# zenustech/zpc

Hardware: AMD Instinct MI355X
Metric: particle*steps/s (P2G+G2P) (higher is better)
Workload: dtype f32

## Files before the change

include/zs_rocm.h:

```cpp
#ifndef ZS_ROCM_H
#define ZS_ROCM_H
#include <stdbool.h>
#include <stddef.h>
#include <stdint.h>

#ifdef __cplusplus
extern "C" {
#endif

#if defined(__GNUC__)
#  define ZS_ROCM_EXPORT __attribute__((visibility("default")))
#else
#  define ZS_ROCM_EXPORT
#endif

typedef struct zs_rocm_policy zs_rocm_policy;

ZS_ROCM_EXPORT zs_rocm_policy *policy__device(void);
ZS_ROCM_EXPORT void del_policy__device(zs_rocm_policy *);
ZS_ROCM_EXPORT void zs_rocm_policy_sync(zs_rocm_policy *, int sync);
ZS_ROCM_EXPORT void zs_rocm_policy_profile(zs_rocm_policy *, int profile);
ZS_ROCM_EXPORT void zs_rocm_policy_device(zs_rocm_policy *, int procid);
ZS_ROCM_EXPORT void zs_rocm_policy_stream(zs_rocm_policy *, int streamid);
ZS_ROCM_EXPORT void zs_rocm_policy_listen(zs_rocm_policy *, int incomingProc, int incomingStreamid);
// ... 315 lines not shown
typedef struct {
  zs_rocm_attr mass;
  zs_rocm_attr pos;
  zs_rocm_attr vel;
  zs_rocm_attr C;
  zs_rocm_attr F;
  zs_rocm_attr logJp;
  zs_rocm_attr stress;
  size_t n;
} zs_rocm_particles;

enum {
  ZS_MPM_FIXED_COROTATED = 0, ZS_MPM_DRUCKER_PRAGER = 1, ZS_MPM_VONMISES_FIXED_COROTATED = 2, ZS_MPM_NACC = 3,
  ZS_MPM_EQUATION_OF_STATE = 4
};
typedef struct {
  int model;
  float dx, dt;
  float volume, E, nu;
  float cohesion, beta, yieldSurface;
  int volCorrection;
  int side;
  int keyIsOrigin;
  float yieldStress;
  float xi, Msqr;
  int hardeningOn;
  float bulk, viscosity;
} zs_rocm_mpm_params;
ZS_ROCM_EXPORT float zs_rocm_nacc_msqr(float fa);


ZS_ROCM_EXPORT void zs_rocm_mpm_compute_sparsity(zs_rocm_policy *, zs_rocm_bht_3 *, zs_rocm_attr pos, size_t n,
                                                 float dx, int side, int keyIsOrigin);
ZS_ROCM_EXPORT void zs_rocm_mpm_enlarge_sparsity(zs_rocm_policy *, zs_rocm_bht_3 *, const int lo[3], const int hi[3],
                                                 int keyStride);
typedef struct zs_rocm_index_buckets zs_rocm_index_buckets;
typedef struct {
  zs_rocm_hashtable *table;
  int *indices;
  int *offsets, *counts;
  int numBuckets, numEntries;
  float dx;
} zs_rocm_index_buckets_view;
ZS_ROCM_EXPORT zs_rocm_index_buckets *zs_rocm_index_buckets_create(void);
ZS_ROCM_EXPORT void zs_rocm_index_buckets_destroy(zs_rocm_index_buckets *);
ZS_ROCM_EXPORT void zs_rocm_index_buckets_get_view(const zs_rocm_index_buckets *, zs_rocm_index_buckets_view *out);
ZS_ROCM_EXPORT void zs_rocm_index_buckets_for_particles(zs_rocm_policy *, zs_rocm_index_buckets *, zs_rocm_attr pos, size_t n,
                                                        float dx, float displacement, size_t expectedCells);
ZS_ROCM_EXPORT void zs_rocm_index_buckets_for_partition(zs_rocm_policy *, zs_rocm_index_buckets *, zs_rocm_attr pos, size_t n, float dx,
                                                        const zs_rocm_bht_3 *table, int side, int keyIsOrigin);
ZS_ROCM_EXPORT void zs_rocm_mpm_partition_for_particles(zs_rocm_policy *, zs_rocm_hashtable *, zs_rocm_attr pos, size_t n,
                                                        float dx, int blocklen);
ZS_ROCM_EXPORT void zs_rocm_mpm_enlarge_sparsity__hashtable(zs_rocm_policy *, zs_rocm_hashtable *, const int lo[3],
                                                            const int hi[3]);

ZS_ROCM_EXPORT void zs_rocm_mpm_bin_particles(zs_rocm_policy *, const zs_rocm_bht_3 *, zs_rocm_attr pos, size_t n,
                                              float dx, int side, int keyIsOrigin, int *order, int *binStart,
                                              unsigned *cellCount);
ZS_ROCM_EXPORT void zs_rocm_mpm_build_neighbors(zs_rocm_policy *, const zs_rocm_bht_3 *, int *nbr, int keyStride);

ZS_ROCM_EXPORT void zs_rocm_mpm_p2g(zs_rocm_policy *, const zs_rocm_mpm_params *, zs_rocm_particles,
                                    const zs_rocm_bht_3 *, float *grid, size_t nblocks, const int *binStart,
                                    const unsigned *cellCount, const int *nbr);
ZS_ROCM_EXPORT void zs_rocm_mpm_grid_update(zs_rocm_policy *, const zs_rocm_mpm_params *, float *grid, size_t nblocks,
                                            const float extf[3], float *maxVelSqr);
enum { ZS_ROCM_GEOM_PLANE = 0, ZS_ROCM_GEOM_CUBOID = 1, ZS_ROCM_GEOM_SPHERE = 2, ZS_ROCM_GEOM_CYLINDER = 3 };
enum { ZS_ROCM_COLLIDER_STICKY = 0, ZS_ROCM_COLLIDER_SLIP = 1, ZS_ROCM_COLLIDER_SEPARATE = 2 };
typedef struct zs_rocm_collider {
  int geometry, type;
  float param[8];
  float s, dsdt;
  float R[9];
  float omega[3];
  float b[3], dbdt[3];
} zs_rocm_collider;
ZS_ROCM_EXPORT void zs_rocm_collider_init(zs_rocm_collider *c, int geometry, int type, const float *param, int nparam);
ZS_ROCM_EXPORT void zs_rocm_mpm_apply_boundary(zs_rocm_policy *, const zs_rocm_mpm_params *, const zs_rocm_bht_3 *, float *grid,
                                               size_t nblocks, const zs_rocm_collider *collider);
ZS_ROCM_EXPORT void zs_rocm_collider_resolve(zs_rocm_policy *, const zs_rocm_collider *collider, const float *x, float *v, size_t n,
                                             int *inside);
ZS_ROCM_EXPORT int zs_rocm_mpm_p2c2g(zs_rocm_policy *, const zs_rocm_mpm_params *, zs_rocm_particles, const zs_rocm_index_buckets *buckets,
                                     const zs_rocm_bht_3 *, float *grid, size_t nblocks, int kind);
ZS_ROCM_EXPORT void zs_rocm_mpm_pre_g2c2p(zs_rocm_policy *, zs_rocm_particles);
ZS_ROCM_EXPORT int zs_rocm_mpm_g2c2p(zs_rocm_policy *, const zs_rocm_mpm_params *, zs_rocm_particles, const zs_rocm_index_buckets *buckets,
                                     const zs_rocm_bht_3 *, const float *grid, size_t nblocks);
ZS_ROCM_EXPORT void zs_rocm_mpm_post_g2c2p(zs_rocm_policy *, const zs_rocm_mpm_params *, zs_rocm_particles);
ZS_ROCM_EXPORT int zs_rocm_mpm_g2c2p_step(zs_rocm_policy *, const zs_rocm_mpm_params *, zs_rocm_particles, const zs_rocm_bht_3 *,
                                          const float *grid, size_t nblocks);
ZS_ROCM_EXPORT void zs_rocm_mpm_g2p(zs_rocm_policy *, const zs_rocm_mpm_params *, zs_rocm_particles,
                                    const zs_rocm_bht_3 *, const float *grid, size_t nblocks, const int *binStart,
                                    const unsigned *cellCount, const int *nbr);
ZS_ROCM_EXPORT int zs_rocm_mpm_implicit_force(zs_rocm_policy *, const zs_rocm_mpm_params *, zs_rocm_particles, const zs_rocm_bht_3 *,
                                              size_t nblocks, const int *binStart, const unsigned *cellCount, const int *nbr,
                                              const float *vIn, float *fOut, float *trial);
ZS_ROCM_EXPORT int zs_rocm_mpm_implicit_multiply(zs_rocm_policy *, const zs_rocm_mpm_params *, zs_rocm_particles, const zs_rocm_bht_3 *,
                                                 const float *grid, size_t nblocks, const int *binStart, const unsigned *cellCount,
                                                 const int *nbr, const float *vIn, float *out);
ZS_ROCM_EXPORT int zs_rocm_mpm_implicit_project(zs_rocm_policy *, const zs_rocm_mpm_params *, const zs_rocm_bht_3 *, const float *grid,
                                                size_t nblocks, const zs_rocm_collider *collider, float *inout);
ZS_ROCM_EXPORT int zs_rocm_mpm_implicit_precondition(zs_rocm_policy *, const float *grid, size_t nblocks, int side, const float *in,
                                                     float *out);
ZS_ROCM_EXPORT void zs_rocm_dof_assign(zs_rocm_policy *, const float *a, float *b, size_t n);
ZS_ROCM_EXPORT void zs_rocm_dof_fill(zs_rocm_policy *, float *a, float v, size_t n);
ZS_ROCM_EXPORT int zs_rocm_dof_compwise(zs_rocm_policy *, int op, const float *a, const float *b, float *c, size_t n);
ZS_ROCM_EXPORT void zs_rocm_dof_linear_combine(zs_rocm_policy *, float m, const float *a, float n_, const float *b, float *c, size_t n);
ZS_ROCM_EXPORT void zs_rocm_dof_dot(zs_rocm_policy *, const float *a, const float *b, size_t n, float *out);
ZS_ROCM_EXPORT int zs_rocm_mpm_implicit_solve(zs_rocm_policy *, const zs_rocm_mpm_params *, zs_rocm_particles, const zs_rocm_bht_3 *,
                                              const float *grid, size_t nblocks, const int *binStart, const unsigned *cellCount,
                                              const int *nbr, const zs_rocm_collider *collider, const float *b, float *x, int maxIters,
                                              float tol, float relTol, int *iters);
typedef struct zs_rocm_levelset {
  zs_rocm_bht_view_lite table;
  const float *tiles;
  size_t numBlocks;
  int numChannels, sdfChannel, velChannel;
  float h;
  float origin[3];
  float background;
  unsigned *stats;
} zs_rocm_levelset;
ZS_ROCM_EXPORT int zs_rocm_levelset_sample(zs_rocm_policy *, const zs_rocm_levelset *, const float *x, size_t n, float *sdf, float *normal,
                                           float *vel);
ZS_ROCM_EXPORT int zs_rocm_levelset_collider_resolve(zs_rocm_policy *, const zs_rocm_collider *collider, const zs_rocm_levelset *, const float *x,
                                                     float *v, size_t n, int *inside);
ZS_ROCM_EXPORT int zs_rocm_mpm_apply_boundary_levelset(zs_rocm_policy *, const zs_rocm_mpm_params *, const zs_rocm_bht_3 *, float *grid,
                                                       size_t nblocks, const zs_rocm_collider *collider, const zs_rocm_levelset *);
ZS_ROCM_EXPORT int zs_rocm_mpm_implicit_project_levelset(zs_rocm_policy *, const zs_rocm_mpm_params *, const zs_rocm_bht_3 *, const float *grid,
                                                         size_t nblocks, const zs_rocm_collider *collider, const zs_rocm_levelset *,
                                                         float *inout);
ZS_ROCM_EXPORT int zs_rocm_mpm_implicit_solve_levelset(zs_rocm_policy *, const zs_rocm_mpm_params *, zs_rocm_particles, const zs_rocm_bht_3 *,
                                                       const float *grid, size_t nblocks, const int *binStart, const unsigned *cellCount,
                                                       const int *nbr, const zs_rocm_collider *collider, const zs_rocm_levelset *,
                                                       const float *b, float *x, int maxIters, float tol, float relTol, int *iters);
typedef struct zs_rocm_levelset_transition {
  zs_rocm_levelset src, dst;
  float stepDt, alpha, maxSpeed;
} zs_rocm_levelset_transition;
ZS_ROCM_EXPORT int zs_rocm_levelset_max_speed(zs_rocm_policy *, const zs_rocm_levelset *, float *out);
ZS_ROCM_EXPORT int zs_rocm_levelset_transition_sample(zs_rocm_policy *, const zs_rocm_levelset_transition *, const float *x, size_t n, float *sdf,
                                                      float *normal, float *vel);
ZS_ROCM_EXPORT int zs_rocm_levelset_transition_collider_resolve(zs_rocm_policy *, const zs_rocm_collider *collider,
                                                                const zs_rocm_levelset_transition *, const float *x, float *v, size_t n,
                                                                int *inside);
ZS_ROCM_EXPORT int zs_rocm_mpm_apply_boundary_transition(zs_rocm_policy *, const zs_rocm_mpm_params *, const zs_rocm_bht_3 *, float *grid,
                                                         size_t nblocks, const zs_rocm_collider *collider, const zs_rocm_levelset_transition *);
ZS_ROCM_EXPORT int zs_rocm_mpm_implicit_project_transition(zs_rocm_policy *, const zs_rocm_mpm_params *, const zs_rocm_bht_3 *, const float *grid,
                                                           size_t nblocks, const zs_rocm_collider *collider,
                                                           const zs_rocm_levelset_transition *, float *inout);
ZS_ROCM_EXPORT int zs_rocm_mpm_implicit_solve_transition(zs_rocm_policy *, const zs_rocm_mpm_params *, zs_rocm_particles, const zs_rocm_bht_3 *,
                                                         const float *grid, size_t nblocks, const int *binStart, const unsigned *cellCount,
                                                         const int *nbr, const zs_rocm_collider *collider,
                                                         const zs_rocm_levelset_transition *, const float *b, float *x, int maxIters, float tol,
                                                         float relTol, int *iters);
typedef struct zs_rocm_mesh zs_rocm_mesh;
typedef struct {
  const float *verts;
  const int *tris;
  const float *vel;
  const float *faceNormals, *vertNormals, *edgeNormals;
  zs_rocm_lbvh_view bvh;
  int numVerts, numTris;
} zs_rocm_mesh_view;
#define ZS_ROCM_MESH_STAT_WORDS 8
ZS_ROCM_EXPORT zs_rocm_mesh *zs_rocm_mesh_create(zs_rocm_policy *, const float *verts, size_t nv, const int *tris, size_t nt, const float *vel);
ZS_ROCM_EXPORT void zs_rocm_mesh_destroy(zs_rocm_mesh *);
ZS_ROCM_EXPORT int zs_rocm_mesh_refit(zs_rocm_policy *, zs_rocm_mesh *, const float *verts, const float *vel);
ZS_ROCM_EXPORT void zs_rocm_mesh_stats(zs_rocm_policy *, const zs_rocm_mesh *, int *out);
ZS_ROCM_EXPORT int zs_rocm_mesh_total_box(zs_rocm_policy *, const zs_rocm_mesh *, float *box6);
ZS_ROCM_EXPORT void zs_rocm_mesh_get_view(const zs_rocm_mesh *, zs_rocm_mesh_view *out);
ZS_ROCM_EXPORT int zs_rocm_mesh_closest_point(zs_rocm_policy *, const zs_rocm_mesh *, const float *points, size_t nq, float cap, float *dist,
                                              int *tri, int *feature, float *bary);
ZS_ROCM_EXPORT int zs_rocm_mesh_signed_distance(zs_rocm_policy *, const zs_rocm_mesh *, const float *points, size_t nq, float cap, float *sdf,
                                                float *vel);
ZS_ROCM_EXPORT size_t zs_rocm_mesh_levelset_count(zs_rocm_policy *, const zs_rocm_mesh *, const float *origin, float voxel, float band);
ZS_ROCM_EXPORT int zs_rocm_mesh_levelset_candidates(zs_rocm_policy *, const zs_rocm_mesh *, const float *origin, float voxel, float band,
                                                    zs_rocm_bht_3 *cand);
ZS_ROCM_EXPORT int zs_rocm_mesh_levelset_blocks(zs_rocm_policy *, const zs_rocm_mesh *, const float *origin, float voxel, float band,
                                                const zs_rocm_bht_3 *cand, size_t ncand, float *tiles, int numChannels, int *keep,
                                                unsigned *stats);
ZS_ROCM_EXPORT size_t zs_rocm_mesh_levelset_select(zs_rocm_policy *, const zs_rocm_bht_3 *cand, size_t ncand, const int *keep, int *keptKeys);
ZS_ROCM_EXPORT int zs_rocm_mesh_levelset_gather(zs_rocm_policy *, const zs_rocm_bht_3 *cand, size_t ncand, const int *keep, const float *tiles,
                                                const zs_rocm_bht_3 *table, float *dstTiles, int numChannels);
#define ZS_ROCM_SLOT_STATUS_WORDS (8 + 2 * 256)
ZS_ROCM_EXPORT size_t zs_rocm_mpm_slot_outbox_bytes(size_t nbins, int outboxCap, int which);
ZS_ROCM_EXPORT void zs_rocm_mpm_build_neighbors27(zs_rocm_policy *, const zs_rocm_bht_3 *, int *nbr27 , int keyStride);
ZS_ROCM_EXPORT int zs_rocm_mpm_slot_particles(zs_rocm_policy *, const zs_rocm_bht_3 *, zs_rocm_attr pos, size_t n, float dx, int side,
                                              int keyIsOrigin, int K, const float *src, float *dst, int C, unsigned *cellMask, int *status);
ZS_ROCM_EXPORT size_t zs_rocm_mpm_slot_list(zs_rocm_policy *, const unsigned *cellMask, size_t nbins, int K, int *slots);
typedef struct zs_rocm_slot_storage {
  unsigned *cellMask;
  int K;
  const int *nbr;
  const int *nbr27;
  int *moverCount;
  unsigned *claim;
  float *moverRec;
  int outboxCap;
  int *status;
  const unsigned char *blockEdge;
} zs_rocm_slot_storage;
ZS_ROCM_EXPORT void zs_rocm_mpm_partition_edge(zs_rocm_policy *, const zs_rocm_bht_3 *, unsigned char *edge , int keyStride,
                                               int lo, int hi);
ZS_ROCM_EXPORT void zs_rocm_mpm_slot_compute_sparsity(zs_rocm_policy *, const zs_rocm_bht_3 *oldTab, const unsigned *cellMask, size_t nblocksOld,
                                                      int side, int keyIsOrigin, zs_rocm_bht_3 *newTab);
ZS_ROCM_EXPORT int zs_rocm_mpm_reslot(zs_rocm_policy *, const zs_rocm_bht_3 *oldTab, const zs_rocm_bht_3 *newTab, int side, int K, int C,
                                      const float *oldBuf, float *newBuf, const unsigned *oldMask, unsigned *newMask, const float *oldGrid,
                                      float *newGrid, int *status);
ZS_ROCM_EXPORT int zs_rocm_mpm_g2p2g_slots(zs_rocm_policy *, const zs_rocm_mpm_params *, zs_rocm_particles, const zs_rocm_bht_3 *,
                                           const float *gridA, float *gridB, size_t nblocks, const zs_rocm_slot_storage *st, int writeAll,
                                           size_t blockBegin, size_t blockEnd, int finish);
ZS_ROCM_EXPORT int zs_rocm_mpm_g2p2g_slotted(zs_rocm_policy *, const zs_rocm_mpm_params *, zs_rocm_particles, const zs_rocm_bht_3 *,
                                             const float *gridA, float *gridB, size_t nblocks, unsigned *cellMask, int K, const int *nbr,
                                             const int *nbr27, int *moverCount, unsigned *claim, float *moverRec, int outboxCap,
                                             int writeAll, int *status);
ZS_ROCM_EXPORT int zs_rocm_mpm_g2p2g_slotted_range(zs_rocm_policy *, const zs_rocm_mpm_params *, zs_rocm_particles, const zs_rocm_bht_3 *,
                                                   const float *gridA, float *gridB, size_t nblocks, unsigned *cellMask, int K, const int *nbr,
                                                   const int *nbr27, int *moverCount, unsigned *claim, float *moverRec, int outboxCap,
                                                   int writeAll, int *status, size_t blockBegin, size_t blockEnd, int finish);
ZS_ROCM_EXPORT int zs_rocm_mpm_g2p2g(zs_rocm_policy *, const zs_rocm_mpm_params *, zs_rocm_particles, const zs_rocm_bht_3 *,
                                     const float *gridA, float *gridB, size_t nblocks, const int *binStart,
                                     const unsigned *cellCount, const int *nbr, int writeAll);
ZS_ROCM_EXPORT int zs_rocm_mpm_g2p2g_range(zs_rocm_policy *, const zs_rocm_mpm_params *, zs_rocm_particles, const zs_rocm_bht_3 *,
                                           const float *gridA, float *gridB, size_t nblocks, const int *binStart,
                                           const unsigned *cellCount, const int *nbr, int writeAll, size_t blockBegin,
                                           size_t blockEnd, int *driftFlag);
ZS_ROCM_EXPORT int zs_rocm_mpm_g2p2g_reorder_range(zs_rocm_policy *, const zs_rocm_mpm_params *, zs_rocm_particles particlesOut,
                                                   zs_rocm_particles particlesIn, const int *order, const zs_rocm_bht_3 *,
                                                   const float *gridA, float *gridB, size_t nblocks, const int *binStart,
                                                   const unsigned *cellCount, const int *nbr, int writeAll, size_t blockBegin,
                                                   size_t blockEnd, int *driftFlag);
ZS_ROCM_EXPORT void zs_rocm_mpm_update_stress(zs_rocm_policy *, const zs_rocm_mpm_params *, zs_rocm_particles);
ZS_ROCM_EXPORT int zs_rocm_mpm_stress_channels(void);
ZS_ROCM_EXPORT void zs_rocm_mpm_stress(zs_rocm_policy *, const zs_rocm_mpm_params *, float *F, float *logJp, size_t n, float *PF);
ZS_ROCM_EXPORT void zs_rocm_svd3(zs_rocm_policy *, const float *F, size_t n, float *U, float *S, float *V);

ZS_ROCM_EXPORT void zs_rocm_mpm_owner_rank(zs_rocm_policy *, zs_rocm_attr pos, size_t n, float dx, const int lo[3], const int hi[3],
                                           const int dims[3], int align, int *owner);
ZS_ROCM_EXPORT void zs_rocm_mpm_owner_counts(zs_rocm_policy *, const int *owner, size_t n, int world, int *counts);
ZS_ROCM_EXPORT void zs_rocm_mpm_halo_pack(zs_rocm_policy *, const float *grid, const int *blocks, size_t nb, int side,
                                          int chn0, int nchn, float *buf);
ZS_ROCM_EXPORT void zs_rocm_mpm_halo_unpack(zs_rocm_policy *, float *grid, const int *blocks, size_t nb, int side,
                                            int chn0, int nchn, const float *buf, int add);


typedef struct zs_rocm_dist zs_rocm_dist;
ZS_ROCM_EXPORT size_t zs_rocm_dist_unique_id_bytes(void);
ZS_ROCM_EXPORT int zs_rocm_dist_unique_id(void *out);
ZS_ROCM_EXPORT zs_rocm_dist *zs_rocm_dist_create(int rank, int world, const void *uniqueId, int device);
ZS_ROCM_EXPORT void zs_rocm_dist_destroy(zs_rocm_dist *);
ZS_ROCM_EXPORT int zs_rocm_dist_rank(const zs_rocm_dist *);
ZS_ROCM_EXPORT int zs_rocm_dist_world(const zs_rocm_dist *);
ZS_ROCM_EXPORT int zs_rocm_dist_comm_count(const zs_rocm_dist *);
ZS_ROCM_EXPORT int zs_rocm_dist_halo_exchange(zs_rocm_dist *, zs_rocm_policy *, float *grid, int side, int chn0, int nchn, const int *blocks,
                                              size_t totalBlocks, int npeers, const int *peerRank, const size_t *peerOffset,
                                              const size_t *peerCount, float *sendbuf, float *recvbuf);
ZS_ROCM_EXPORT int zs_rocm_dist_allreduce_f32(zs_rocm_dist *, zs_rocm_policy *, float *buf, size_t n, int op);
ZS_ROCM_EXPORT int zs_rocm_dist_allreduce_i64(zs_rocm_dist *, zs_rocm_policy *, long long *buf, size_t n, int op);
ZS_ROCM_EXPORT int zs_rocm_dist_alltoall_i64(zs_rocm_dist *, zs_rocm_policy *, const long long *send, long long *recv);
ZS_ROCM_EXPORT int zs_rocm_dist_alltoallv_f32(zs_rocm_dist *, zs_rocm_policy *, const float *send, const size_t *sendCounts,
                                              const size_t *sendOffsets, float *recv, const size_t *recvCounts, const size_t *recvOffsets);
ZS_ROCM_EXPORT int zs_rocm_dist_barrier(zs_rocm_dist *, zs_rocm_policy *);
typedef struct zs_rocm_halo_plan zs_rocm_halo_plan;
ZS_ROCM_EXPORT size_t zs_rocm_halo_plan_from_keys(const int *keysAll, const size_t *counts, int world, int rank, int *npeers, int *peerRank,
                                                  size_t *peerOffset, size_t *peerCount, int *blocks);
ZS_ROCM_EXPORT zs_rocm_halo_plan *zs_rocm_dist_halo_plan_create(zs_rocm_dist *, zs_rocm_policy *, const int *keys, size_t nblocks, int side);
ZS_ROCM_EXPORT void zs_rocm_dist_halo_plan_destroy(zs_rocm_halo_plan *);
ZS_ROCM_EXPORT int zs_rocm_dist_halo_plan_npeers(const zs_rocm_halo_plan *);
ZS_ROCM_EXPORT size_t zs_rocm_dist_halo_plan_blocks(const zs_rocm_halo_plan *);
ZS_ROCM_EXPORT size_t zs_rocm_dist_halo_plan_bytes(const zs_rocm_halo_plan *);
ZS_ROCM_EXPORT const int *zs_rocm_dist_halo_plan_block_list(const zs_rocm_halo_plan *);
ZS_ROCM_EXPORT int zs_rocm_dist_halo_plan_exchange(zs_rocm_halo_plan *, zs_rocm_dist *, zs_rocm_policy *, float *grid, int chn0, int nchn);
ZS_ROCM_EXPORT zs_rocm_halo_plan *zs_rocm_dist_halo_plan_from_lists(zs_rocm_dist *, int side, int npeers, const int *peerRank,
                                                                    const size_t *peerOffset, const size_t *peerCount, const int *blocks,
                                                                    size_t total);
typedef struct zs_rocm_mpm_step {
  const zs_rocm_mpm_params *params;
  zs_rocm_particles particles;
  const zs_rocm_bht_3 *table;
  const float *gridA;
  float *gridB;
  size_t nblocks;
  const zs_rocm_slot_storage *storage;
  int writeAll;
  float extf[3];
  float *maxVelSqr;
  const zs_rocm_collider *collider;
  size_t nBoundary;
  zs_rocm_dist *dist;
  zs_rocm_halo_plan *plan;
  zs_rocm_policy *commPolicy;
  float *haloGrid;
  void *evTransferBegin, *evTransferEnd;
  void **evBreakdown;
  int haloChannels;
  int rangeSchedule;
  float *handoverSnapshot;
  const zs_rocm_levelset *levelset;
} zs_rocm_mpm_step;
#define ZS_ROCM_STEP_EVENTS 8
#define ZS_ROCM_RANGES_IN_TURN 0
#define ZS_ROCM_RANGES_SIDE_BY_SIDE 1
#define ZS_ROCM_RANGES_ONE_LAUNCH 2
ZS_ROCM_EXPORT int zs_rocm_mpm_step_slotted(zs_rocm_policy *, const zs_rocm_mpm_step *);

#ifdef __cplusplus
}
#endif
#endif
```

zpc_amd/_lib.py:

```python
import ctypes as C
import os

_HERE = os.path.dirname(os.path.abspath(__file__))
LIB_PATH = os.path.join(_HERE, "lib", "libzsrocm.so")
if os.environ.get("ZS_ROCM_LIB"):
    LIB_PATH = os.environ["ZS_ROCM_LIB"]
    print("[zpc_amd] using HIP library %s" % LIB_PATH, flush=True)


class Port(C.Structure):
    _fields_ = [("base", C.c_void_p), ("idx", C.c_uint32), ("numTileBits", C.c_uint32),
                ("tileMask", C.c_uint32), ("numChns", C.c_uint32)]


class HashTableView(C.Structure):
    _fields_ = [("keys", C.c_void_p), ("indices", C.c_void_p), ("status", C.c_void_p), ("activeKeys", C.c_void_p),
                ("cnt", C.c_void_p), ("tableSize", C.c_int)]


class LBvhView(C.Structure):
    _fields_ = [("orderedBvs", C.c_void_p), ("parents", C.c_void_p), ("levels", C.c_void_p), ("leafInds", C.c_void_p),
                ("auxIndices", C.c_void_p), ("numNodes", C.c_int), ("numLeaves", C.c_int)]


# ... 51 lines not shown
def lib():
    global _lib
    if _lib is None:
        if not os.path.exists(LIB_PATH):
            raise RuntimeError(
                "libzsrocm.so not built (%s): run `python -m zpc_amd.build` -- zpc_amd has no CPU fallback" % LIB_PATH)
        try:
            import torch
        except ImportError:
            pass
        _lib = C.CDLL(LIB_PATH)
        _declare(_lib)
    return _lib


class Collider(C.Structure):
    _fields_ = [("geometry", C.c_int), ("type", C.c_int), ("param", C.c_float * 8), ("s", C.c_float), ("dsdt", C.c_float),
                ("R", C.c_float * 9), ("omega", C.c_float * 3), ("b", C.c_float * 3), ("dbdt", C.c_float * 3)]


class LevelSet(C.Structure):
    _fields_ = [("table", BhtViewLite), ("tiles", C.c_void_p), ("numBlocks", C.c_size_t), ("numChannels", C.c_int),
                ("sdfChannel", C.c_int), ("velChannel", C.c_int), ("h", C.c_float), ("origin", C.c_float * 3), ("background", C.c_float),
                ("stats", C.c_void_p)]


class LevelSetTransition(C.Structure):
    _fields_ = [("src", LevelSet), ("dst", LevelSet), ("stepDt", C.c_float), ("alpha", C.c_float), ("maxSpeed", C.c_float)]


class MeshView(C.Structure):
    _fields_ = [("verts", C.c_void_p), ("tris", C.c_void_p), ("vel", C.c_void_p), ("faceNormals", C.c_void_p), ("vertNormals", C.c_void_p),
                ("edgeNormals", C.c_void_p), ("bvh", LBvhView), ("numVerts", C.c_int), ("numTris", C.c_int)]


def _declare(L):
    vp, sz, i32, f32 = C.c_void_p, C.c_size_t, C.c_int, C.c_float
    L.policy__device.restype = vp
    L.del_policy__device.argtypes = [vp]
    for n in ("sync", "profile", "device", "stream", "block"):
        getattr(L, "zs_rocm_policy_" + n).argtypes = [vp, i32]
    L.zs_rocm_policy_listen.argtypes = [vp, i32, i32]
    L.zs_rocm_policy_shmem.argtypes = [vp, sz]
    L.zs_rocm_policy_external_stream.argtypes = [vp, vp]
    L.zs_rocm_policy_get_stream.argtypes = [vp]
    L.zs_rocm_policy_get_stream.restype = vp
    L.zs_rocm_policy_should_sync.argtypes = [vp]
    L.zs_rocm_policy_sync_ctx.argtypes = [vp]
    L.zs_rocm_policy_last_elapsed_ms.argtypes = [vp]
    L.zs_rocm_policy_last_elapsed_ms.restype = f32
    L.zs_rocm_memset.argtypes = [vp, vp, i32, sz]
    L.zs_rocm_dist_unique_id_bytes.restype = sz
    L.zs_rocm_dist_unique_id.argtypes = [vp]
    L.zs_rocm_dist_create.argtypes = [i32, i32, vp, i32]
    L.zs_rocm_dist_create.restype = vp
    L.zs_rocm_dist_destroy.argtypes = [vp]
    L.zs_rocm_dist_rank.argtypes = [vp]
    L.zs_rocm_dist_world.argtypes = [vp]
    L.zs_rocm_dist_comm_count.argtypes = [vp]
    L.zs_rocm_dist_comm_count.restype = C.c_int
    L.zs_rocm_dist_halo_exchange.argtypes = [vp, vp, vp, i32, i32, i32, vp, sz, i32, vp, vp, vp, vp, vp]
    L.zs_rocm_dist_allreduce_f32.argtypes = [vp, vp, vp, sz, i32]
    L.zs_rocm_dist_allreduce_i64.argtypes = [vp, vp, vp, sz, i32]
    L.zs_rocm_dist_alltoall_i64.argtypes = [vp, vp, vp, vp]
    L.zs_rocm_dist_alltoallv_f32.argtypes = [vp, vp, vp, vp, vp, vp, vp, vp]
    L.zs_rocm_dist_barrier.argtypes = [vp, vp]
    L.zs_rocm_halo_plan_from_keys.argtypes = [vp, vp, i32, i32, vp, vp, vp, vp, vp]
    L.zs_rocm_halo_plan_from_keys.restype = sz
    L.zs_rocm_dist_halo_plan_create.argtypes = [vp, vp, vp, sz, i32]
    L.zs_rocm_dist_halo_plan_create.restype = vp
    L.zs_rocm_dist_halo_plan_destroy.argtypes = [vp]
    L.zs_rocm_dist_halo_plan_npeers.argtypes = [vp]
    L.zs_rocm_dist_halo_plan_npeers.restype = i32
    L.zs_rocm_dist_halo_plan_blocks.argtypes = [vp]
    L.zs_rocm_dist_halo_plan_blocks.restype = sz
    L.zs_rocm_dist_halo_plan_bytes.argtypes = [vp]
    L.zs_rocm_dist_halo_plan_bytes.restype = sz
    L.zs_rocm_dist_halo_plan_block_list.argtypes = [vp]
    L.zs_rocm_dist_halo_plan_block_list.restype = vp
    L.zs_rocm_dist_halo_plan_exchange.argtypes = [vp, vp, vp, vp, i32, i32]
    L.zs_rocm_dist_halo_plan_exchange.restype = i32
    L.zs_rocm_mpm_slot_outbox_bytes.argtypes = [sz, i32, i32]
    L.zs_rocm_mpm_slot_outbox_bytes.restype = sz
    L.zs_rocm_mpm_build_neighbors27.argtypes = [vp, vp, vp, i32]
    L.zs_rocm_mpm_slot_particles.argtypes = [vp, vp, Port, sz, f32, i32, i32, i32, vp, vp, i32, vp, vp]
    L.zs_rocm_mpm_slot_particles.restype = i32
    L.zs_rocm_mpm_slot_list.argtypes = [vp, vp, sz, i32, vp]
    L.zs_rocm_mpm_slot_list.restype = sz
    L.zs_rocm_policy_temporary.argtypes = [vp, sz]
    L.zs_rocm_policy_temporary.restype = vp
    L.zs_rocm_policy_temporary_free.argtypes = [vp, vp]
    L.zs_rocm_last_error.argtypes = [i32]
    L.zs_rocm_clear_error.argtypes = [i32]
    L.launch__device.argtypes = [vp, vp, sz, vp]
    L.rocm_compile_program.argtypes = [C.c_char_p, i32, C.c_char_p, C.c_bool, C.c_bool, C.c_bool, C.c_bool, C.c_char_p]
    L.rocm_compile_program.restype = sz
    L.rocm_load_module.argtypes = [vp, C.c_char_p]
    L.rocm_load_module.restype = vp
    L.rocm_unload_module.argtypes = [vp, vp]
    L.rocm_get_kernel.argtypes = [vp, vp, C.c_char_p]
    L.rocm_get_kernel.restype = vp
    L.rocm_launch_kernel.argtypes = [vp, vp, sz, vp, vp]
    L.rocm_launch_kernel.restype = sz
    for T in ("int", "float", "double"):
        for op in ("reduce_sum", "reduce_prod", "reduce_min", "reduce_max", "exclusive_scan_sum",
                   "exclusive_scan_prod", "inclusive_scan_sum", "inclusive_scan_prod"):
            getattr(L, "%s__rocm_%s_1" % (op, T)).argtypes = [vp, Port, Port, Port]
        getattr(L, "radix_sort__rocm_%s_1" % T).argtypes = [vp, Port, Port, Port]
        getattr(L, "merge_sort__rocm_%s_1" % T).argtypes = [vp, Port, Port]
        getattr(L, "merge_sort_pair__rocm_%s_1" % T).argtypes = [vp, Port, Port, sz]
        getattr(L, "radix_sort_pair__rocm_%s_1" % T).argtypes = [vp, Port, Port, Port, Port, sz]
    for S, ct in (("i32", C.c_int32), ("i64", C.c_int64), ("f32", C.c_float), ("f64", C.c_double)):
        getattr(L, "zs_rocm_reduce_" + S).argtypes = [vp, vp, sz, vp, ct, i32]
        getattr(L, "zs_rocm_scan_" + S).argtypes = [vp, vp, sz, vp, ct, i32, i32]
    for S in ("i32", "u32", "i64", "u64"):
        getattr(L, "zs_rocm_radix_sort_" + S).argtypes = [vp, vp, vp, vp, vp, sz, i32, i32]
    for S in ("i32", "u32", "i64", "u64", "f32", "f64"):
        getattr(L, "zs_rocm_merge_sort_" + S).argtypes = [vp, vp, vp, sz, i32]


def _declare_containers(L):
    vp, sz, i32, f32, i8 = C.c_void_p, C.c_size_t, C.c_int, C.c_float, C.c_int8
    L.allocator.argtypes = [i32, i8]
    L.allocator.restype = vp
    L.del_allocator.argtypes = [vp]
    L.property_tags.argtypes = [C.POINTER(C.c_char_p), C.POINTER(C.c_int), sz]
    L.property_tags.restype = vp
    L.del_property_tags.argtypes = [vp]
    L.allocator_virtual.argtypes = [i32, i8, sz]
    L.allocator_virtual.restype = vp
    L.del_allocator_virtual.argtypes = [vp]
    L.property_tags_get_item.argtypes = [vp, sz, C.POINTER(C.c_char_p), C.POINTER(sz)]
    L.property_tags_get_size.argtypes = [vp]
    L.property_tags_get_size.restype = sz
    for T, ct in (("int", C.c_int), ("float", C.c_float), ("double", C.c_double)):
        for sfx in ("", "_virtual"):
            g = lambda n: getattr(L, (n % T) + sfx)
            g("container__v_%s").argtypes = [vp, sz]
            g("container__v_%s").restype = vp
            g("del_container__v_%s").argtypes = [vp]
            g("relocate_container__v_%s").argtypes = [vp, i32, i8]
            g("resize_container__v_%s").argtypes = [vp, sz]
            g("reset_container__v_%s").argtypes = [vp, i32]
            g("container_size__v_%s").argtypes = [vp]
            g("container_size__v_%s").restype = sz
            g("container_capacity__v_%s").argtypes = [vp]
            g("container_capacity__v_%s").restype = sz
            g("get_val_container__v_%s").argtypes = [vp]
            g("get_val_container__v_%s").restype = ct
            g("set_val_container__v_%s").argtypes = [vp, ct]
            g("get_val_i_container__v_%s").argtypes = [vp, sz]
            g("get_val_i_container__v_%s").restype = ct
            g("set_val_i_container__v_%s").argtypes = [vp, sz, ct]
            g("copy_to_container__v_%s").argtypes = [vp, vp]
            g("copy_from_container__v_%s").argtypes = [vp, vp]
            g("get_handle_container__v_%s").argtypes = [vp]
            g("get_handle_container__v_%s").restype = vp
            g("pyview__v_%s").argtypes = [vp]
            g("pyview__v_%s").restype = C.POINTER(C.c_void_p)
            g("pyview__v_const_%s").argtypes = [vp]
            g("pyview__v_const_%s").restype = C.POINTER(C.c_void_p)
            for it in ("get_iterator_1__v_%s", "get_iterator_1__v_const_%s", "get_iterator_3__v_%s", "get_iterator_3__v_const_%s"):
                g(it).argtypes = [vp, C.c_uint32]
                g(it).restype = Port
        getattr(L, "del_pyview__v_%s" % T).argtypes = [vp]
        getattr(L, "del_pyview__v_const_%s" % T).argtypes = [vp]
        getattr(L, "container_data__v_%s" % T).argtypes = [vp]
        getattr(L, "container_data__v_%s" % T).restype = vp
        for Lw in (8, 32, 64, 512):
            s = "%s_%d" % (T, Lw)
            for sfx in ("", "_virtual"):
                h = lambda n: getattr(L, (n % s) + sfx)
                h("container__tv_%s").argtypes = [vp, vp, sz]
                h("container__tv_%s").restype = vp
                h("del_container__tv_%s").argtypes = [vp]
                h("relocate_container__tv_%s").argtypes = [vp, i32, i8]
                h("resize_container__tv_%s").argtypes = [vp, sz]
                h("reset_container__tv_%s").argtypes = [vp, i32]
                for q in ("container_size__tv_%s", "container_capacity__tv_%s"):
                    h(q).argtypes = [vp]
                    h(q).restype = sz
                h("property_offset__tv_%s").argtypes = [vp, C.c_char_p]
                h("property_size__tv_%s").argtypes = [vp, C.c_char_p]
                for it in ("get_iterator_1__tv_%s", "get_iterator_3__tv_%s"):
                    h(it).argtypes = [vp, C.c_uint32, C.c_uint32]
                    h(it).restype = Port
                for it in ("get_iterator_1__tv_const_%s", "get_iterator_3__tv_const_%s"):
                    h(it).argtypes = [vp, C.c_uint32, C.c_uint32]
                    h(it).restype = Port
                for pv, rt in (("pyview__tv_%s", TvViewLite), ("pyview__tv_const_%s", TvViewLite), ("pyview__tvn_%s", TvNamedViewLite),
                               ("pyview__tvn_const_%s", TvNamedViewLite)):
                    h(pv).argtypes = [vp]
                    h(pv).restype = C.POINTER(rt)
                h("append_properties__rocm_tv_%s").argtypes = [vp, vp, vp]
            k = lambda n: getattr(L, n % s)
            for dv in ("del_pyview__tv_%s", "del_pyview__tv_const_%s", "del_pyview__tvn_%s", "del_pyview__tvn_const_%s"):
                k(dv).argtypes = [vp]
            k("container_num_channels__tv_%s").argtypes = [vp]
            k("container_num_channels__tv_%s").restype = sz
            k("container_data__tv_%s").argtypes = [vp]
            k("container_data__tv_%s").restype = vp
            k("zs_rocm_fill__tv_%s").argtypes = [vp, vp, ct]
            k("zs_rocm_reorder__tv_%s").argtypes = [vp, vp, vp, i32]
    L.zs_rocm_tv_from_aos_f32.argtypes = [vp, vp, sz, i32, i32, vp]
    L.zs_rocm_tv_to_aos_f32.argtypes = [vp, vp, sz, i32, i32, vp]
    L.zs_rocm_tv_scale_f32.argtypes = [vp, vp, sz, i32, i32, f32]
    L.zs_rocm_tv_gather_f32.argtypes = [vp, vp, vp, sz, i32, i32, vp]
    L.zs_rocm_tv_gather_channels_f32.argtypes = [vp, vp, vp, sz, i32, i32, vp, C.c_uint64]
    L.zs_rocm_tv_gather_rows_f32.argtypes = [vp, vp, vp, sz, i32, i32, vp]
    L.zs_rocm_tv_scatter_rows_f32.argtypes = [vp, vp, sz, i32, i32, vp, sz]
    for D, B in ((d, b) for d in (1, 2, 3, 4) for b in (16, 32)):
        s = "bht_int_%d_int_%d" % (D, B)
        for sfx in ("", "_virtual"):
            getattr(L, "relocate_container__" + s + sfx).argtypes = [vp, i32, i8]
            getattr(L, "pyview__bht_const_int_%d_int_%d" % (D, B) + sfx).argtypes = [vp]
            getattr(L, "pyview__bht_const_int_%d_int_%d" % (D, B) + sfx).restype = C.POINTER(BhtViewLite)
            if sfx:
                getattr(L, "container__" + s + sfx).argtypes = [vp, sz]
                getattr(L, "container__" + s + sfx).restype = vp
                getattr(L, "del_container__" + s + sfx).argtypes = [vp]
                getattr(L, "container_size__" + s + sfx).argtypes = [vp]
                getattr(L, "container_size__" + s + sfx).restype = sz
        getattr(L, "container__" + s).argtypes = [vp, sz]
        getattr(L, "container__" + s).restype = vp
        getattr(L, "del_container__" + s).argtypes = [vp]
        getattr(L, "container_size__" + s).argtypes = [vp]
        getattr(L, "container_size__" + s).restype = sz
        getattr(L, "container_capacity__" + s).argtypes = [vp]
        getattr(L, "container_capacity__" + s).restype = sz
        getattr(L, "reset_container__" + s).argtypes = [vp, i32]
        getattr(L, "pyview__" + s).argtypes = [vp]
        getattr(L, "pyview__" + s).restype = C.POINTER(BhtViewLite)
        getattr(L, "del_pyview__" + s).argtypes = [C.POINTER(BhtViewLite)]
        getattr(L, "resize_container__rocm_" + s).argtypes = [vp, vp, sz]
        getattr(L, "zs_rocm_insert__" + s).argtypes = [vp, vp, vp, sz, vp]
        getattr(L, "zs_rocm_query__" + s).argtypes = [vp, vp, vp, sz, vp]
        getattr(L, "zs_rocm_assign__" + s).argtypes = [vp, vp, vp, sz]
        getattr(L, "zs_rocm_reorder__" + s).argtypes = [vp, vp, vp, i32]
        getattr(L, "zs_rocm_canonicalize__" + s).argtypes = [vp, vp]
        getattr(L, "zs_rocm_canonicalize_axes__" + s).argtypes = [vp, vp, C.POINTER(C.c_int)]
        getattr(L, "zs_rocm_canonicalize_axes__" + s).restype = i32
        getattr(L, "zs_rocm_canonicalize_tail__" + s).argtypes = [vp, vp, C.POINTER(C.c_int), sz]
        getattr(L, "zs_rocm_canonicalize_tail__" + s).restype = i32
        getattr(L, "zs_rocm_order_morton__" + s).argtypes = [vp, vp]
    L.zs_rocm_hashtable_create.argtypes = [i32, sz, i32, i32]
    L.zs_rocm_hashtable_create.restype = vp
    L.zs_rocm_hashtable_destroy.argtypes = [vp]
    L.zs_rocm_hashtable_dim.argtypes = [vp]
    L.zs_rocm_hashtable_table_size.argtypes = [vp]
    L.zs_rocm_hashtable_table_size.restype = sz
    L.zs_rocm_hashtable_size.argtypes = [vp]
    L.zs_rocm_hashtable_get_view.argtypes = [vp, C.POINTER(HashTableView)]
    L.zs_rocm_hashtable_reset.argtypes = [vp, vp, i32]
    L.zs_rocm_hashtable_insert.argtypes = [vp, vp, vp, sz, vp]
    L.zs_rocm_hashtable_insert_ids.argtypes = [vp, vp, vp, vp, sz, vp]
    L.zs_rocm_hashtable_query.argtypes = [vp, vp, vp, sz, vp]
    L.zs_rocm_hashtable_entry.argtypes = [vp, vp, vp, sz, vp]
    L.zs_rocm_hashtable_resize.argtypes = [vp, vp, sz]
    L.zs_rocm_hashtable_preserve.argtypes = [vp, vp, sz]
    L.zs_rocm_mpm_partition_for_particles.argtypes = [vp, vp, Port, sz, f32, i32]
    L.zs_rocm_mpm_enlarge_sparsity__hashtable.argtypes = [vp, vp, C.POINTER(C.c_int), C.POINTER(C.c_int)]
    L.zs_rocm_lbvh_create.restype = vp
    L.zs_rocm_lbvh_destroy.argtypes = [vp]
    L.zs_rocm_lbvh_num_leaves.argtypes = [vp]
    L.zs_rocm_lbvh_num_leaves.restype = sz
    L.zs_rocm_lbvh_num_nodes.argtypes = [vp]
    L.zs_rocm_lbvh_num_nodes.restype = sz
    L.zs_rocm_lbvh_get_view.argtypes = [vp, C.POINTER(LBvhView)]
    L.zs_rocm_lbvh_build.argtypes = [vp, vp, vp, sz, i32]
    L.zs_rocm_lbvh_refit.argtypes = [vp, vp, vp, sz]
    L.zs_rocm_lbvh_total_box.argtypes = [vp, vp, vp]
    L.zs_rocm_lbvh_query_count.argtypes = [vp, vp, vp, sz, vp]
    L.zs_rocm_lbvh_query_fill.argtypes = [vp, vp, vp, sz, vp, vp]
    L.zs_rocm_lbvh_self_query_count.argtypes = [vp, vp, vp]
    L.zs_rocm_lbvh_self_query_fill.argtypes = [vp, vp, vp, vp]
    L.zs_rocm_index_buckets_create.restype = vp
    L.zs_rocm_index_buckets_destroy.argtypes = [vp]
    L.zs_rocm_index_buckets_get_view.argtypes = [vp, C.POINTER(IndexBucketsView)]
    L.zs_rocm_index_buckets_for_particles.argtypes = [vp, vp, Port, sz, f32, f32, sz]
    L.zs_rocm_index_buckets_for_partition.argtypes = [vp, vp, Port, sz, f32, vp, i32, i32]
    PP = C.POINTER(MpmParams)
    L.zs_rocm_mpm_compute_sparsity.argtypes = [vp, vp, Port, sz, f32, i32, i32]
    L.zs_rocm_mpm_enlarge_sparsity.argtypes = [vp, vp, C.POINTER(C.c_int), C.POINTER(C.c_int), i32]
    L.zs_rocm_mpm_bin_particles.argtypes = [vp, vp, Port, sz, f32, i32, i32, vp, vp, vp]
    L.zs_rocm_mpm_build_neighbors.argtypes = [vp, vp, vp, i32]
    L.zs_rocm_mpm_p2g.argtypes = [vp, PP, Particles, vp, vp, sz, vp, vp, vp]
    L.zs_rocm_mpm_owner_rank.argtypes = [vp, Port, sz, f32, C.POINTER(C.c_int), C.POINTER(C.c_int), C.POINTER(C.c_int), i32, vp]
    L.zs_rocm_mpm_owner_counts.argtypes = [vp, vp, sz, i32, vp]
    L.zs_rocm_mpm_owner_counts.restype = None
    L.zs_rocm_mpm_g2p2g.argtypes = [vp, PP, Particles, vp, vp, vp, sz, vp, vp, vp, i32]
    L.zs_rocm_mpm_g2p2g_range.argtypes = [vp, PP, Particles, vp, vp, vp, sz, vp, vp, vp, i32, sz, sz, vp]
    L.zs_rocm_mpm_g2p2g_slotted.argtypes = [vp, PP, Particles, vp, vp, vp, sz, vp, i32, vp, vp, vp, vp, vp, i32, i32, vp]
    L.zs_rocm_mpm_g2p2g_slotted.restype = i32
    L.zs_rocm_mpm_g2p2g_slotted_range.argtypes = [vp, PP, Particles, vp, vp, vp, sz, vp, i32, vp, vp, vp, vp, vp, i32, i32, vp, sz, sz, i32]
    L.zs_rocm_mpm_g2p2g_slotted_range.restype = i32
    L.zs_rocm_mpm_g2p2g_slots.argtypes = [vp, PP, Particles, vp, vp, vp, sz, C.POINTER(SlotStorage), i32, sz, sz, i32]
    L.zs_rocm_mpm_g2p2g_slots.restype = i32
    L.zs_rocm_mpm_partition_edge.argtypes = [vp, vp, vp, i32, i32, i32]
    L.zs_rocm_mpm_slot_compute_sparsity.argtypes = [vp, vp, vp, sz, i32, i32, vp]
    L.zs_rocm_mpm_reslot.argtypes = [vp, vp, vp, i32, i32, i32, vp, vp, vp, vp, vp, vp, vp]
    L.zs_rocm_mpm_reslot.restype = i32
    L.zs_rocm_mpm_step_slotted.argtypes = [vp, C.POINTER(MpmStep)]
    L.zs_rocm_mpm_step_slotted.restype = i32
    L.zs_rocm_dist_halo_plan_from_lists.argtypes = [vp, i32, i32, C.POINTER(C.c_int), C.POINTER(C.c_size_t), C.POINTER(C.c_size_t),
                                                    C.POINTER(C.c_int), sz]
    L.zs_rocm_dist_halo_plan_from_lists.restype = vp
    L.zs_rocm_mpm_g2p2g_reorder_range.argtypes = [vp, PP, Particles, Particles, vp, vp, vp, vp, sz, vp, vp, vp, i32, sz, sz, vp]
    L.zs_rocm_mpm_grid_update.argtypes = [vp, PP, vp, sz, C.POINTER(C.c_float), vp]
    L.zs_rocm_mpm_g2p.argtypes = [vp, PP, Particles, vp, vp, sz, vp, vp, vp]
    L.zs_rocm_mpm_p2c2g.argtypes = [vp, PP, Particles, vp, vp, vp, sz, i32]
    L.zs_rocm_mpm_p2c2g.restype = i32
    L.zs_rocm_mpm_pre_g2c2p.argtypes = [vp, Particles]
    L.zs_rocm_mpm_g2c2p.argtypes = [vp, PP, Particles, vp, vp, vp, sz]
    L.zs_rocm_mpm_g2c2p.restype = i32
    L.zs_rocm_mpm_post_g2c2p.argtypes = [vp, PP, Particles]
    L.zs_rocm_mpm_g2c2p_step.argtypes = [vp, PP, Particles, vp, vp, sz]
    L.zs_rocm_mpm_g2c2p_step.restype = i32
    L.zs_rocm_mpm_stress.argtypes = [vp, PP, vp, vp, sz, vp]
    L.zs_rocm_mpm_update_stress.argtypes = [vp, PP, Particles]
    L.zs_rocm_svd3.argtypes = [vp, vp, sz, vp, vp, vp]
    L.zs_rocm_nacc_msqr.argtypes = [f32]
    L.zs_rocm_nacc_msqr.restype = f32
    L.zs_rocm_collider_init.argtypes = [C.POINTER(Collider), i32, i32, C.POINTER(C.c_float), i32]
    L.zs_rocm_mpm_apply_boundary.argtypes = [vp, PP, vp, vp, sz, C.POINTER(Collider)]
    L.zs_rocm_collider_resolve.argtypes = [vp, C.POINTER(Collider), vp, vp, sz, vp]
    L.zs_rocm_mpm_implicit_force.argtypes = [vp, PP, Particles, vp, sz, vp, vp, vp, vp, vp, vp]
    L.zs_rocm_mpm_implicit_multiply.argtypes = [vp, PP, Particles, vp, vp, sz, vp, vp, vp, vp, vp]
    L.zs_rocm_mpm_implicit_project.argtypes = [vp, PP, vp, vp, sz, C.POINTER(Collider), vp]
    L.zs_rocm_mpm_implicit_precondition.argtypes = [vp, vp, sz, i32, vp, vp]
    L.zs_rocm_mpm_implicit_solve.argtypes = [vp, PP, Particles, vp, vp, sz, vp, vp, vp, C.POINTER(Collider), vp, vp, i32, f32, f32,
                                             C.POINTER(C.c_int)]
    for name in ("force", "multiply", "project", "precondition", "solve"):
        getattr(L, "zs_rocm_mpm_implicit_" + name).restype = i32
    PC, PL = C.POINTER(Collider), C.POINTER(LevelSet)
    L.zs_rocm_levelset_sample.argtypes = [vp, PL, vp, sz, vp, vp, vp]
    L.zs_rocm_levelset_collider_resolve.argtypes = [vp, PC, PL, vp, vp, sz, vp]
    L.zs_rocm_mpm_apply_boundary_levelset.argtypes = [vp, PP, vp, vp, sz, PC, PL]
    L.zs_rocm_mpm_implicit_project_levelset.argtypes = [vp, PP, vp, vp, sz, PC, PL, vp]
    L.zs_rocm_mpm_implicit_solve_levelset.argtypes = [vp, PP, Particles, vp, vp, sz, vp, vp, vp, PC, PL, vp, vp, i32, f32, f32,
                                                      C.POINTER(C.c_int)]
    for name in ("levelset_sample", "levelset_collider_resolve", "mpm_apply_boundary_levelset", "mpm_implicit_project_levelset",
                 "mpm_implicit_solve_levelset"):
        getattr(L, "zs_rocm_" + name).restype = i32
    PT = C.POINTER(LevelSetTransition)
    L.zs_rocm_levelset_max_speed.argtypes = [vp, PL, vp]
    L.zs_rocm_levelset_transition_sample.argtypes = [vp, PT, vp, sz, vp, vp, vp]
    L.zs_rocm_levelset_transition_collider_resolve.argtypes = [vp, PC, PT, vp, vp, sz, vp]
    L.zs_rocm_mpm_apply_boundary_transition.argtypes = [vp, PP, vp, vp, sz, PC, PT]
    L.zs_rocm_mpm_implicit_project_transition.argtypes = [vp, PP, vp, vp, sz, PC, PT, vp]
    L.zs_rocm_mpm_implicit_solve_transition.argtypes = [vp, PP, Particles, vp, vp, sz, vp, vp, vp, PC, PT, vp, vp, i32, f32, f32,
                                                        C.POINTER(C.c_int)]
    for name in ("levelset_max_speed", "levelset_transition_sample", "levelset_transition_collider_resolve", "mpm_apply_boundary_transition",
                 "mpm_implicit_project_transition", "mpm_implicit_solve_transition"):
        getattr(L, "zs_rocm_" + name).restype = i32
    L.zs_rocm_mesh_create.argtypes = [vp, vp, sz, vp, sz, vp]
    L.zs_rocm_mesh_create.restype = vp
    L.zs_rocm_mesh_destroy.argtypes = [vp]
    L.zs_rocm_mesh_destroy.restype = None
    L.zs_rocm_mesh_refit.argtypes = [vp, vp, vp, vp]
    L.zs_rocm_mesh_stats.argtypes = [vp, vp, C.POINTER(C.c_int)]
    L.zs_rocm_mesh_stats.restype = None
    L.zs_rocm_mesh_total_box.argtypes = [vp, vp, C.POINTER(C.c_float)]
    L.zs_rocm_mesh_get_view.argtypes = [vp, C.POINTER(MeshView)]
    L.zs_rocm_mesh_get_view.restype = None
    L.zs_rocm_mesh_closest_point.argtypes = [vp, vp, vp, sz, f32, vp, vp, vp, vp]
    L.zs_rocm_mesh_signed_distance.argtypes = [vp, vp, vp, sz, f32, vp, vp]
    P3 = C.POINTER(C.c_float)
    L.zs_rocm_mesh_levelset_count.argtypes = [vp, vp, P3, f32, f32]
    L.zs_rocm_mesh_levelset_count.restype = sz
    L.zs_rocm_mesh_levelset_candidates.argtypes = [vp, vp, P3, f32, f32, vp]
    L.zs_rocm_mesh_levelset_blocks.argtypes = [vp, vp, P3, f32, f32, vp, sz, vp, i32, vp, vp]
    L.zs_rocm_mesh_levelset_select.argtypes = [vp, vp, sz, vp, vp]
    L.zs_rocm_mesh_levelset_select.restype = sz
    L.zs_rocm_mesh_levelset_gather.argtypes = [vp, vp, sz, vp, vp, vp, vp, i32]
    for name in ("refit", "total_box", "closest_point", "signed_distance", "levelset_candidates", "levelset_blocks", "levelset_gather"):
        getattr(L, "zs_rocm_mesh_" + name).restype = i32
    L.zs_rocm_dof_assign.argtypes = [vp, vp, vp, sz]
    L.zs_rocm_dof_assign.restype = None
    L.zs_rocm_dof_fill.argtypes = [vp, vp, f32, sz]
    L.zs_rocm_dof_fill.restype = None
    L.zs_rocm_dof_compwise.argtypes = [vp, i32, vp, vp, vp, sz]
    L.zs_rocm_dof_compwise.restype = i32
    L.zs_rocm_dof_linear_combine.argtypes = [vp, f32, vp, f32, vp, vp, sz]
    L.zs_rocm_dof_linear_combine.restype = None
    L.zs_rocm_dof_dot.argtypes = [vp, vp, vp, sz, vp]
    L.zs_rocm_dof_dot.restype = None
    L.zs_rocm_mpm_halo_pack.argtypes = [vp, vp, vp, sz, i32, i32, i32, vp]
    L.zs_rocm_mpm_halo_unpack.argtypes = [vp, vp, vp, sz, i32, i32, i32, vp, i32]


_declare_base = _declare


def _declare(L):
    _declare_base(L)
    _declare_containers(L)
```

zpc_amd/csrc/common.hpp:

```cpp
#pragma once
#include <hip/hip_runtime.h>

#include <cstdint>
#include <cstdio>
#include <cstdlib>
#include <map>
#include <mutex>
#include <vector>

#include "../../include/zs_rocm.h"

namespace zsr {

constexpr int kWave = 64;
constexpr int kNumSpareStreams = 32;
constexpr size_t kCtlBytes = 132 << 10;
constexpr size_t kCtlDesc8 = 32 << 10, kCtlTicket = 128 << 10;
constexpr size_t kCtlScanTiles = 4096;

struct DeviceContext {
  int dev = 0;
  hipStream_t streams[kNumSpareStreams] = {};
  hipEvent_t events[kNumSpareStreams + 1] = {};
  int errorStatus = 0;
  bool errorPrinted = false;
  int cuCount = 0;
  std::mutex mtx;
  struct Block {
    char *ptr = nullptr;
    size_t cap = 0;
  };
  struct Arena {
    std::vector<Block> blocks;
    char *ctl = nullptr;
    unsigned scanGen = 0, ticketShadow = 0;
  };
  std::map<hipStream_t, Arena> arenas;
};

DeviceContext &context(int dev);
int current_device();
void report_error(hipError_t e, const char *what, const char *file, int line);

struct DeviceGuard {
  int prev, dev;
  explicit DeviceGuard(int d) : prev(current_device()), dev(d) {
    if (dev >= 0 && dev != prev) (void)hipSetDevice(dev);
  }
  ~DeviceGuard() {
    if (dev >= 0 && dev != prev) (void)hipSetDevice(prev);
  }
};

#define ZSR_CHECK(expr)                                                  \
  do {                                                                   \
    hipError_t _e = (expr);                                              \
    if (_e != hipSuccess) ::zsr::report_error(_e, #expr, __FILE__, __LINE__); \
  } while (0)

}

struct zs_rocm_allocator {
  int memsrc;
  int8_t devid;
  size_t virtualReserve = 0;
};

struct zs_rocm_policy {
  int sync = 1;
  int profile = 0;
  int device = -1;
  int streamid = -1;
  int listenProc = -1, listenStream = -1;
  size_t shmem = 0;
  int block = 0;
  hipStream_t external = nullptr;
  bool hasExternal = false;
  float lastMs = 0.f;
};

namespace zsr {

struct Launch {
  explicit Launch(zs_rocm_policy *p, const char *what);
  ~Launch();
  hipStream_t stream = nullptr;
  int dev = 0, prevDev = 0;
  zs_rocm_policy *pol;
  const char *what;
  hipEvent_t t0 = nullptr, t1 = nullptr;
  void *temp(size_t bytes);
  std::vector<size_t> tempUsed;
  DeviceContext::Arena &control();
  char *scan_control(size_t numTiles, unsigned &gen, unsigned &ticketBase, bool &wrapped);
  void scan_control_reset();
  unsigned cu_count();
};

template <class T> struct Port {
  T *base;
  uint32_t idx, bits, mask, chns;
  __host__ __device__ __forceinline__ size_t off(size_t i) const {
    size_t j = (size_t)idx + i;
    return (((j >> bits) * (size_t)chns) << bits) | (j & (size_t)mask);
  }
  __host__ __device__ __forceinline__ T &operator[](size_t i) const { return base[off(i)]; }
  __host__ __device__ __forceinline__ size_t cstride() const { return (size_t)mask + 1; }
  __host__ __device__ bool contiguous() const { return chns == 1; }
};
template <class T, class P> inline Port<T> make_port(const P &p) {
  return Port<T>{(T *)p.base, p.idx, p.numTileBits, p.tileMask, p.numChns};
}
template <class T> inline Port<T> contiguous_port(T *p) { return Port<T>{p, 0u, 0u, 0u, 1u}; }

inline unsigned ceil_div(size_t a, size_t b) { return (unsigned)((a + b - 1) / b); }

int mpm_g2p2g_slots_signal(zs_rocm_policy *pol, const zs_rocm_mpm_params *p, zs_rocm_particles ps, const zs_rocm_bht_3 *tab, const float *gridA,
                           float *gridB, size_t nblocks, const zs_rocm_slot_storage *st, int writeAll, size_t blockBegin, size_t blockEnd, int finish,
                           unsigned long long *signal, size_t signalBlocks);
bool levelset_collider_ok(const zs_rocm_collider *collider, const zs_rocm_levelset *levelset);
void levelset_blocks_enqueue(hipStream_t stream, const zs_rocm_mpm_params *p, const int *activeKeys, float *grid, size_t nblocks,
                             const zs_rocm_collider *collider, const zs_rocm_levelset *levelset, float *dof);
bool levelset_ok(const zs_rocm_levelset *levelset);
bool transition_collider_ok(const zs_rocm_collider *collider, const zs_rocm_levelset_transition *transition);
bool transition_blocks_enqueue(hipStream_t stream, const zs_rocm_mpm_params *p, const int *activeKeys, float *grid, size_t nblocks,
                               const zs_rocm_collider *collider, const zs_rocm_levelset_transition *transition, float *dof);

}

namespace zsr {

__device__ __forceinline__ int lane_id() { return (int)(threadIdx.x & 63); }
__device__ __forceinline__ int wave_id() { return (int)(threadIdx.x >> 6); }

template <class T> __device__ __forceinline__ T shfl_down(T v, int d) { return __shfl_down(v, d, 64); }
template <class T> __device__ __forceinline__ T shfl_up(T v, int d) { return __shfl_up(v, d, 64); }
template <class T> __device__ __forceinline__ T shfl(T v, int l) { return __shfl(v, l, 64); }

__device__ __forceinline__ unsigned long long lanemask_lt() {
  return (1ull << (threadIdx.x & 63)) - 1ull;
}

enum { OP_PLUS = 0, OP_MUL = 1, OP_MIN = 2, OP_MAX = 3 };
template <int OP, class T> __host__ __device__ __forceinline__ T apply(T a, T b) {
  if constexpr (OP == OP_PLUS) return a + b;
  else if constexpr (OP == OP_MUL) return a * b;
  else if constexpr (OP == OP_MIN) return a < b ? a : b;
  else return a > b ? a : b;
}

}
```

zpc_amd/csrc/dist.hip:

```cpp
#include <rccl/rccl.h>

#include <algorithm>
#include <cstring>
#include <utility>
#include <vector>

#include "common.hpp"

struct zs_rocm_dist {
  ncclComm_t comm = nullptr;
  int rank = 0, world = 1, device = 0;
  bool broken = false;
};

namespace zsr {
static int nccl_check(ncclResult_t r, const char *what, const char *file, int line) {
  if (r == ncclSuccess) return 0;
  fprintf(stderr, "[zs_rocm | rccl] %s failed: %s at %s:%d\n", what, ncclGetErrorString(r), file, line);
  report_error(hipErrorUnknown, what, file, line);
  return -1;
}
#define ZSR_NCCL(expr)                                               \
  do {                                                               \
    if (::zsr::nccl_check((expr), #expr, __FILE__, __LINE__)) return -1; \
// ... 34 lines not shown
zs_rocm_dist *zs_rocm_dist_create(int rank, int world, const void *uniqueId, int device) {
  if (world < 1 || rank < 0 || rank >= world || !uniqueId) return nullptr;
  auto *d = new zs_rocm_dist;
  d->rank = rank;
  d->world = world;
  d->device = device >= 0 ? device : current_device();
  DeviceGuard guard(d->device);
  ncclUniqueId id;
  std::memcpy(&id, uniqueId, sizeof(id));
  if (nccl_check(ncclCommInitRank(&d->comm, world, id, rank), "ncclCommInitRank", __FILE__, __LINE__)) {
    delete d;
    return nullptr;
  }
  int count = -1, urank = -1, cudev = -1;
  (void)ncclCommCount(d->comm, &count);
  (void)ncclCommUserRank(d->comm, &urank);
  (void)ncclCommCuDevice(d->comm, &cudev);
  if (count != world || urank != rank) {
    fprintf(stderr, "[zs_rocm] dist_create: RCCL communicator has %d ranks (asked for %d), this rank is %d (asked for %d), device %d\n", count, world,
            urank, rank, cudev);
    (void)ncclCommAbort(d->comm);
    delete d;
    return nullptr;
  }
  if (getenv("ZS_ROCM_DIST_VERBOSE"))
    fprintf(stderr, "[zs_rocm] dist_create: rank %d of ncclCommCount = %d on HIP device %d\n", urank, count, cudev);
  return d;
}
int zs_rocm_dist_comm_count(const zs_rocm_dist *d) {
  int count = -1;
  if (!d || !d->comm || ncclCommCount(d->comm, &count) != ncclSuccess) return -1;
  return count;
}
void zs_rocm_dist_destroy(zs_rocm_dist *d) {
  if (!d) return;
  if (d->comm) (void)(d->broken ? ncclCommAbort(d->comm) : ncclCommDestroy(d->comm));
  delete d;
}
int zs_rocm_dist_rank(const zs_rocm_dist *d) { return d->rank; }
int zs_rocm_dist_world(const zs_rocm_dist *d) { return d->world; }

int zs_rocm_dist_halo_exchange(zs_rocm_dist *d, zs_rocm_policy *pol, float *grid, int side, int chn0, int nchn, const int *blocks,
                               size_t totalBlocks, int npeers, const int *peerRank, const size_t *peerOffset, const size_t *peerCount,
                               float *sendbuf, float *recvbuf) {
  if (!d || !totalBlocks || npeers <= 0) return 0;
  if ((side != 4 && side != 8) || chn0 < 0 || nchn < 1 || chn0 + nchn > 7) {
    report_error(hipErrorInvalidValue, "halo_exchange: side must be 4 | 8 and [chn0, chn0 + nchn) within the 7 grid channels", __FILE__, __LINE__);
    return -1;
  }
  const size_t bf = (size_t)nchn * side * side * side;
  if (same_device(d, pol, "halo_exchange")) return -1;
  zs_rocm_mpm_halo_pack(pol, grid, blocks, totalBlocks, side, chn0, nchn, sendbuf);
  {
    Launch L(pol, "halo_exchange");
    ZSR_NCCL(ncclGroupStart());
    for (int k = 0; k < npeers; ++k) {
      ZSR_NCCL_G(d, ncclSend(sendbuf + peerOffset[k] * bf, peerCount[k] * bf, ncclFloat, peerRank[k], d->comm, L.stream));
      ZSR_NCCL_G(d, ncclRecv(recvbuf + peerOffset[k] * bf, peerCount[k] * bf, ncclFloat, peerRank[k], d->comm, L.stream));
    }
    ZSR_NCCL(ncclGroupEnd());
  }
  zs_rocm_mpm_halo_unpack(pol, grid, blocks, totalBlocks, side, chn0, nchn, recvbuf, 2);
  return 0;
}

size_t zs_rocm_halo_plan_from_keys(const int *keysAll, const size_t *counts, int world, int rank, int *npeers, int *peerRank,
                                   size_t *peerOffset, size_t *peerCount, int *blocks) {
  struct Key {
    int k[3];
    bool operator<(const Key &o) const { return k[0] != o.k[0] ? k[0] < o.k[0] : (k[1] != o.k[1] ? k[1] < o.k[1] : k[2] < o.k[2]); }
    bool operator==(const Key &o) const { return k[0] == o.k[0] && k[1] == o.k[1] && k[2] == o.k[2]; }
  };
  std::vector<size_t> start(world + 1, 0);
  for (int r = 0; r < world; ++r) start[r + 1] = start[r] + counts[r];
  std::vector<std::pair<Key, int>> mine(counts[rank]);
  for (size_t i = 0; i < counts[rank]; ++i) {
    const int *q = keysAll + 3 * (start[rank] + i);
    mine[i] = {Key{{q[0], q[1], q[2]}}, (int)i};
  }
  std::sort(mine.begin(), mine.end(), [](const auto &a, const auto &b) { return a.first < b.first; });
  size_t total = 0;
  int np = 0;
  std::vector<Key> theirs;
  for (int p = 0; p < world; ++p) {
    if (p == rank || counts[p] == 0 || mine.empty()) continue;
    theirs.resize(counts[p]);
    for (size_t i = 0; i < counts[p]; ++i) {
      const int *q = keysAll + 3 * (start[p] + i);
      theirs[i] = Key{{q[0], q[1], q[2]}};
    }
    std::sort(theirs.begin(), theirs.end());
    size_t a = 0, b = 0, n = 0;
    while (a < mine.size() && b < theirs.size()) {
      if (mine[a].first < theirs[b]) ++a;
      else if (theirs[b] < mine[a].first) ++b;
      else {
        if (blocks) blocks[total + n] = mine[a].second;
        ++n, ++a, ++b;
      }
    }
    if (n) {
      if (peerRank) {
        peerRank[np] = p;
        peerOffset[np] = total;
        peerCount[np] = n;
      }
      ++np;
      total += n;
    }
  }
  if (npeers) *npeers = np;
  return total;
}

struct zs_rocm_halo_plan {
  hipEvent_t evBoundary = nullptr, evDone = nullptr;
  hipEvent_t evReady = nullptr;
  unsigned long long *signal = nullptr;
  unsigned long long signalTarget = 0;
  int device = 0, side = 0, npeers = 0;
  size_t total = 0;
  std::vector<int> peerRank;
  std::vector<size_t> peerOffset, peerCount;
  int *blocks = nullptr;
  float *sendbuf = nullptr, *recvbuf = nullptr;
};
zs_rocm_halo_plan *zs_rocm_dist_halo_plan_create(zs_rocm_dist *d, zs_rocm_policy *pol, const int *keys, size_t nblocks, int side) {
  if (!d || (side != 4 && side != 8)) return nullptr;
  if (same_device(d, pol, "halo_plan_create")) return nullptr;
  Launch L(pol, "halo_plan");
  auto *plan = new zs_rocm_halo_plan;
  plan->device = d->device;
  plan->side = side;
  const int world = d->world;
  unsigned long long *cntD = (unsigned long long *)L.temp(sizeof(unsigned long long) * (size_t)(world + 1));
  const unsigned long long mineCnt = nblocks;
  std::vector<unsigned long long> cntH(world);
  bool ok = hipMemcpyAsync(cntD + world, &mineCnt, sizeof(mineCnt), hipMemcpyHostToDevice, L.stream) == hipSuccess;
  ok = ok && ncclAllGather(cntD + world, cntD, 1, ncclUint64, d->comm, L.stream) == ncclSuccess;
  ok = ok && hipMemcpyAsync(cntH.data(), cntD, sizeof(unsigned long long) * world, hipMemcpyDeviceToHost, L.stream) == hipSuccess;
  ok = ok && hipStreamSynchronize(L.stream) == hipSuccess;
  if (!ok) {
    report_error(hipErrorUnknown, "halo plan: count all-gather", __FILE__, __LINE__);
    delete plan;
    return nullptr;
  }
  size_t mx = 1;
  for (int r = 0; r < world; ++r) mx = std::max<size_t>(mx, cntH[r]);
  int *padD = (int *)L.temp(sizeof(int) * 3 * mx * (size_t)(world + 1));
  int *mineD = padD + 3 * mx * (size_t)world;
  ok = hipMemsetAsync(mineD, 0, sizeof(int) * 3 * mx, L.stream) == hipSuccess;
  if (nblocks) ok = ok && hipMemcpyAsync(mineD, keys, sizeof(int) * 3 * nblocks, hipMemcpyDeviceToDevice, L.stream) == hipSuccess;
  ok = ok && ncclAllGather(mineD, padD, 3 * mx, ncclInt32, d->comm, L.stream) == ncclSuccess;
  std::vector<int> padH(3 * mx * (size_t)world);
  ok = ok && hipMemcpyAsync(padH.data(), padD, sizeof(int) * padH.size(), hipMemcpyDeviceToHost, L.stream) == hipSuccess;
  ok = ok && hipStreamSynchronize(L.stream) == hipSuccess;
  if (!ok) {
    report_error(hipErrorUnknown, "halo plan: key all-gather", __FILE__, __LINE__);
    delete plan;
    return nullptr;
  }
  std::vector<int> keysAll;
  std::vector<size_t> counts(world);
  for (int r = 0; r < world; ++r) {
    counts[r] = cntH[r];
    keysAll.insert(keysAll.end(), padH.begin() + 3 * mx * (size_t)r, padH.begin() + 3 * (mx * (size_t)r + counts[r]));
  }
  int np = 0;
  const size_t total = zs_rocm_halo_plan_from_keys(keysAll.data(), counts.data(), world, d->rank, &np, nullptr, nullptr, nullptr, nullptr);
  plan->npeers = np;
  plan->total = total;
  plan->peerRank.resize(np);
  plan->peerOffset.resize(np);
  plan->peerCount.resize(np);
  std::vector<int> blocksH(total);
  zs_rocm_halo_plan_from_keys(keysAll.data(), counts.data(), world, d->rank, &np, plan->peerRank.data(), plan->peerOffset.data(),
                              plan->peerCount.data(), blocksH.data());
  if (total) {
    DeviceGuard guard(d->device);
    const size_t bf = (size_t)7 * side * side * side;
    ok = hipMalloc((void **)&plan->blocks, sizeof(int) * total) == hipSuccess && hipMalloc((void **)&plan->sendbuf, sizeof(float) * total * bf) == hipSuccess
         && hipMalloc((void **)&plan->recvbuf, sizeof(float) * total * bf) == hipSuccess
         && hipMemcpy(plan->blocks, blocksH.data(), sizeof(int) * total, hipMemcpyHostToDevice) == hipSuccess;
    if (!ok) {
      report_error(hipErrorOutOfMemory, "halo plan: buffers", __FILE__, __LINE__);
      zs_rocm_dist_halo_plan_destroy(plan);
      return nullptr;
    }
  }
  return plan;
}
zs_rocm_halo_plan *zs_rocm_dist_halo_plan_from_lists(zs_rocm_dist *d, int side, int npeers, const int *peerRank, const size_t *peerOffset,
                                                     const size_t *peerCount, const int *blocks, size_t total) {
  if (!d || (side != 4 && side != 8) || npeers < 0 || (total && (!blocks || !peerRank || !peerOffset || !peerCount))) return nullptr;
  auto *plan = new zs_rocm_halo_plan;
  plan->device = d->device;
  plan->side = side;
  plan->npeers = npeers;
  plan->total = total;
  plan->peerRank.assign(peerRank, peerRank + npeers);
  plan->peerOffset.assign(peerOffset, peerOffset + npeers);
  plan->peerCount.assign(peerCount, peerCount + npeers);
  if (total) {
    DeviceGuard guard(d->device);
    const size_t bf = (size_t)7 * side * side * side;
    const bool ok = hipMalloc((void **)&plan->blocks, sizeof(int) * total) == hipSuccess && hipMalloc((void **)&plan->sendbuf, sizeof(float) * total * bf) == hipSuccess
                    && hipMalloc((void **)&plan->recvbuf, sizeof(float) * total * bf) == hipSuccess
                    && hipMemcpy(plan->blocks, blocks, sizeof(int) * total, hipMemcpyHostToDevice) == hipSuccess;
    if (!ok) {
      report_error(hipErrorOutOfMemory, "halo plan: buffers", __FILE__, __LINE__);
      zs_rocm_dist_halo_plan_destroy(plan);
      return nullptr;
    }
  }
  return plan;
}
void zs_rocm_dist_halo_plan_destroy(zs_rocm_halo_plan *p) {
  if (!p) return;
  DeviceGuard guard(p->device);
  if (p->evBoundary) (void)hipEventDestroy(p->evBoundary);
  if (p->evReady) (void)hipEventDestroy(p->evReady);
  if (p->signal) (void)hipFree(p->signal);
  if (p->evDone) (void)hipEventDestroy(p->evDone);
  if (p->blocks) (void)hipFree(p->blocks);
  if (p->sendbuf) (void)hipFree(p->sendbuf);
  if (p->recvbuf) (void)hipFree(p->recvbuf);
  delete p;
}
int zs_rocm_dist_halo_plan_npeers(const zs_rocm_halo_plan *p) { return p ? p->npeers : 0; }
size_t zs_rocm_dist_halo_plan_blocks(const zs_rocm_halo_plan *p) { return p ? p->total : 0; }
size_t zs_rocm_dist_halo_plan_bytes(const zs_rocm_halo_plan *p) { return p ? p->total * (size_t)7 * p->side * p->side * p->side * sizeof(float) : 0; }
const int *zs_rocm_dist_halo_plan_block_list(const zs_rocm_halo_plan *p) { return p ? p->blocks : nullptr; }
int zs_rocm_dist_halo_plan_exchange(zs_rocm_halo_plan *p, zs_rocm_dist *d, zs_rocm_policy *pol, float *grid, int chn0, int nchn) {
  if (!p || !p->total) return 0;
  if (chn0 < 0 || nchn < 1 || chn0 + nchn > 7) {
    report_error(hipErrorInvalidValue, "halo_plan_exchange: [chn0, chn0 + nchn) must lie within the 7 grid channels", __FILE__, __LINE__);
    return -1;
  }
  return zs_rocm_dist_halo_exchange(d, pol, grid, p->side, chn0, nchn, p->blocks, p->total, p->npeers, p->peerRank.data(), p->peerOffset.data(),
                                    p->peerCount.data(), p->sendbuf, p->recvbuf);
}

static ncclRedOp_t red_op(int op) { return op == 1 ? ncclMax : (op == 2 ? ncclMin : ncclSum); }
int zs_rocm_dist_allreduce_f32(zs_rocm_dist *d, zs_rocm_policy *pol, float *buf, size_t n, int op) {
  if (!d || !n) return 0;
  if (same_device(d, pol, "allreduce_f32")) return -1;
  Launch L(pol, "allreduce_f32");
  ZSR_NCCL(ncclAllReduce(buf, buf, n, ncclFloat, red_op(op), d->comm, L.stream));
  return 0;
}
int zs_rocm_dist_allreduce_i64(zs_rocm_dist *d, zs_rocm_policy *pol, long long *buf, size_t n, int op) {
  if (!d || !n) return 0;
  if (same_device(d, pol, "allreduce_i64")) return -1;
  Launch L(pol, "allreduce_i64");
  ZSR_NCCL(ncclAllReduce(buf, buf, n, ncclInt64, red_op(op), d->comm, L.stream));
  return 0;
}
int zs_rocm_dist_alltoall_i64(zs_rocm_dist *d, zs_rocm_policy *pol, const long long *send, long long *recv) {
  if (!d) return 0;
  if (same_device(d, pol, "alltoall_i64")) return -1;
  Launch L(pol, "alltoall_i64");
  ZSR_NCCL(ncclGroupStart());
  for (int r = 0; r < d->world; ++r) {
    ZSR_NCCL_G(d, ncclSend(send + r, 1, ncclInt64, r, d->comm, L.stream));
    ZSR_NCCL_G(d, ncclRecv(recv + r, 1, ncclInt64, r, d->comm, L.stream));
  }
  ZSR_NCCL(ncclGroupEnd());
  return 0;
}
int zs_rocm_dist_alltoallv_f32(zs_rocm_dist *d, zs_rocm_policy *pol, const float *send, const size_t *sendCounts, const size_t *sendOffsets,
                               float *recv, const size_t *recvCounts, const size_t *recvOffsets) {
  if (!d) return 0;
  if (same_device(d, pol, "alltoallv_f32")) return -1;
  Launch L(pol, "alltoallv_f32");
  ZSR_NCCL(ncclGroupStart());
  for (int r = 0; r < d->world; ++r) {
    if (sendCounts[r]) ZSR_NCCL_G(d, ncclSend(send + sendOffsets[r], sendCounts[r], ncclFloat, r, d->comm, L.stream));
    if (recvCounts[r]) ZSR_NCCL_G(d, ncclRecv(recv + recvOffsets[r], recvCounts[r], ncclFloat, r, d->comm, L.stream));
  }
  ZSR_NCCL(ncclGroupEnd());
  return 0;
}
int zs_rocm_dist_barrier(zs_rocm_dist *d, zs_rocm_policy *pol) {
  if (!d) return 0;
  if (same_device(d, pol, "dist_barrier")) return -1;
  Launch L(pol, "dist_barrier");
  int *flag = (int *)L.temp(sizeof(int));
  ZSR_CHECK(hipMemsetAsync(flag, 0, sizeof(int), L.stream));
  ZSR_NCCL(ncclAllReduce(flag, flag, 1, ncclInt32, ncclSum, d->comm, L.stream));
  ZSR_CHECK(hipStreamSynchronize(L.stream));
  return 0;
}

}
static __global__ void step_gate_kernel(const unsigned long long *signal, unsigned long long target) {
  const unsigned long long t0 = wall_clock64();
  while (__hip_atomic_load(signal, __ATOMIC_RELAXED, __HIP_MEMORY_SCOPE_AGENT) < target) {
    __builtin_amdgcn_s_sleep(64);
    if (wall_clock64() - t0 > 1000000000ull) __builtin_trap();
  }
}
extern "C" {

int zs_rocm_mpm_step_slotted(zs_rocm_policy *pol, const zs_rocm_mpm_step *a) {
  if (!pol || !a || !a->params || !a->table || !a->gridA || !a->gridB || !a->storage) return -1;
  if (a->levelset && !zsr::levelset_collider_ok(a->collider, a->levelset)) return -1;
  const size_t nb = a->nblocks;
  if (!nb) return 0;
  const int side = a->params->side;
  const size_t gridBytes = nb * (size_t)7 * side * side * side * sizeof(float);
  zs_rocm_memset(pol, a->gridB, 0, gridBytes);
  float *const hgrid = a->haloGrid ? a->haloGrid : a->gridB;
  const bool exchange = a->dist && a->plan && a->plan->total;
  if (a->haloChannels < 0 || a->haloChannels > 7) return -1;
  if (a->rangeSchedule < ZS_ROCM_RANGES_IN_TURN || a->rangeSchedule > ZS_ROCM_RANGES_ONE_LAUNCH) return -1;
  if (a->rangeSchedule == ZS_ROCM_RANGES_ONE_LAUNCH && side != 8) return -1;
  const int hch = a->haloChannels ? a->haloChannels : 7;
  const bool overlap = exchange && a->commPolicy && a->nBoundary > 0 && a->nBoundary < nb;
  int rc = 0;
  auto stamp = [&](void *ev) {
    if (!ev) return;
    Launch L(pol, "step: event");
    ZSR_CHECK(hipEventRecord((hipEvent_t)ev, L.stream));
  };
  auto bd = [&](int k, zs_rocm_policy *on) {
    if (!a->evBreakdown || !a->evBreakdown[k]) return;
    Launch L(on, "step: breakdown event");
    ZSR_CHECK(hipEventRecord((hipEvent_t)a->evBreakdown[k], L.stream));
  };
  stamp(a->evTransferBegin);
  bd(0, pol);
  if (overlap) {
    zs_rocm_halo_plan *p = a->plan;
    if (!p->evBoundary || !p->evDone) {
      DeviceGuard guard(p->device);
      if (!p->evBoundary && hipEventCreateWithFlags(&p->evBoundary, hipEventDisableTiming) != hipSuccess) p->evBoundary = nullptr;
      if (!p->evDone && hipEventCreateWithFlags(&p->evDone, hipEventDisableTiming) != hipSuccess) p->evDone = nullptr;
      if (!p->evBoundary || !p->evDone) {
        report_error(hipErrorOutOfMemory, "step_slotted: could not create the overlap events", __FILE__, __LINE__);
        return -1;
      }
    }
    const int sched = a->rangeSchedule;
    if (sched == ZS_ROCM_RANGES_ONE_LAUNCH) {
      if (!p->signal) {
        DeviceGuard guard(p->device);
        if (hipMalloc((void **)&p->signal, sizeof(unsigned long long)) != hipSuccess) {
          p->signal = nullptr;
          report_error(hipErrorOutOfMemory, "step_slotted: could not allocate the boundary signal", __FILE__, __LINE__);
          return -1;
        }
        Launch L(pol, "step: boundary signal := 0");
        ZSR_CHECK(hipMemsetAsync(p->signal, 0, sizeof(unsigned long long), L.stream));
        ZSR_CHECK(hipStreamSynchronize(L.stream));
        p->signalTarget = 0;
      }
      rc = mpm_g2p2g_slots_signal(pol, a->params, a->particles, a->table, a->gridA, a->gridB, nb, a->storage, a->writeAll, 0, nb, 1, p->signal, a->nBoundary);
      if (rc) return rc;
      p->signalTarget += a->nBoundary;
      {
        Launch C(a->commPolicy, "step: gate");
        hipLaunchKernelGGL(step_gate_kernel, dim3(1), dim3(1), 0, C.stream, (const unsigned long long *)p->signal, p->signalTarget);
      }
      bd(1, a->commPolicy);
    } else {
      const bool sideBySide = sched == ZS_ROCM_RANGES_SIDE_BY_SIDE;
      zs_rocm_policy *const bpol = sideBySide ? a->commPolicy : pol;
      if (sideBySide) {
        if (!p->evReady) {
          DeviceGuard guard(p->device);
          if (hipEventCreateWithFlags(&p->evReady, hipEventDisableTiming) != hipSuccess) {
            p->evReady = nullptr;
            report_error(hipErrorOutOfMemory, "step_slotted: could not create the overlap events", __FILE__, __LINE__);
            return -1;
          }
        }
        {
          Launch L(pol, "step: grids ready");
          ZSR_CHECK(hipEventRecord(p->evReady, L.stream));
        }
        Launch C(a->commPolicy, "step: boundary range start");
        ZSR_CHECK(hipStreamWaitEvent(C.stream, p->evReady, 0));
      }
      rc = zs_rocm_mpm_g2p2g_slots(bpol, a->params, a->particles, a->table, a->gridA, a->gridB, nb, a->storage, a->writeAll, 0, a->nBoundary, 0);
      if (rc) return rc;
      bd(1, bpol);
      {
        Launch L(bpol, "step: boundary done");
        ZSR_CHECK(hipEventRecord(p->evBoundary, L.stream));
      }
      if (!sideBySide) {
        Launch C(a->commPolicy, "step: exchange start");
        ZSR_CHECK(hipStreamWaitEvent(C.stream, p->evBoundary, 0));
      }
    }
    bd(3, a->commPolicy);
    if (a->handoverSnapshot)
      zs_rocm_mpm_halo_pack(a->commPolicy, a->gridB, p->blocks, p->total, p->side, 0, 1, a->handoverSnapshot);
    const int rcx = zs_rocm_dist_halo_plan_exchange(p, a->dist, a->commPolicy, hgrid, 0, hch);
    bd(4, a->commPolicy);
    {
      Launch C(a->commPolicy, "step: exchange done");
      ZSR_CHECK(hipEventRecord(p->evDone, C.stream));
    }
    if (sched == ZS_ROCM_RANGES_IN_TURN) {
      rc = zs_rocm_mpm_g2p2g_slots(pol, a->params, a->particles, a->table, a->gridA, a->gridB, nb, a->storage, a->writeAll, a->nBoundary, nb, 1);
    } else if (sched == ZS_ROCM_RANGES_SIDE_BY_SIDE) {
      rc = zs_rocm_mpm_g2p2g_slots(pol, a->params, a->particles, a->table, a->gridA, a->gridB, nb, a->storage, a->writeAll, a->nBoundary, nb, 0);
      {
        Launch L(pol, "step: wait for the boundary range");
        ZSR_CHECK(hipStreamWaitEvent(L.stream, p->evBoundary, 0));
      }
      const int rcf = zs_rocm_mpm_g2p2g_slots(pol, a->params, a->particles, a->table, a->gridA, a->gridB, nb, a->storage, a->writeAll, nb, nb, 1);
      if (!rc) rc = rcf;
    }
    bd(2, pol);
    stamp(a->evTransferEnd);
    {
      Launch L(pol, "step: wait for the exchange");
      ZSR_CHECK(hipStreamWaitEvent(L.stream, p->evDone, 0));
    }
    bd(5, pol);
    if (rcx || rc) return rcx ? rcx : rc;
  } else {
    bd(1, pol);
    rc = zs_rocm_mpm_g2p2g_slots(pol, a->params, a->particles, a->table, a->gridA, a->gridB, nb, a->storage, a->writeAll, 0, nb, 1);
    if (rc) return rc;
    bd(2, pol);
    stamp(a->evTransferEnd);
    bd(3, pol);
    if (exchange) {
      rc = zs_rocm_dist_halo_plan_exchange(a->plan, a->dist, pol, hgrid, 0, hch);
      if (rc) return rc;
    }
    bd(4, pol);
    bd(5, pol);
  }
  if (a->maxVelSqr) zs_rocm_memset(pol, a->maxVelSqr, 0, sizeof(float));
  zs_rocm_mpm_grid_update(pol, a->params, a->gridB, nb, a->extf, a->maxVelSqr);
  if (a->levelset) rc = zs_rocm_mpm_apply_boundary_levelset(pol, a->params, a->table, a->gridB, nb, a->collider, a->levelset);
  else if (a->collider) zs_rocm_mpm_apply_boundary(pol, a->params, a->table, a->gridB, nb, a->collider);
  bd(6, pol);
  if (a->dist && a->maxVelSqr) rc = zs_rocm_dist_allreduce_f32(a->dist, pol, a->maxVelSqr, 1, 1);
  bd(7, pol);
  return rc;
}

}
```

zpc_amd/csrc/mpm_slot.hpp:

```cpp
#pragma once
#include "mpm_arena.hpp"
#include "mpm_fused_common.hpp"

namespace zsr {

constexpr int SL_REC = 48;
constexpr int SLR_DCELL = 14, SLR_FLAG = 15, SLR_V = 16, SLR_C = 19, SLR_PF = 28;

struct SlotArgs {
  const float *gridA;
  float *gridB;
  unsigned *cellMask;
  int K;
  const int *nbr;
  const int *nbr27;
  int *moverCount;
  unsigned *claim;
  float *moverRec;
  int *status;
  int binBase, nbins, nbinsAll;
  int cap;
  const unsigned char *blockEdge;
  unsigned long long *signal;
  int signalBlocks;
};

constexpr int SL_NCTR = 256, SL_SENT = 8, SL_DELIVERED = 8 + SL_NCTR;
__device__ __forceinline__ int neighbour_bin8(const int *row27, int blk, int sub, int code) {
  if (code == 13) return blk * 8 + sub;
  const int dd[3] = {code / 9 - 1, (code / 3) % 3 - 1, code % 3 - 1};
  int sx[3] = {((sub >> 2) & 1) + dd[0], ((sub >> 1) & 1) + dd[1], (sub & 1) + dd[2]}, bo[3];
#pragma unroll
  for (int d = 0; d < 3; ++d) {
    bo[d] = sx[d] < 0 ? -1 : (sx[d] > 1 ? 1 : 0);
    sx[d] &= 1;
  }
  const int nb = row27[(bo[0] + 1) * 9 + (bo[1] + 1) * 3 + (bo[2] + 1)];
  return nb < 0 ? -1 : nb * 8 + ((sx[0] * 2 + sx[1]) * 2 + sx[2]);
}

constexpr int SL_NG = 9;
constexpr int SL_KMAX = 32;
constexpr int SL_ARRQ = 4;
constexpr int SL_XQ = 64;

__device__ __forceinline__ int nth_low_bit(unsigned w, unsigned t) {
  for (unsigned k = 0; k < t && w; ++k) w &= w - 1u;
  return w ? __ffs((int)w) - 1 : -1;
}
struct SlotShared {
  float *varena;
  float *parena;
  float *stage;
  unsigned long long *smask;
  unsigned short *tab;
  unsigned *mask0;
  unsigned *clr;
  unsigned *arrLocal;
  const int *nbrBlk;
  const int *nbrBin;
  unsigned (*arrCnt)[64];
  unsigned short (*arrQ)[64][SL_ARRQ];
  unsigned *xCnt;
  unsigned (*xq)[SL_XQ];
  int *outCount, *sent, *homed, *xOver;
};

template <int SIDE, class FM, class FV, class FC, class FP>
__device__ __forceinline__ void scatter_node_task(const MpmDev &mp, int node, int ch, const int (&nc)[3], const float (&d0)[3], FM fm, FV fv, FC fC,
                                                  FP fP, const int *nbrBlk, float *gridB, int *status) {
  constexpr int NC = SIDE * SIDE * SIDE;
  const int sel[3] = {node / 9, (node / 3) % 3, node % 3};
  float Wt = 1.f, xi[3];
  int g[3], code = 0;
#pragma unroll
  for (int d = 0; d < 3; ++d) {
    const float u = sel[d] == 0 ? 1.5f - d0[d] : (sel[d] == 1 ? d0[d] - 1.0f : d0[d] - 0.5f);
    Wt *= sel[d] == 1 ? 0.75f - u * u : 0.5f * u * u;
    xi[d] = (float)sel[d] * mp.dx - d0[d] * mp.dx;
    g[d] = nc[d] + sel[d];
    code = code * 3 + (g[d] < 0 ? 0 : (g[d] >= SIDE ? 2 : 1));
  }
  float val;
  if (ch == 0) {
    val = fm() * Wt;
  } else if (ch < 4) {
    const int d = ch - 1;
    val = Wt * fm() * (fv(d) + (fC(d) * xi[0] + fC(3 + d) * xi[1] + fC(6 + d) * xi[2]));
  } else {
    const int d = ch - 4;
    const float dxi = mp.dxi;
    const float kscale = mp.fscale;
    val = (fP(d) * kscale * xi[0] + fP(3 + d) * kscale * xi[1] + fP(6 + d) * kscale * xi[2]) * Wt;
  }
  const int bn = nbrBlk[code];
  if (bn >= 0) {
    const int cell = ((g[0] & (SIDE - 1)) * SIDE + (g[1] & (SIDE - 1))) * SIDE + (g[2] & (SIDE - 1));
    if (val != 0.f) unsafeAtomicAdd(gridB + ((size_t)bn * 7 + ch) * NC + cell, val);
  } else if (ch == 0) {
    status[2] = 1;
  }
}

template <int SIDE, class GEO>
__device__ __forceinline__ void outbox_scatter_global(const MpmDev &mp, const GEO &geo, const float *recs, int n, int w, int lane,
                                                      const int *nbrBlk, float *gridB, int *status) {
  const float dxi = mp.dxi;
#pragma unroll 1
  for (int q = 0;; ++q) {
    const int j = w + 8 * (q / 3), p = q % 3;
    if (j >= n) break;
    const int t = p * 64 + lane;
    const float *rc = recs + (size_t)j * SL_REC;
    if (t >= 189 || (reinterpret_cast<const unsigned *>(rc)[SLR_FLAG] & 1u) == 0u) continue;
    int nc[3];
    float d0[3];
#pragma unroll
    for (int d = 0; d < 3; ++d) {
      const float X = rc[1 + d] * dxi;
      const float fl = floorf(X - 0.5f);
      d0[d] = X - fl;
      nc[d] = (int)fl - geo.org[d] + geo.o[d];
    }
    scatter_node_task<SIDE>(mp, t % 27, t / 27, nc, d0, [&]() { return rc[0]; }, [&](int d) { return rc[SLR_V + d]; },
                            [&](int k) { return rc[SLR_C + k]; }, [&](int k) { return rc[SLR_PF + k]; }, nbrBlk, gridB, status);
  }
}

template <int SIDE, int CS, class GEO>
__device__ __forceinline__ void slot_xlist_scatter(const MpmDev &mp, const GEO &geo, const float *stage, const unsigned *xq, int nx, int lane,
                                                   const int *nbrBlk, const SlotArgs &A) {
  using S = ConsumerSet<CS>;
  constexpr int NC = SIDE * SIDE * SIDE;
  const int node = lane & 31, half = lane >> 5;
  if (node >= 27 || nx <= 0) return;
  const StencilNodeLane sn(node);
#pragma unroll 1
  for (int k = half; k < nx; k += 2) {
    const unsigned e = xq[k];
    const float *st = stage + (size_t)((e & 1023u) >> 6) * (G2P2G_QF * 64) + (e & 63u);
    float Wt = 1.f;
    int g[3], code = 0;
#pragma unroll
    for (int q = 0; q < 3; ++q) {
      Wt *= sn.weight(q, st[(1 + q) * 64]);
      g[q] = (int)((e >> (10 + 3 * q)) & 7u) - 1 + geo.o[q] + sn.sel[q];
      code = code * 3 + 1 + (g[q] >= SIDE ? 1 : 0) - (g[q] < 0 ? 1 : 0);
    }
    const int bn = nbrBlk[code];
    if (bn >= 0) {
      const int cell = ((g[0] & (SIDE - 1)) * SIDE + (g[1] & (SIDE - 1))) * SIDE + (g[2] & (SIDE - 1));
      float *gp = A.gridB + ((size_t)bn * 7 + S::CH0) * NC + cell;
#pragma unroll
      for (int q = 0; q < S::NA; ++q) {
        const float val = sn.value<CS>(st, Wt, q);
        if (val != 0.f) unsafeAtomicAdd(gp + q * NC, val);
      }
    } else if (S::MASS) {
      A.status[2] = 1;
    }
  }
}


struct SlotBinView {
  int bin;
  int org[3];
  size_t rowBase;
  unsigned kmask;
  const float *va;
  unsigned *mask0;
  unsigned *clr;
  unsigned *arrLocal;
  const int *nbrBin;
  int *outCount, *sent, *homed, *xOver;
  unsigned (*arrBlk)[64];
  const unsigned (*maskBlk)[64];
};

template <int SIDE, int SMODEL, bool WRITE_ALL, class VA, bool INBLK = false, class REC, class WAIT>
__device__ __forceinline__ bool slot_produce_entry(const MpmDev &mp, const ParticlesDev &ps, const REC &cur, unsigned code0, size_t i0, int lane,
                                                   unsigned spos, float *myStage, const SlotBinView &bv, const SlotArgs &A, unsigned *arrCnt,
                                                   unsigned short (*arrQ)[SL_ARRQ], unsigned *xCnt, unsigned *xq, WAIT beforeStage) {
  constexpr int LW = 64;
  constexpr bool DP = model_uses_logjp(SMODEL);
  constexpr bool FLUID = model_is_fluid(SMODEL);
  const float dxi = mp.dxi;
  const float D_inv = mp.D_inv;
  bool valid = false;
  const int cell = (int)(code0 & 63u), r = (int)(code0 >> 6);
  const int cx = cell >> 4, cy = (cell >> 2) & 3, cz = cell & 3;
  Arena ar;
  make_arena(mp.dx, mp.dxi, cur.pos, ar);
  const int ocx = ar.corner[0] - bv.org[0], ocy = ar.corner[1] - bv.org[1], ocz = ar.corner[2] - bv.org[2];
  if (ocx != cx || ocy != cy || ocz != cz) {
    A.status[4] = 1;
  } else {
    float vel[3], C[9];
    g2p_gather_lds<VA>(mp, ar, bv.va + VA::at(ocx, ocy, ocz), D_inv, vel, C);
    float pos[3];
#pragma unroll
    for (int d = 0; d < 3; ++d) pos[d] = cur.pos[d] + vel[d] * mp.dt;
    float F[9], PF[9];
    advance_state<FLUID>(cur.F, C, mp.dt, F);
    float lpn[3];
    int nc[3];
#pragma unroll
    for (int d = 0; d < 3; ++d) {
      const float X = pos[d] * dxi;
      const float fl = floorf(X - 0.5f);
      nc[d] = (int)fl - bv.org[d];
      lpn[d] = X - fl;
    }
    const float pm = cur.m;
    float plj = 0.f;
    if constexpr (DP) plj = cur.logJp;
    const bool moved = nc[0] != cx || nc[1] != cy || nc[2] != cz;
    const bool edge = !(lpn[0] >= 0.5f && lpn[0] < 1.5f && lpn[1] >= 0.5f && lpn[1] < 1.5f && lpn[2] >= 0.5f && lpn[2] < 1.5f);
    bool outbox = false;
    bool staged = !moved;
    bool home = false;
    bool byList = false;
    bool lowered = false;
    bool keep = false;
    unsigned recFlag = 0u;
    float *rec = nullptr;
    POff<LW> o = particle_offset<LW>(ps.pos.chns, i0);
    if (moved) {
      int code = 0;
      bool far = false;
#pragma unroll
      for (int d = 0; d < 3; ++d) {
        far = far || (unsigned)(nc[d] + 1) > 5u;
        code = code * 3 + (nc[d] < 0 ? 0 : (nc[d] > 3 ? 2 : 1));
      }
      const int dl = ((nc[0] & 3) * 4 + (nc[1] & 3)) * 4 + (nc[2] & 3);
      unsigned dcell = 0xffffffffu;
      bool viaX = true;
      const int dbin = far ? -1 : (code == 13 ? bv.bin : bv.nbrBin[code]);
      const bool local = !far && (INBLK ? dbin >= 0 && (dbin >> 3) == (bv.bin >> 3) : code == 13);
      if (far) {
        A.status[4] = 1;
        viaX = false;
        keep = true;
      } else if (local) {
        unsigned *const arr = INBLK ? bv.arrBlk[dbin & 7] : bv.arrLocal;
        const unsigned m0 = INBLK ? bv.maskBlk[dbin & 7][dl] : bv.mask0[dl];
        const int rr = nth_low_bit(~m0 & bv.kmask, atomicAdd(&arr[dl], 1u));
        if (rr >= 0) {
          home = true;
          const size_t row = INBLK ? (size_t)dbin * (size_t)A.K : bv.rowBase;
          o = particle_offset<LW>(ps.pos.chns, (row + (size_t)rr) * 64 + (size_t)dl);
        } else {
          A.status[1] = 1;
          keep = true;
        }
        if (code == 13) {
          const unsigned q = edge ? (unsigned)SL_ARRQ : atomicAdd(&arrCnt[dl], 1u);
          if (q < (unsigned)SL_ARRQ) {
            viaX = false;
            staged = true;
            arrQ[dl][q] = (unsigned short)spos;
          }
        }
      } else if (dbin >= 0) {
        outbox = true;
        dcell = (unsigned)dbin * 64u + (unsigned)dl;
      } else {
        A.status[2] = 1;
        keep = true;
      }
      if (viaX) {
        const unsigned k = atomicAdd(xCnt, 1u);
        if (k < (unsigned)SL_XQ) {
          staged = true;
          xq[k] = spos | ((unsigned)(nc[0] + 1) << 10) | ((unsigned)(nc[1] + 1) << 13) |
                       ((unsigned)(nc[2] + 1) << 16);
        } else {
          outbox = true;
          recFlag = 1u;
          atomicAdd(bv.xOver, 1);
        }
      }
      if (outbox) {
        const int k = atomicAdd(bv.outCount, 1);
        if (k < A.cap) {
          rec = A.moverRec + ((size_t)bv.bin * A.cap + (size_t)k) * SL_REC;
#pragma unroll
          for (int d = 0; d < 3; ++d) rec[1 + d] = pos[d];
#pragma unroll
          for (int d = 0; d < 9; ++d) rec[4 + d] = F[d];
          if (WRITE_ALL || recFlag) {
#pragma unroll
            for (int d = 0; d < 3; ++d) rec[SLR_V + d] = vel[d];
#pragma unroll
            for (int d = 0; d < 9; ++d) rec[SLR_C + d] = C[d];
          }
          reinterpret_cast<unsigned *>(rec)[SLR_DCELL] = dcell;
          reinterpret_cast<unsigned *>(rec)[SLR_FLAG] = recFlag | (code0 << 1);
        } else {
          A.status[0] = 1;
          keep = !home;
        }
      }
      if (home || keep) {
        pstore_state<LW, FLUID>(ps.F, o, F);
        pstore<LW, 3>(ps.pos, o, pos);
        if (WRITE_ALL) {
          pstore<LW, 3>(ps.vel, o, vel);
          pstore<LW, 9>(ps.C, o, C);
        }
      }
      if (home) atomicAdd(bv.homed, 1);
      if (!keep) {
        atomicOr(&bv.clr[cell], 1u << r);
        atomicAdd(bv.sent, 1);
      }
    } else {
      {
        const unsigned m0 = bv.mask0[cell];
        if (r > 0 && (m0 >> r) == 1u && (m0 & ((1u << r) - 1u)) != ((1u << r) - 1u) && __popc(~m0 & bv.kmask) >= 8) {
          const int rr = nth_low_bit(~m0 & bv.kmask, atomicAdd(&bv.arrLocal[cell], 1u));
          if (rr >= 0) {
            o = particle_offset<LW>(ps.pos.chns, (bv.rowBase + (size_t)rr) * 64 + (size_t)cell);
            atomicOr(&bv.clr[cell], 1u << r);
            lowered = true;
          }
// ... 195 lines not shown
```

zpc_amd/csrc/mpm_slotblk.hip:

```cpp
#include "mpm_slot.hpp"

namespace zsr {

constexpr int SB_NG = 5;
constexpr int SB_MAXCH = 64;

struct SubGeom {
  int o[3], org[3];
};
__device__ __forceinline__ SubGeom sub_geom(const int (&borg)[3], int b) {
  SubGeom g;
  g.o[0] = ((b >> 2) & 1) * 4;
  g.o[1] = ((b >> 1) & 1) * 4;
  g.o[2] = (b & 1) * 4;
#pragma unroll
  for (int d = 0; d < 3; ++d) g.org[d] = borg[d] + g.o[d];
  return g;
}

struct BlkShared {
  float *varena, *parena, *stage;
  unsigned long long *smask;
  unsigned short (*tab)[SL_KMAX * 64];
  unsigned (*masks)[64];
  unsigned (*clr)[64];
  unsigned (*arrLocal)[64];
  unsigned (*arrCnt)[64];
  unsigned short (*arrQ)[64][SL_ARRQ];
  unsigned *xCnt;
  unsigned (*xq)[SL_XQ];
  int *nbrBlk, (*nbrBin)[27], *nbr8;
  int (*cnt)[4];
  int *oc;
  const unsigned *desc;
  unsigned *done;
  int *sums;
};

struct ChunkDesc {
  unsigned w;
  __device__ static unsigned pack(int b, int c, int qp, bool last, int total, int gbase) {
    return (unsigned)b | ((unsigned)c << 3) | ((unsigned)(qp & 1) << 7) | ((unsigned)last << 8) | ((unsigned)total << 9) | ((unsigned)gbase << 21) | (1u << 31);
  }
  __device__ int bin() const { return (int)(w & 7u); }
  __device__ int idx() const { return (int)((w >> 3) & 15u); }
  __device__ int qp() const { return (int)((w >> 7) & 1u); }
  __device__ bool last() const { return (w >> 8) & 1u; }
  __device__ int total() const { return (int)((w >> 9) & 4095u); }
  __device__ int gbase() const { return (int)((w >> 21) & 127u); }
};
template <int N> __device__ __forceinline__ void blk_chunk_descs(const unsigned *desc, int g, ChunkDesc (&d)[N]) {
#pragma unroll
  for (int k = 0; k < N; ++k) d[k].w = desc[g + k];
#pragma unroll
  for (int k = 0; k < N; ++k) d[k].w = (unsigned)__builtin_amdgcn_readfirstlane((int)d[k].w);
}

__device__ __forceinline__ void blk_build_tab(unsigned mask, int lane, int w, int nw, unsigned short *tab) {
  const unsigned long long lt = lanemask_lt();
  int total = 0;
#pragma unroll 1
  for (int r = 0; r < SL_KMAX; ++r) {
    if (__ballot((mask >> r) != 0u) == 0ull) break;
    const bool has = (mask >> r) & 1u;
    const unsigned long long occ = __ballot(has);
    if ((r % nw) == w && has) tab[total + __popcll(occ & lt)] = (unsigned short)(r * 64 + lane);
    total += __popcll(occ);
  }
}

__device__ __forceinline__ void blk_finish_bin(const BlkShared &sh, const SlotArgs &A, int bin0, int b, int qp, int lane) {
  const int bin = bin0 + b;
  const unsigned c = sh.clr[qp][lane];
  const int cv = sh.cnt[qp][lane & 3];
  if (c) A.claim[((size_t)A.nbinsAll + (size_t)bin) * 64 + lane] = c;
  sh.clr[qp][lane] = 0u;
  const int c0 = __builtin_amdgcn_readlane(cv, 0), c1 = __builtin_amdgcn_readlane(cv, 1), c2 = __builtin_amdgcn_readlane(cv, 2),
            c3 = __builtin_amdgcn_readlane(cv, 3);
  if (lane == 0) {
    const int oc = c0 < A.cap ? c0 : A.cap;
    A.moverCount[bin] = oc;
    sh.oc[b] = oc;
  }
  if (lane < 3) {
    const int add = lane == 0 ? c1 : (lane == 1 ? c2 : (c3 > 0 ? 1 << b : 0));
    if (add) atomicAdd(&sh.sums[lane], add);
  }
  if (lane < 4) sh.cnt[qp][lane] = 0;
}

struct ArenaBin8 {
  static constexpr int W = 8;
  static constexpr int SY = 8, SX = 68, CH = W * SX;
  __device__ static constexpr int at(int x, int y, int z) { return x * SX + y * SY + z; }
};

template <int CS>
__device__ __forceinline__ void blk_xlist_lds(const float *stage, const unsigned *xq, int nx, int lane, float *pa) {
  using S = ConsumerSet<CS>;
  using A8 = ArenaBin8;
  const int node = lane & 31, half = lane >> 5;
  if (nx <= 0) return;
  const StencilNodeLane sn(node);
#pragma unroll 1
  for (int k0 = 0; k0 < nx; k0 += 2) {
    const int k = k0 + half;
    const bool act = node < 27 && k < nx;
    float val[S::NA];
    int an = 0;
    if (act) {
      const unsigned e = xq[k];
      const float *st = stage + (size_t)((e & 1023u) >> 6) * (G2P2G_QF * 64) + (e & 63u);
      float Wt = 1.f;
#pragma unroll
      for (int q = 0; q < 3; ++q) Wt *= sn.weight(q, st[(1 + q) * 64]);
      an = A8::at((int)((e >> 10) & 7u) + sn.sel[0], (int)((e >> 13) & 7u) + sn.sel[1], (int)((e >> 16) & 7u) + sn.sel[2]);
#pragma unroll
      for (int q = 0; q < S::NA; ++q) val[q] = sn.value<CS>(st, Wt, q);
    }
#pragma unroll
    for (int h = 0; h < 2; ++h) {
      if (act && half == h) {
#pragma unroll
        for (int q = 0; q < S::NA; ++q) pa[q * A8::CH + an] += val[q];
      }
      __builtin_amdgcn_fence(__ATOMIC_ACQ_REL, "wavefront");
    }
  }
}

template <int SMODEL, bool WRITE_ALL>
__device__ __forceinline__ void blk_producer(const MpmDev &mp, const ParticlesDev &ps, const int (&borg)[3], int blk, int lane, int G,
                                             const BlkShared &sh, const SlotArgs &A, const int W) {
  constexpr int LW = 64;
  constexpr bool DP = model_uses_logjp(SMODEL);
  constexpr bool FLUID = model_is_fluid(SMODEL);
  const int bin0 = blk * 8;
  const unsigned kmask = A.K >= 32 ? 0xffffffffu : ((1u << A.K) - 1u);
  RecG<LW, DP, FLUID> cur, nxt;
  bool has0 = false, has1 = false;
  unsigned code0 = 0, code1 = 0;
  auto elem = [&](int b, unsigned code) { return ((size_t)(bin0 + b) * (size_t)A.K + (size_t)(code >> 6)) * 64 + (size_t)(code & 63u); };
  {
    ChunkDesc d[2];
    blk_chunk_descs(sh.desc, 0, d);
    const int b = d[1].bin();
    const int j = 64 * W + lane;
    has1 = j < d[1].total();
    if (has1) {
      code1 = sh.tab[d[1].qp()][j];
      nxt.load(ps, elem(b, code1));
    }
  }
  __syncthreads();
  for (int g = 0; g < G; ++g) {
    ChunkDesc d[3];
    blk_chunk_descs(sh.desc, g, d);
    const int b = d[1].bin();
    const int qp = d[1].qp();
    const int grp = 4 * g + W, slot = grp % SB_NG, par = g % 3;
    float *myStage = sh.stage + (size_t)slot * (G2P2G_QF * 64);
    cur = nxt;
    has0 = has1;
    code0 = code1;
    has1 = false;
    if (g + 1 < G) {
      const int b1 = d[2].bin();
      const int j1 = 256 * d[2].idx() + 64 * W + lane;
      has1 = j1 < d[2].total();
      if (has1) {
        code1 = sh.tab[d[2].qp()][j1];
        nxt.load(ps, elem(b1, code1));
      }
    }
    const SubGeom sg = sub_geom(borg, b);
    const SlotBinView bv{bin0 + b, {sg.org[0], sg.org[1], sg.org[2]}, (size_t)(bin0 + b) * (size_t)A.K, kmask,
                         sh.varena + ArenaBlk::at(sg.o[0], sg.o[1], sg.o[2]), sh.masks[b], sh.clr[qp], sh.arrLocal[b], sh.nbrBin[qp],
                         &sh.cnt[qp][0], &sh.cnt[qp][1], &sh.cnt[qp][2], &sh.cnt[qp][3], sh.arrLocal, sh.masks};
    auto ringFree = [&] {
      while (__hip_atomic_load(sh.done, __ATOMIC_RELAXED, __HIP_MEMORY_SCOPE_WORKGROUP) < 4u * (unsigned)g) __builtin_amdgcn_s_sleep(2);
      __builtin_amdgcn_fence(__ATOMIC_ACQUIRE, "workgroup");
    };
    bool valid = false;
    if (has0)
      valid = slot_produce_entry<8, SMODEL, WRITE_ALL, ArenaBlk, true>(mp, ps, cur, code0, elem(b, code0), lane, (unsigned)(slot * 64 + lane), myStage + lane, bv, A,
                                                                 sh.arrCnt[par], sh.arrQ[par], &sh.xCnt[par], sh.xq[par], ringFree);
    ringFree();
    {
      const unsigned long long vm = __ballot(valid);
      if (lane == 0) sh.smask[slot] = vm;
    }
    __syncthreads();
  }
  __syncthreads();
}

template <int CS>
__device__ __forceinline__ void blk_consumer(const MpmDev &mp, const int (&borg)[3], int blk, int lane, int G, const BlkShared &sh, const SlotArgs &A) {
  using S = ConsumerSet<CS>;
  using AL = ArenaBin8;
  constexpr int NC = 512;
  const int cx = lane >> 4, cy = (lane >> 2) & 3, cz = lane & 3;
  const unsigned long long lt = lanemask_lt();
  const float *const stage = sh.stage;
  float *const pa = sh.parena + (size_t)S::CH0 * AL::CH;
  float acc[27][S::NA];
#pragma unroll
  for (int k = 0; k < 27; ++k)
#pragma unroll
    for (int q = 0; q < S::NA; ++q) acc[k][q] = 0.f;
  unsigned mask = 0u;
  int r = 0, off = 0;
  __syncthreads();
  auto binState = [&](int g, const ChunkDesc &c2, const ChunkDesc &c3) {
    if (g + 3 < G && c3.idx() == 0) blk_build_tab(sh.masks[c3.bin()][lane], lane, CS, 4, sh.tab[c3.qp()]);
    if (CS == 2 && g >= 0 && g + 2 < G && c2.idx() == 0 && lane < 27) sh.nbrBin[c2.qp()][lane] = neighbour_bin8(sh.nbrBlk, blk, c2.bin(), lane);
  };
  {
    ChunkDesc d[5];
    blk_chunk_descs(sh.desc, -1 + 1, d);
    binState(-1, d[2], d[3]);
  }
  for (int g = 0; g < G; ++g) {
    __syncthreads();
    ChunkDesc d[5];
    blk_chunk_descs(sh.desc, g, d);
    const int b = d[1].bin(), c = d[1].idx(), total = d[1].total(), par = g % 3;
    const int gb = 4 * d[1].gbase();
    if (c == 0) {
      r = 0;
      off = 0;
      mask = sh.masks[b][lane];
      for (int k = lane; k < S::NA * AL::CH; k += 64) pa[k] = 0.f;
      __builtin_amdgcn_fence(__ATOMIC_ACQ_REL, "wavefront");
    }
    const int produced = 256 * (c + 1) < total ? 256 * (c + 1) : total;
    const unsigned qn = sh.arrCnt[par][lane];
    const int na = qn < (unsigned)SL_ARRQ ? (int)qn : SL_ARRQ;
    int ai = 0;
    if (CS == 0) sh.arrCnt[(g + 2) % 3][lane] = 0u;
#pragma unroll 1
    for (;;) {
      bool roundOk = false, has = false;
      unsigned long long occ = 0ull;
      int cnt = 0;
      if (off < total) {
        has = (mask >> r) & 1u;
        occ = __ballot(has);
        cnt = __popcll(occ);
        roundOk = off + cnt <= produced;
      }
      const bool pend = ai < na;
      if (!roundOk && __ballot(pend) == 0ull) break;
      int spos = -1;
      if (roundOk) {
        if (has) {
          const int e = off + __popcll(occ & lt);
          const int slot = (gb + (e >> 6)) % SB_NG, pos = e & 63;
          if ((sh.smask[slot] >> pos) & 1ull) spos = slot * (G2P2G_QF * 64) + pos;
        }
        off += cnt;
        ++r;
      }
      if (spos < 0 && pend) {
        const unsigned p = sh.arrQ[par][lane][ai++];
        spos = (int)(p >> 6) * (G2P2G_QF * 64) + (int)(p & 63u);
      }
      if (spos >= 0) g2p2g_consume_set<CS>(mp, stage, spos, acc);
    }
    {
      const int nx = sh.xCnt[par] < (unsigned)SL_XQ ? (int)sh.xCnt[par] : SL_XQ;
      if (CS == 0 && lane == 0) sh.xCnt[(g + 2) % 3] = 0u;
      blk_xlist_lds<CS>(stage, sh.xq[par], nx, lane, pa);
    }
    __builtin_amdgcn_fence(__ATOMIC_RELEASE, "workgroup");
    if (lane == 0) atomicAdd(sh.done, 1u);
    binState(g, d[3], d[4]);
    if (CS == 3 && d[1].last()) blk_finish_bin(sh, A, blk * 8, b, d[1].qp(), lane);
    if (d[1].last()) {
      acc_to_arena<AL, true>(pa + AL::at(cx + 1, cy + 1, cz + 1), acc);
      const SubGeom sg = sub_geom(borg, b);
      for (int n = lane; n < 512; n += 64) {
        const int x = n >> 6, y = (n >> 3) & 7, z = n & 7;
        const int g[3] = {sg.o[0] - 1 + x, sg.o[1] - 1 + y, sg.o[2] - 1 + z};
        const int code = ((g[0] < 0 ? 0 : (g[0] >= 8 ? 2 : 1)) * 3 + (g[1] < 0 ? 0 : (g[1] >= 8 ? 2 : 1))) * 3 + (g[2] < 0 ? 0 : (g[2] >= 8 ? 2 : 1));
        const int bn = sh.nbrBlk[code];
        const float *a = pa + AL::at(x, y, z);
        if (bn >= 0) {
          float *gq = A.gridB + ((size_t)bn * 7 + S::CH0) * NC + (((g[0] & 7) * 8 + (g[1] & 7)) * 8 + (g[2] & 7));
#pragma unroll
          for (int q = 0; q < S::NA; ++q) {
            const float v = a[q * AL::CH];
            if (v != 0.f) unsafeAtomicAdd(gq + q * NC, v);
          }
        } else if (S::MASS && a[0] != 0.f) {
          A.status[2] = 1;
        }
      }
      __builtin_amdgcn_fence(__ATOMIC_ACQ_REL, "wavefront");
    }
  }
  __syncthreads();
}

template <int SMODEL, bool WRITE_ALL>
static __global__ __launch_bounds__(512, 4) void g2p2g_slotblk_kernel(MpmDev mp, ParticlesDev ps, BhtDev t, SlotArgs A) {
  constexpr int NC = 512;
  __shared__ float s_varena[3 * ArenaBlk::CH];
  __shared__ float s_parena[7 * ArenaBin8::CH];
  __shared__ float s_stage[SB_NG * G2P2G_QF * 64];
  __shared__ unsigned long long s_smask[SB_NG];
  __shared__ unsigned short s_tab[2][SL_KMAX * 64];
  __shared__ unsigned s_masks[8][64];
  __shared__ unsigned s_clr[2][64], s_arrLocal[8][64], s_arrCnt[3][64];
  __shared__ unsigned short s_arrQ[3][64][SL_ARRQ];
  __shared__ unsigned s_xCnt[3], s_xq[3][SL_XQ];
  __shared__ int s_nbrBlk[27], s_nbrBin[2][27], s_nbr8[8];
  __shared__ int s_cnt[2][4];
  __shared__ int s_total[8], s_gbase[8], s_nch[8], s_binQ[8], s_oc[8];
  __shared__ unsigned char s_chBin[SB_MAXCH], s_chIdx[SB_MAXCH];
  __shared__ unsigned s_desc[SB_MAXCH + 5];
  __shared__ unsigned s_done;
  __shared__ int s_sums[3], s_G;
  const BlkShared sh{s_varena, s_parena, s_stage, s_smask, s_tab, s_masks, s_clr, s_arrLocal, s_arrCnt, s_arrQ, s_xCnt, s_xq, s_nbrBlk, s_nbrBin, s_nbr8,
                     s_cnt, s_oc, s_desc, &s_done, s_sums};
  const int tid = threadIdx.x, lane = tid & 63, w = tid >> 6;
  const int blk = (int)blockIdx.x + A.binBase / 8;
  const int bin0 = blk * 8;
  const unsigned mask = A.cellMask[(size_t)(bin0 + w) * 64 + lane];
  s_masks[w][lane] = mask;
  s_arrLocal[w][lane] = 0u;
  {
    int n = __popc(mask);
#pragma unroll
    for (int sft = 32; sft >= 1; sft >>= 1) n += __shfl_xor(n, sft, 64);
    if (lane == 0) s_total[w] = n;
  }
  if (tid < 128) s_clr[tid >> 6][tid & 63] = 0u;
  if (tid < 192) s_arrCnt[tid >> 6][tid & 63] = 0u;
  if (tid < 3) {
    s_xCnt[tid] = 0u;
    s_sums[tid] = 0;
  }
  if (tid < 8) (&s_cnt[0][0])[tid] = 0;
  if (tid == 0) s_done = 0u;
  if (tid >= 64 && tid < 64 + 27) s_nbrBlk[tid - 64] = A.nbr27[(size_t)blk * 27 + (tid - 64)];
  if (tid >= 96 && tid < 104) s_nbr8[tid - 96] = A.nbr[(size_t)blk * 8 + (tid - 96)];
  int borg[3];
#pragma unroll
  for (int d = 0; d < 3; ++d) borg[d] = t.activeKeys[3 * (size_t)blk + d] * (8 / mp.kscale);
  __syncthreads();
  if ((s_total[0] | s_total[1] | s_total[2] | s_total[3] | s_total[4] | s_total[5] | s_total[6] | s_total[7]) == 0) {
    if (tid < 8) A.moverCount[bin0 + tid] = 0;
    if (A.signal && blk < A.signalBlocks && tid == 0) atomicAdd(A.signal, 1ull);
    return;
  }
  if (tid == 0) {
    int G = 0, q = 0;
    for (int b = 0; b < 8; ++b) {
      const int nch = (s_total[b] + 255) >> 8;
      s_nch[b] = nch;
      s_gbase[b] = G;
      s_binQ[b] = q;
      s_oc[b] = 0;
      if (nch) ++q;
      for (int c = 0; c < nch; ++c) {
        s_chBin[G] = (unsigned char)b;
        s_chIdx[G] = (unsigned char)c;
        s_desc[G + 1] = ChunkDesc::pack(b, c, s_binQ[b], c == nch - 1, s_total[b], s_gbase[b]);
        ++G;
      }
    }
    s_desc[0] = 0u;
    for (int k = G + 1; k < G + 5; ++k) s_desc[k] = 0u;
    s_G = G;
    if (G && A.blockEdge && A.blockEdge[blk]) A.status[3] = 1;
  }
  for (int n = tid; n < 1000; n += 512) {
    const int x = n / 100, y = (n / 10) % 10, z = n % 10;
    const int slot = ((x >= 8) << 2) | ((y >= 8) << 1) | (z >= 8);
    const int cell = ((x & 7) * 8 + (y & 7)) * 8 + (z & 7);
    const int bn = s_nbr8[slot];
    float *a = s_varena + ArenaBlk::at(x, y, z);
    const float *g = A.gridA + ((size_t)(bn < 0 ? 0 : bn) * 7 + 1) * NC + cell;
#pragma unroll
    for (int ch = 0; ch < 3; ++ch) a[ch * ArenaBlk::CH] = bn >= 0 ? g[ch * NC] : 0.f;
  }
  __syncthreads();
  const int G = s_G;
  if (tid < 8 && s_total[tid] == 0) A.moverCount[bin0 + tid] = 0;
  {
    const int b0 = s_chBin[0];
    blk_build_tab(s_masks[b0][lane], lane, w, 8, s_tab[s_binQ[b0] & 1]);
    if (tid < 27) s_nbrBin[s_binQ[b0] & 1][tid] = neighbour_bin8(s_nbrBlk, blk, b0, tid);
    if (G > 1 && s_chIdx[1] == 0) {
      const int b1 = s_chBin[1];
      blk_build_tab(s_masks[b1][lane], lane, w, 8, s_tab[s_binQ[b1] & 1]);
      if (tid >= 64 && tid < 64 + 27) s_nbrBin[s_binQ[b1] & 1][tid - 64] = neighbour_bin8(s_nbrBlk, blk, b1, tid - 64);
    }
  }
  __syncthreads();
  if (w < 4) blk_producer<SMODEL, WRITE_ALL>(mp, ps, borg, blk, lane, G, sh, A, __builtin_amdgcn_readfirstlane(w));
  else {
    if (w == 4) blk_consumer<0>(mp, borg, blk, lane, G, sh, A);
    else if (w == 5) blk_consumer<1>(mp, borg, blk, lane, G, sh, A);
    else if (w == 6) blk_consumer<2>(mp, borg, blk, lane, G, sh, A);
    else blk_consumer<3>(mp, borg, blk, lane, G, sh, A);
  }
  __syncthreads();
  {
    const unsigned nl = s_arrLocal[w][lane];
    if (nl) A.claim[(size_t)(bin0 + w) * 64 + lane] = nl << 16;
  }
  if (tid == 0) {
    if (s_sums[0]) atomicAdd(&A.status[SL_SENT + (blk & (SL_NCTR - 1))], s_sums[0]);
    if (s_sums[1]) atomicAdd(&A.status[SL_DELIVERED + (blk & (SL_NCTR - 1))], s_sums[1]);
  }
  if (s_sums[2]) {
    asm volatile("s_waitcnt vmcnt(0)" ::: "memory");
    __syncthreads();
    constexpr int RB = SB_NG * G2P2G_QF * 64 / SL_REC;
    for (int b = 0; b < 8; ++b) {
      if (!((s_sums[2] >> b) & 1)) continue;
      const SubGeom sg = sub_geom(borg, b);
      const int oc = s_oc[b];
      for (int j0 = 0; j0 < oc; j0 += RB) {
        const int nb = oc - j0 < RB ? oc - j0 : RB;
        const float *src = A.moverRec + ((size_t)(bin0 + b) * A.cap + (size_t)j0) * SL_REC;
        for (int k = tid; k < nb * SL_REC; k += 512) s_stage[k] = __hip_atomic_load(src + k, __ATOMIC_RELAXED, __HIP_MEMORY_SCOPE_AGENT);
        __syncthreads();
        outbox_scatter_global<8>(mp, sg, s_stage, nb, w, lane, s_nbrBlk, A.gridB, A.status);
        __syncthreads();
      }
    }
  }
  if (A.signal && blk < A.signalBlocks) {
    asm volatile("s_waitcnt vmcnt(0)" ::: "memory");
    __syncthreads();
    if (tid == 0) atomicAdd(A.signal, 1ull);
  }
}

template <int M, bool WA> static void launch_blk(hipStream_t stream, unsigned nblk, const MpmDev &mp, const ParticlesDev &pd, const BhtDev &t, const SlotArgs &A) {
  hipLaunchKernelGGL((g2p2g_slotblk_kernel<M, WA>), dim3(nblk), dim3(512), 0, stream, mp, pd, t, A);
}

void launch_g2p2g_slotblk(hipStream_t stream, int model, bool writeAll, const MpmDev &mp, const ParticlesDev &pd, const BhtDev &t, const SlotArgs &A) {
  const unsigned nblk = (unsigned)(A.nbins / 8);
  if (!nblk) return;
#define CALL_BLK(SS, M)                                            \
  do {                                                             \
    if (writeAll) launch_blk<M, true>(stream, nblk, mp, pd, t, A); \
    else launch_blk<M, false>(stream, nblk, mp, pd, t, A);         \
  } while (0)
  ZSR_DISPATCH_PURE_(8, model, CALL_BLK)
#undef CALL_BLK
}

}
```

zpc_amd/csrc/mpm_slotted.hip:

```cpp
#include "mpm_slot.hpp"

namespace zsr {

void exclusive_scan_u32(Launch &L, const unsigned *in, size_t n, unsigned *out);

template <int SIDE>
static __global__ __launch_bounds__(256) void slot_assign_kernel(BhtDev t, Port<float> pos, size_t n, float dx, unsigned *cellCount, int K,
                                                                 int *srcOf, int *status, int kscale) {
  size_t i = (size_t)blockIdx.x * blockDim.x + threadIdx.x;
  if (i >= n) return;
  float p[3];
  load_attr<3>(pos, i, p);
  int key[3], loc[3];
#pragma unroll
  for (int d = 0; d < 3; ++d) {
    const int c = (int)floorf(p[d] * (1.0f / dx) - 0.5f);
    loc[d] = c & (SIDE - 1);
    key[d] = (c - loc[d]) / SIDE * kscale;
  }
  const int b = bht_query<3>(t, key);
  if (b < 0) {
    status[2] = 1;
    return;
  }
  const int sub = SIDE == 4 ? 0 : (((loc[0] >> 2) * 2 + (loc[1] >> 2)) * 2 + (loc[2] >> 2));
  const unsigned bin = (unsigned)b * bins_per_block<SIDE>() + sub;
  const unsigned lane = (unsigned)(((loc[0] & 3) * 4 + (loc[1] & 3)) * 4 + (loc[2] & 3));
  const unsigned r = atomicAdd(&cellCount[bin * 64u + lane], 1u);
  if (r >= (unsigned)K) {
    status[1] = 1;
    return;
  }
  srcOf[((size_t)bin * K + r) * 64 + lane] = (int)i;
}
static __global__ __launch_bounds__(256) void slot_mask_kernel(unsigned *cellCountToMask, size_t ncells, int K) {
  size_t c = (size_t)blockIdx.x * blockDim.x + threadIdx.x;
  if (c >= ncells) return;
  unsigned n = cellCountToMask[c];
  if (n > (unsigned)K) n = (unsigned)K;
  cellCountToMask[c] = n >= 32u ? 0xffffffffu : ((1u << n) - 1u);
}
static __global__ __launch_bounds__(256) void slot_gather_kernel(const float *src, float *dst, size_t nslots, int C, const int *srcOf) {
  size_t s = (size_t)blockIdx.x * blockDim.x + threadIdx.x;
  if (s >= nslots) return;
  const int i = srcOf[s];
  float *d = dst + (s >> 6) * (size_t)C * 64 + (s & 63);
  if (i < 0) {
    for (int c = 0; c < C; ++c) d[(size_t)c * 64] = 0.f;
    return;
  }
  const float *q = src + ((size_t)i >> 6) * (size_t)C * 64 + ((size_t)i & 63);
  for (int c = 0; c < C; ++c) d[(size_t)c * 64] = q[(size_t)c * 64];
}
static __global__ __launch_bounds__(256) void slot_popc_kernel(const unsigned *cellMask, size_t ncells, unsigned *cnt) {
  size_t c = (size_t)blockIdx.x * blockDim.x + threadIdx.x;
  if (c < ncells) cnt[c] = (unsigned)__popc(cellMask[c]);
}
static __global__ __launch_bounds__(256) void slot_emit_kernel(const unsigned *cellMask, const unsigned *start, size_t ncells, int K, int *slots) {
  size_t c = (size_t)blockIdx.x * blockDim.x + threadIdx.x;
  if (c >= ncells) return;
  unsigned m = cellMask[c], o = start[c];
  const size_t bin = c >> 6, lane = c & 63;
  while (m) {
    const int r = __ffs((int)m) - 1;
    m &= m - 1;
    slots[o++] = (int)((bin * (size_t)K + (size_t)r) * 64 + lane);
  }
}
static __global__ __launch_bounds__(256) void build_neighbors27_kernel(BhtDev t, int nblocks, int *nbr27, int kscale) {
  size_t g = (size_t)blockIdx.x * blockDim.x + threadIdx.x;
  if (g >= (size_t)nblocks * 27) return;
  const int i = (int)(g / 27), o = (int)(g % 27);
  int k[3] = {t.activeKeys[3 * (size_t)i] + (o / 9 - 1) * kscale, t.activeKeys[3 * (size_t)i + 1] + ((o / 3) % 3 - 1) * kscale,
              t.activeKeys[3 * (size_t)i + 2] + (o % 3 - 1) * kscale};
  nbr27[g] = bht_query<3>(t, k);
}

static __global__ __launch_bounds__(256) void partition_edge_kernel(BhtDev t, int nblocks, unsigned char *edge, int kscale, int lo, int hi) {
  const int i = (int)(blockIdx.x * blockDim.x + threadIdx.x);
  if (i >= nblocks) return;
  const int k0[3] = {t.activeKeys[3 * (size_t)i], t.activeKeys[3 * (size_t)i + 1], t.activeKeys[3 * (size_t)i + 2]};
  int missing = 0;
  for (int a = lo; a <= hi; ++a)
    for (int b = lo; b <= hi; ++b)
      for (int c = lo; c <= hi; ++c) {
        int k[3] = {k0[0] + a * kscale, k0[1] + b * kscale, k0[2] + c * kscale};
        missing |= bht_query<3>(t, k) < 0;
      }
  edge[i] = (unsigned char)missing;
}

template <int SIDE, int SMODEL, bool WRITE_ALL>
static __global__ __launch_bounds__(512, 4) void g2p2g_slot_kernel(MpmDev mp, ParticlesDev ps, BhtDev t, SlotArgs A) {
  using AL = ArenaLds;
  static_assert(SIDE == 4, "one workgroup per bin serves 4^3 blocks (bin == block); 8^3 blocks run g2p2g_slotblk_kernel");
  __shared__ float s_varena[3 * AL::CH];
  __shared__ float s_stage[SL_NG * G2P2G_QF * 64];
  float *const s_parena = s_stage;
  __shared__ unsigned long long s_smask[SL_NG];
  __shared__ unsigned short s_tab[SL_KMAX * 64];
  __shared__ unsigned s_mask0[64], s_clr[64], s_arrLocal[64], s_arrCnt[3][64];
  __shared__ unsigned short s_arrQ[3][64][SL_ARRQ];
  __shared__ int s_nbrBlk[27], s_nbrBin[27];
  __shared__ unsigned s_xCnt[3], s_xq[3][SL_XQ];
  __shared__ int s_outCount, s_sent, s_homed, s_xOver;
  const SlotShared sh{s_varena, s_parena, s_stage, s_smask, s_tab, s_mask0, s_clr, s_arrLocal, s_nbrBlk, s_nbrBin, s_arrCnt, s_arrQ,
                      s_xCnt, s_xq, &s_outCount, &s_sent, &s_homed, &s_xOver};
  const int tid = threadIdx.x, lane = tid & 63, w = tid >> 6;
  const int bin = (int)blockIdx.x + A.binBase;
  const unsigned mask = A.cellMask[(size_t)bin * 64 + lane];
  unsigned any = mask;
#pragma unroll
  for (int sft = 32; sft >= 1; sft >>= 1) any |= (unsigned)__shfl_xor((int)any, sft, 64);
  if (any == 0u) {
    if (tid == 0) A.moverCount[bin] = 0;
    return;
  }
  const int nrounds = 32 - __clz((int)any);
  int total = 0;
  {
    const unsigned long long lt = lanemask_lt();
    for (int r = 0; r < nrounds; ++r) {
      const bool has = (mask >> r) & 1u;
      const unsigned long long occ = __ballot(has);
      if ((r & 7) == w && has) s_tab[total + __popcll(occ & lt)] = (unsigned short)(r * 64 + lane);
      total += __popcll(occ);
    }
  }
  const int nchunks = (total + 255) >> 8;
  if (tid < 64) {
    s_mask0[tid] = mask;
    s_clr[tid] = 0u;
    s_arrLocal[tid] = 0u;
    s_arrCnt[0][tid] = s_arrCnt[1][tid] = s_arrCnt[2][tid] = 0u;
  }
  if (tid == 0) s_outCount = s_sent = s_homed = s_xOver = 0;
  if (tid < 3) s_xCnt[tid] = 0u;
  const BinGeom<SIDE> geo(t, bin, mp.kscale);
  if (tid == 0 && A.blockEdge && A.blockEdge[geo.block]) A.status[3] = 1;
  if (tid >= 64 && tid < 64 + 27) {
    const int code = tid - 64;
    const int nb = A.nbr27[(size_t)geo.block * 27 + code];
    s_nbrBlk[code] = nb;
    s_nbrBin[code] = code == 13 ? bin : nb;
  }
  __syncthreads();
  if (w == 0) g2p2g_slot_producer<SIDE, SMODEL, WRITE_ALL, 0>(mp, ps, geo, bin, total, lane, nchunks, sh, A);
  else if (w == 1) g2p2g_slot_producer<SIDE, SMODEL, WRITE_ALL, 1>(mp, ps, geo, bin, total, lane, nchunks, sh, A);
  else if (w == 2) g2p2g_slot_producer<SIDE, SMODEL, WRITE_ALL, 2>(mp, ps, geo, bin, total, lane, nchunks, sh, A);
  else if (w == 3) g2p2g_slot_producer<SIDE, SMODEL, WRITE_ALL, 3>(mp, ps, geo, bin, total, lane, nchunks, sh, A);
  else {
    if (w == 4) g2p2g_slot_consumer<SIDE, 0>(mp, geo, mask, total, lane, nchunks, sh, A);
    else if (w == 5) g2p2g_slot_consumer<SIDE, 1>(mp, geo, mask, total, lane, nchunks, sh, A);
    else if (w == 6) g2p2g_slot_consumer<SIDE, 2>(mp, geo, mask, total, lane, nchunks, sh, A);
    else g2p2g_slot_consumer<SIDE, 3>(mp, geo, mask, total, lane, nchunks, sh, A);
  }
  __syncthreads();
  if (tid < 64) {
    const unsigned c = s_clr[tid], nl = s_arrLocal[tid];
    if (c) A.claim[((size_t)A.nbinsAll + (size_t)bin) * 64 + tid] = c;
    if (nl) A.claim[(size_t)bin * 64 + tid] = nl << 16;
  }
  if (tid == 0) {
    A.moverCount[bin] = s_outCount < A.cap ? s_outCount : A.cap;
    if (s_sent) atomicAdd(&A.status[SL_SENT + (bin & (SL_NCTR - 1))], s_sent);
    if (s_homed) atomicAdd(&A.status[SL_DELIVERED + (bin & (SL_NCTR - 1))], s_homed);
  }
  arena_flush_to_grid<SIDE>(geo, A.nbr, s_parena, A.gridB, &A.status[2], tid);
  if (s_xOver > 0) {
    asm volatile("s_waitcnt vmcnt(0)" ::: "memory");
    __syncthreads();
    const int oc = s_outCount < A.cap ? s_outCount : A.cap;
    constexpr int RB = SL_NG * G2P2G_QF * 64 / SL_REC;
    for (int j0 = 0; j0 < oc; j0 += RB) {
      const int nb = oc - j0 < RB ? oc - j0 : RB;
      const float *src = A.moverRec + ((size_t)bin * A.cap + (size_t)j0) * SL_REC;
      for (int k = tid; k < nb * SL_REC; k += 512) s_stage[k] = __hip_atomic_load(src + k, __ATOMIC_RELAXED, __HIP_MEMORY_SCOPE_AGENT);
      __syncthreads();
      outbox_scatter_global<SIDE>(mp, geo, s_stage, nb, w, lane, s_nbrBlk, A.gridB, A.status);
      __syncthreads();
    }
  }
}

template <bool FLUID, bool DP, bool WRITE_ALL>
static __global__ __launch_bounds__(256) void slot_rehome_kernel(ParticlesDev ps, const unsigned *cellMask, unsigned *claim, const int *moverCount,
                                                                 const float *moverRec, int cap, size_t nbins, int K, int *status) {
  constexpr int LW = 64;
  const size_t bin = ((size_t)blockIdx.x * 4 + (threadIdx.x >> 6)) * 8 + ((threadIdx.x & 63) >> 3);
  const int n = bin < nbins ? moverCount[bin] : 0;
  if (__ballot(n > 0) == 0ull) return;
  const unsigned kmask = K >= 32 ? 0xffffffffu : ((1u << K) - 1u);
  int nhomed = 0;
  for (int k = (int)(threadIdx.x & 7); k < n; k += 8) {
    const float *rc = moverRec + (bin * (size_t)cap + (size_t)k) * SL_REC;
    const float4 r0 = reinterpret_cast<const float4 *>(rc)[0], r1 = reinterpret_cast<const float4 *>(rc)[1],
                 r2 = reinterpret_cast<const float4 *>(rc)[2], r3 = reinterpret_cast<const float4 *>(rc)[3];
    const unsigned dcell = __float_as_uint(r3.z);
    if (dcell == 0xffffffffu) continue;
    const unsigned occ = cellMask[dcell];
    const unsigned old = atomicAdd(&claim[dcell], 1u);
    const int rr = nth_low_bit(~occ & kmask, (old >> 16) + (old & 0xffffu));
    size_t i;
    if (rr >= 0) {
      i = ((size_t)(dcell >> 6) * (size_t)K + (size_t)rr) * 64 + (size_t)(dcell & 63u);
    } else {
      status[1] = 1;
      const unsigned src = __float_as_uint(r3.w) >> 1;
      i = (bin * (size_t)K + (size_t)(src >> 6)) * 64 + (size_t)(src & 63u);
      atomicAnd(&claim[(nbins + bin) * 64 + (size_t)(src & 63u)], ~(1u << (src >> 6)));
    }
    ++nhomed;
    const POff<LW> o = particle_offset<LW>(ps.pos.chns, i);
    const float x[3] = {r0.y, r0.z, r0.w};
    const float F[9] = {r1.x, r1.y, r1.z, r1.w, r2.x, r2.y, r2.z, r2.w, r3.x};
    pstore1<LW>(ps.mass, o, r0.x);
    pstore<LW, 3>(ps.pos, o, x);
    pstore_state<LW, FLUID>(ps.F, o, F);
    if constexpr (DP) pstore1<LW>(ps.logJp, o, r3.y);
    if constexpr (WRITE_ALL) {
      float v[3], C[9], PF[9];
#pragma unroll
      for (int d = 0; d < 3; ++d) v[d] = rc[SLR_V + d];
#pragma unroll
      for (int d = 0; d < 9; ++d) {
        C[d] = rc[SLR_C + d];
        PF[d] = rc[SLR_PF + d];
      }
      pstore<LW, 3>(ps.vel, o, v);
      pstore<LW, 9>(ps.C, o, C);
      {
        float S[STRESS_N];
        stress_pack(PF, S);
        pstore<LW, STRESS_N>(ps.stress, o, S);
      }
    }
  }
#pragma unroll
  for (int sft = 32; sft >= 1; sft >>= 1) nhomed += __shfl_xor(nhomed, sft, 64);
  if ((threadIdx.x & 63) == 0 && nhomed) atomicAdd(&status[SL_DELIVERED + (int)((bin >> 3) & (SL_NCTR - 1))], nhomed);
}

static __global__ __launch_bounds__(256) void slot_commit_kernel(unsigned *cellMask, unsigned *claim, size_t ncells, int K) {
  const size_t c = (size_t)blockIdx.x * blockDim.x + threadIdx.x;
  if (c >= ncells) return;
  const unsigned tk = claim[c], clr = claim[ncells + c];
  if (!tk && !clr) return;
  const unsigned m0 = cellMask[c];
  const unsigned kmask = K >= 32 ? 0xffffffffu : ((1u << K) - 1u);
  const unsigned n = (tk >> 16) + (tk & 0xffffu);
  unsigned rest = ~m0 & kmask, bits = 0u;
  for (unsigned k = 0; k < n && rest; ++k) {
    const unsigned b = rest & (0u - rest);
    bits |= b;
    rest ^= b;
  }
  cellMask[c] = (m0 & ~clr) | bits;
  claim[c] = 0u;
  claim[ncells + c] = 0u;
}

template <int SIDE>
static __global__ __launch_bounds__(256) void slot_sparsity_kernel(BhtDev oldT, const unsigned *cellMask, size_t ncells, int kscale, BhtDev newT) {
  const size_t c = (size_t)blockIdx.x * blockDim.x + threadIdx.x;
  const bool valid = c < ncells && cellMask[c] != 0u;
  int b[3] = {0, 0, 0};
  if (valid) {
    const size_t bin = c >> 6;
    const int lane = (int)(c & 63), blk = (int)(bin / bins_per_block<SIDE>()), sub = (int)(bin % bins_per_block<SIDE>());
    const int o[3] = {SIDE == 4 ? 0 : ((sub >> 2) & 1) * 4, SIDE == 4 ? 0 : ((sub >> 1) & 1) * 4, SIDE == 4 ? 0 : (sub & 1) * 4};
    const int l[3] = {lane >> 4, (lane >> 2) & 3, lane & 3};
#pragma unroll
    for (int d = 0; d < 3; ++d) b[d] = floordiv(oldT.activeKeys[3 * (size_t)blk + d] * (SIDE / kscale) + o[d] + l[d] - 1, SIDE) * kscale;
  }
  const int px = shfl_up(b[0], 1), py = shfl_up(b[1], 1), pz = shfl_up(b[2], 1);
  const bool pvalid = shfl_up((int)valid, 1) != 0;
  const bool dup = lane_id() != 0 && pvalid && px == b[0] && py == b[1] && pz == b[2];
  if (valid && !dup) bht_insert<3>(newT, b);
}
static __global__ __launch_bounds__(256) void reslot_map_kernel(BhtDev oldT, int nOld, BhtDev newT, int *map) {
  const int i = (int)(blockIdx.x * blockDim.x + threadIdx.x);
  if (i >= nOld) return;
  const int k[3] = {oldT.activeKeys[3 * (size_t)i], oldT.activeKeys[3 * (size_t)i + 1], oldT.activeKeys[3 * (size_t)i + 2]};
  map[i] = bht_query<3>(newT, k);
}
static __global__ __launch_bounds__(256) void reslot_move_kernel(const int *map, int bpb, int K, int C, const float4 *oldBuf, float4 *newBuf,
                                                                 const unsigned *oldMask, unsigned *newMask, int *status) {
  const size_t bin = blockIdx.x;
  __shared__ unsigned sAny;
  if (threadIdx.x == 0) sAny = 0u;
  __syncthreads();
  const unsigned m = threadIdx.x < 64 ? oldMask[bin * 64 + threadIdx.x] : 0u;
  if (m) atomicOr(&sAny, m);
  __syncthreads();
  const unsigned any = sAny;
  if (!any) return;
  const int nb = map[bin / bpb];
  if (nb < 0) {
    if (threadIdx.x == 0) status[2] = 1;
    return;
  }
  const size_t nbin = (size_t)nb * bpb + bin % bpb;
  if (threadIdx.x < 64) newMask[nbin * 64 + threadIdx.x] = m;
  const int rounds = 32 - __clz((int)any);
  const size_t per = (size_t)K * C * 16, cnt = (size_t)rounds * C * 16;
  const float4 *src = oldBuf + bin * per;
  float4 *dst = newBuf + nbin * per;
  for (size_t i = threadIdx.x; i < cnt; i += 256) dst[i] = src[i];
}
static __global__ __launch_bounds__(256) void reslot_grid_kernel(const int *map, int nOld, int blockFloats4, const float4 *oldGrid, float4 *newGrid) {
  const int b = blockIdx.x;
  const int nb = map[b];
  if (nb < 0) return;
  for (int i = threadIdx.x; i < blockFloats4; i += 256) newGrid[(size_t)nb * blockFloats4 + i] = oldGrid[(size_t)b * blockFloats4 + i];
}

}

using namespace zsr;

extern "C" {

size_t zs_rocm_mpm_slot_outbox_bytes(size_t nbins, int cap, int which) {
  if (which == 0) return nbins * sizeof(int);
  if (which == 1) return 2 * nbins * 64 * sizeof(unsigned);
  return nbins * (size_t)cap * (size_t)SL_REC * sizeof(float);
}

void zs_rocm_mpm_build_neighbors27(zs_rocm_policy *pol, const zs_rocm_bht_3 *tab, int *nbr27, int keyStride) {
  Launch L(pol, "build_neighbors27");
  const int nb = bht_size(tab->t, L.stream);
  if (!nb) return;
  hipLaunchKernelGGL(build_neighbors27_kernel, dim3(ceil_div((size_t)nb * 27, 256)), dim3(256), 0, L.stream, tab->t.dev(), nb, nbr27,
                     keyStride > 0 ? keyStride : 1);
}

int zs_rocm_mpm_slot_particles(zs_rocm_policy *pol, const zs_rocm_bht_3 *tab, zs_rocm_attr pos, size_t n, float dx, int side, int keyIsOrigin,
                               int K, const float *src, float *dst, int C, unsigned *cellMask, int *status) {
  if (K < 1 || K > 32 || (side != 4 && side != 8) || pos.tileMask != 63u) return -1;
  Launch L(pol, "slot_particles");
  const int nb = bht_size(tab->t, L.stream);
  if (nb == 0) return 0;
  const size_t nbins = (size_t)nb * (side == 4 ? 1 : 8), ncells = nbins * 64, nslots = nbins * (size_t)K * 64;
  int *srcOf = (int *)L.temp(sizeof(int) * nslots);
  ZSR_CHECK(hipMemsetAsync(srcOf, 0xff, sizeof(int) * nslots, L.stream));
  ZSR_CHECK(hipMemsetAsync(cellMask, 0, sizeof(unsigned) * ncells, L.stream));
  BhtDev t = tab->t.dev();
  Port<float> pp = make_port<float>(pos);
  if (n) {
    if (side == 4)
      hipLaunchKernelGGL((slot_assign_kernel<4>), dim3(ceil_div(n, 256)), dim3(256), 0, L.stream, t, pp, n, dx, cellMask, K, srcOf, status, keyIsOrigin ? side : 1);
    else
      hipLaunchKernelGGL((slot_assign_kernel<8>), dim3(ceil_div(n, 256)), dim3(256), 0, L.stream, t, pp, n, dx, cellMask, K, srcOf, status, keyIsOrigin ? side : 1);
  }
  hipLaunchKernelGGL(slot_mask_kernel, dim3(ceil_div(ncells, 256)), dim3(256), 0, L.stream, cellMask, ncells, K);
  hipLaunchKernelGGL(slot_gather_kernel, dim3(ceil_div(nslots, 256)), dim3(256), 0, L.stream, src, dst, nslots, C, (const int *)srcOf);
  return 0;
}

size_t zs_rocm_mpm_slot_list(zs_rocm_policy *pol, const unsigned *cellMask, size_t nbins, int K, int *slots) {
  Launch L(pol, "slot_list");
  const size_t ncells = nbins * 64;
  if (!ncells) return 0;
  unsigned *cnt = (unsigned *)L.temp(sizeof(unsigned) * (ncells + 1)), *start = (unsigned *)L.temp(sizeof(unsigned) * (ncells + 1));
  ZSR_CHECK(hipMemsetAsync(cnt + ncells, 0, sizeof(unsigned), L.stream));
  hipLaunchKernelGGL(slot_popc_kernel, dim3(ceil_div(ncells, 256)), dim3(256), 0, L.stream, cellMask, ncells, cnt);
  exclusive_scan_u32(L, cnt, ncells + 1, start);
  unsigned total = 0;
  ZSR_CHECK(hipMemcpyAsync(&total, start + ncells, sizeof(unsigned), hipMemcpyDeviceToHost, L.stream));
  if (slots) hipLaunchKernelGGL(slot_emit_kernel, dim3(ceil_div(ncells, 256)), dim3(256), 0, L.stream, cellMask, (const unsigned *)start, ncells, K, slots);
  ZSR_CHECK(hipStreamSynchronize(L.stream));
  return (size_t)total;
}

int zs_rocm_mpm_g2p2g_slots(zs_rocm_policy *pol, const zs_rocm_mpm_params *p, zs_rocm_particles ps, const zs_rocm_bht_3 *tab,
                            const float *gridA, float *gridB, size_t nblocks, const zs_rocm_slot_storage *st, int writeAll,
                            size_t blockBegin, size_t blockEnd, int finish) {
  return zsr::mpm_g2p2g_slots_signal(pol, p, ps, tab, gridA, gridB, nblocks, st, writeAll, blockBegin, blockEnd, finish, nullptr, 0);
}
}
namespace zsr {
int mpm_g2p2g_slots_signal(zs_rocm_policy *pol, const zs_rocm_mpm_params *p, zs_rocm_particles ps, const zs_rocm_bht_3 *tab, const float *gridA,
                           float *gridB, size_t nblocks, const zs_rocm_slot_storage *st, int writeAll, size_t blockBegin, size_t blockEnd, int finish,
                           unsigned long long *signal, size_t signalBlocks) {
  if (!st) return -1;
  if (signal && p->side != 8) return -1;
  unsigned *const cellMask = st->cellMask;
  const int K = st->K, outboxCap = st->outboxCap;
  const int *const nbr = st->nbr, *const nbr27 = st->nbr27;
  int *const moverCount = st->moverCount, *const status = st->status;
  unsigned *const claim = st->claim;
  float *const moverRec = st->moverRec;
  if (!nblocks) return 0;
  if (!cellMask || !nbr || !nbr27 || !moverCount || !claim || !moverRec || !status || K < 1 || K > 32 || outboxCap < 1 || outboxCap > (1 << 20)) return -1;
  if (p->model < ZS_MPM_FIXED_COROTATED || p->model > ZS_MPM_EQUATION_OF_STATE) return -1;
  if (uniform_lane_width(ps, model_uses_logjp(p->model), writeAll != 0) != 64 || (writeAll && (!ps.vel.base || !ps.C.base))) {
    fprintf(stderr, "[zs_rocm] g2p2g_slotted needs all particle attributes in one TileVector<f32, 64>\n");
    return -1;
  }
  if (blockEnd > nblocks) blockEnd = nblocks;
  Launch L(pol, "G2P2GTransfer(slotted)");
  MpmDev mp = make_dev(p);
  ParticlesDev pd = make_particles(ps);
  BhtDev t = tab->t.dev();
  const unsigned bpb = p->side == 4 ? 1u : 8u;
  const unsigned nbinsAll = (unsigned)(nblocks * bpb);
  const unsigned nbins = blockBegin < blockEnd ? (unsigned)((blockEnd - blockBegin) * bpb) : 0u;
  const SlotArgs A{gridA, gridB, cellMask, K, nbr, nbr27, moverCount, claim, moverRec, status, (int)(blockBegin * bpb), (int)nbins, (int)nbinsAll, outboxCap,
                   st->blockEdge, signal, (int)signalBlocks};
#define CALL_REHOME3(M, WA)                                                                                                              \
  hipLaunchKernelGGL((slot_rehome_kernel<model_is_fluid(M), model_uses_logjp(M), WA>), dim3(ceil_div((size_t)nbinsAll, 32)), dim3(256), 0,  \
                     L.stream, pd, (const unsigned *)cellMask, claim, (const int *)moverCount, (const float *)moverRec, outboxCap,        \
                     (size_t)nbinsAll, K, status)
#define CALL_REHOME(SS, M)                      \
  do {                                          \
    if (writeAll) { CALL_REHOME3(M, true); }    \
    else { CALL_REHOME3(M, false); }            \
  } while (0)
  if (p->side == 8) {
    if (nbins) launch_g2p2g_slotblk(L.stream, p->model, writeAll != 0, mp, pd, t, A);
  } else if (nbins) {
#define CALL_SLOT4(SS, M)                                                                                                  \
  do {                                                                                                                     \
    if (writeAll) hipLaunchKernelGGL((g2p2g_slot_kernel<4, M, true>), dim3(nbins), dim3(512), 0, L.stream, mp, pd, t, A);  \
    else hipLaunchKernelGGL((g2p2g_slot_kernel<4, M, false>), dim3(nbins), dim3(512), 0, L.stream, mp, pd, t, A);          \
  } while (0)
    ZSR_DISPATCH_PURE_(4, p->model, CALL_SLOT4)
  }
  if (finish) ZSR_DISPATCH_PURE_(0, p->model, CALL_REHOME)
  if (finish) {
    const size_t ncells = (size_t)nbinsAll * 64;
    hipLaunchKernelGGL(slot_commit_kernel, dim3(ceil_div(ncells, 256)), dim3(256), 0, L.stream, cellMask, claim, ncells, K);
  }
  return 0;
}
}
extern "C" {

int zs_rocm_mpm_g2p2g_slotted_range(zs_rocm_policy *pol, const zs_rocm_mpm_params *p, zs_rocm_particles ps, const zs_rocm_bht_3 *tab,
                                    const float *gridA, float *gridB, size_t nblocks, unsigned *cellMask, int K, const int *nbr, const int *nbr27,
                                    int *moverCount, unsigned *claim, float *moverRec, int outboxCap, int writeAll, int *status,
                                    size_t blockBegin, size_t blockEnd, int finish) {
  const zs_rocm_slot_storage st{cellMask, K, nbr, nbr27, moverCount, claim, moverRec, outboxCap, status, nullptr};
  return zs_rocm_mpm_g2p2g_slots(pol, p, ps, tab, gridA, gridB, nblocks, &st, writeAll, blockBegin, blockEnd, finish);
}

int zs_rocm_mpm_g2p2g_slotted(zs_rocm_policy *pol, const zs_rocm_mpm_params *p, zs_rocm_particles ps, const zs_rocm_bht_3 *tab, const float *gridA,
                              float *gridB, size_t nblocks, unsigned *cellMask, int K, const int *nbr, const int *nbr27, int *moverCount,
                              unsigned *claim, float *moverRec, int outboxCap, int writeAll, int *status) {
  return zs_rocm_mpm_g2p2g_slotted_range(pol, p, ps, tab, gridA, gridB, nblocks, cellMask, K, nbr, nbr27, moverCount, claim, moverRec, outboxCap,
                                         writeAll, status, 0, nblocks, 1);
}

void zs_rocm_mpm_partition_edge(zs_rocm_policy *pol, const zs_rocm_bht_3 *tab, unsigned char *edge, int keyStride, int lo, int hi) {
  Launch L(pol, "partition_edge");
  const int nb = bht_size(tab->t, L.stream);
  if (!nb) return;
  hipLaunchKernelGGL(partition_edge_kernel, dim3(ceil_div((size_t)nb, 256)), dim3(256), 0, L.stream, tab->t.dev(), nb, edge,
                     keyStride > 0 ? keyStride : 1, lo, hi);
}

void zs_rocm_mpm_slot_compute_sparsity(zs_rocm_policy *pol, const zs_rocm_bht_3 *oldTab, const unsigned *cellMask, size_t nblocksOld, int side,
                                       int keyIsOrigin, zs_rocm_bht_3 *newTab) {
  Launch L(pol, "slot_compute_sparsity");
  if (!nblocksOld || (side != 4 && side != 8)) return;
  const size_t ncells = nblocksOld * (side == 4 ? 1 : 8) * 64;
  if (side == 4)
    hipLaunchKernelGGL((slot_sparsity_kernel<4>), dim3(ceil_div(ncells, 256)), dim3(256), 0, L.stream, oldTab->t.dev(), cellMask, ncells, keyIsOrigin ? side : 1, newTab->t.dev());
  else
    hipLaunchKernelGGL((slot_sparsity_kernel<8>), dim3(ceil_div(ncells, 256)), dim3(256), 0, L.stream, oldTab->t.dev(), cellMask, ncells, keyIsOrigin ? side : 1, newTab->t.dev());
}
int zs_rocm_mpm_reslot(zs_rocm_policy *pol, const zs_rocm_bht_3 *oldTab, const zs_rocm_bht_3 *newTab, int side, int K, int C, const float *oldBuf,
                       float *newBuf, const unsigned *oldMask, unsigned *newMask, const float *oldGrid, float *newGrid, int *status) {
  if ((side != 4 && side != 8) || K < 1 || K > 32 || C < 1 || !oldBuf || !newBuf || !oldMask || !newMask || !status) return -1;
  Launch L(pol, "reslot");
  const int nOld = bht_size(oldTab->t, L.stream), nNew = bht_size(newTab->t, L.stream);
  if (!nOld || !nNew) return 0;
  const int bpb = side == 4 ? 1 : 8;
  int *map = (int *)L.temp(sizeof(int) * (size_t)nOld);
  hipLaunchKernelGGL(reslot_map_kernel, dim3(ceil_div((size_t)nOld, 256)), dim3(256), 0, L.stream, oldTab->t.dev(), nOld, newTab->t.dev(), map);
  ZSR_CHECK(hipMemsetAsync(newMask, 0, sizeof(unsigned) * (size_t)nNew * bpb * 64, L.stream));
  hipLaunchKernelGGL(reslot_move_kernel, dim3((unsigned)((size_t)nOld * bpb)), dim3(256), 0, L.stream, (const int *)map, bpb, K, C,
                     reinterpret_cast<const float4 *>(oldBuf), reinterpret_cast<float4 *>(newBuf), oldMask, newMask, status);
  if (oldGrid && newGrid) {
    const size_t bf = (size_t)7 * side * side * side;
    ZSR_CHECK(hipMemsetAsync(newGrid, 0, sizeof(float) * bf * (size_t)nNew, L.stream));
    hipLaunchKernelGGL(reslot_grid_kernel, dim3((unsigned)nOld), dim3(256), 0, L.stream, (const int *)map, nOld, (int)(bf / 4),
                       reinterpret_cast<const float4 *>(oldGrid), reinterpret_cast<float4 *>(newGrid));
  }
  return 0;
}

}
```

zpc_amd/mpm.py:

```python
import ctypes as C

import torch

from ._lib import lib, Port, Particles, MpmParams, SlotStorage, MpmStep
from .containers import Bht

FIXED_COROTATED, DRUCKER_PRAGER, VONMISES_FIXED_COROTATED, NACC = 0, 1, 2, 3
EQUATION_OF_STATE = 4
HAS_LOGJP = (DRUCKER_PRAGER, NACC)


class MpmTransfer:
    def __init__(self, pol, n, dx, dt, model=FIXED_COROTATED, side=4, lane_width=64, E=5e4, nu=0.4, volume=1.0,
                 cohesion=0.0, beta=1.0, yield_surface=0.816496580927726 * 2.0 * 0.5 / (3.0 - 0.5), vol_correction=True,
                 device="cuda", key_is_origin=False, aos=False, cache_stress=False, yield_stress=240e6, xi=0.8, friction_angle=45.0,
                 hardening=True, bulk=4e4, viscosity=0.0):
        self.pol, self.n, self.L, self.side = pol, int(n), int(lane_width), int(side)
        self.device = torch.device(device)
        self.model = model
        self.fluid = model == EQUATION_OF_STATE
        self.nF = 1 if self.fluid else 9
        self.nchn = 16 + self.nF + (1 if model in HAS_LOGJP else 0)
        self.off = {"m": 0, "x": 1, "v": 4, "C": 7, "F": 16, "logJp": 25}
        self.cache_stress = bool(cache_stress)
        if self.cache_stress and lib().zs_rocm_mpm_stress_channels() != 6:
            raise RuntimeError("libzsrocm expects %d channels in particles.stress, this mirror allocates 6" % lib().zs_rocm_mpm_stress_channels())
        if self.cache_stress:
            self.off["PF"] = self.nchn
            self.nchn += 6
        self.aos = bool(aos)
        if self.aos:
            self.L = 1
        self.tiles = (self.n + self.L - 1) // self.L
        self.buf = torch.zeros(self.tiles * self.L * self.nchn, dtype=torch.float32, device=self.device)
        self.buf2 = None
        self.drift_flag = None
        self.drift_tripped = False
        self.outside_tripped = False
        self.key_is_origin = bool(key_is_origin)
        self.kstride = side if key_is_origin else 1
        self.params = MpmParams(model, dx, dt, volume, E, nu, cohesion, beta, yield_surface, int(vol_correction), side,
                                int(self.key_is_origin), yield_stress, xi, lib().zs_rocm_nacc_msqr(friction_angle), int(hardening),
                                bulk, viscosity)
        self.table = None
        self.grid = None
        self.nblocks = 0
        self.order = self.bin_start = self.cell_count = self.nbr = None
        self.binned = False
        self.slotted = False
        self.n_slots = 0
        self.K = 0
        self.slot_record = {"sent": 0, "homed": 0, "flags": [0] * 5, "periods": 0, "edge_periods": 0, "log": []}

    def _zero(self, t):
        lib().zs_rocm_memset(self.pol.handle, t.data_ptr(), 0, t.numel() * t.element_size())

    def _port(self, name, buf=None):
        buf = self.buf if buf is None else buf
        bits = self.L.bit_length() - 1
        return Port(buf.data_ptr() + self.off[name] * self.L * 4, 0, bits, self.L - 1, self.nchn)

    def particles(self, buf=None):
        null = Port(None, 0, 0, 0, 1)
        return Particles(self._port("m", buf), self._port("x", buf), self._port("v", buf), self._port("C", buf), self._port("F", buf),
                         self._port("logJp", buf) if self.model in HAS_LOGJP else null,
                         self._port("PF", buf) if self.cache_stress else null, self.n_slots if self.slotted else self.n)

    def set_particles(self, buf, n):
        self.n = int(n)
        self.tiles = (self.n + self.L - 1) // self.L
        assert buf.numel() == self.tiles * self.L * self.nchn
        self.buf, self.buf2 = buf, None
        self.order = self.bin_start = self.cell_count = None
        self.binned = False

    def update_stress(self):
        lib().zs_rocm_mpm_update_stress(self.pol.handle, C.byref(self.params), self.particles())

    def upload(self, mass, pos, vel, Cm, F, logJp=None):
        cols = [torch.as_tensor(mass, dtype=torch.float32).reshape(self.n, 1), torch.as_tensor(pos, dtype=torch.float32).reshape(self.n, 3),
                torch.as_tensor(vel, dtype=torch.float32).reshape(self.n, 3), torch.as_tensor(Cm, dtype=torch.float32).reshape(self.n, 9),
                torch.as_tensor(F, dtype=torch.float32).reshape(self.n, self.nF)]
        if self.model in HAS_LOGJP:
            lj = torch.zeros(self.n) if logJp is None else torch.as_tensor(logJp, dtype=torch.float32)
            cols.append(lj.reshape(self.n, 1))
        if self.cache_stress:
            cols.append(torch.zeros(self.n, 6))
        aos = torch.cat([c.to(self.device) for c in cols], dim=1).contiguous()
        lib().zs_rocm_tv_from_aos_f32(self.pol.handle, aos.data_ptr(), self.n, self.nchn, self.L, self.buf.data_ptr())
        self.pol.syncCtx()
        self.binned = False

    def download(self):
        buf = self.buf
        if self.slotted:
            buf, cnt = self._compact_copy()
            assert cnt == self.n, "slotted storage holds %d particles, expected %d" % (cnt, self.n)
        aos = torch.empty(self.n, self.nchn, dtype=torch.float32, device=self.device)
        lib().zs_rocm_tv_to_aos_f32(self.pol.handle, buf.data_ptr(), self.n, self.nchn, self.L, aos.data_ptr())
        self.pol.syncCtx()
        a = aos.cpu().numpy()
        out = {"m": a[:, 0].copy(), "x": a[:, 1:4].copy(), "v": a[:, 4:7].copy(), "C": a[:, 7:16].copy(),
               "J" if self.fluid else "F": a[:, 16:16 + self.nF].copy()}
        if self.model in HAS_LOGJP:
            out["logJp"] = a[:, 25].copy()
        return out

    def build_partition(self, expected_blocks, margin=0, order=None, axes=None):
        order = order or "holders_lex"
        if order not in ("insertion", "holders_lex", "lex", "morton"):
            raise ValueError(f"build_partition: unknown block order {order!r}")
        self.table = Bht(3, int(expected_blocks))
        L = lib()
        L.zs_rocm_mpm_compute_sparsity(self.pol.handle, self.table.handle, self._port("x"), self.n, self.params.dx, self.side,
                                       int(self.key_is_origin))
        n_holders = 0
        if order == "holders_lex":
            self.pol.syncCtx()
            self.table.canonicalize(self.pol, axes)
            self.pol.syncCtx()
            n_holders = self.table.size()
        m = int(margin)
        self.partition_margin = m
        lo, hi = (C.c_int * 3)(-m, -m, -m), (C.c_int * 3)(2 + m, 2 + m, 2 + m)
        L.zs_rocm_mpm_enlarge_sparsity(self.pol.handle, self.table.handle, lo, hi, self.kstride)
        self.pol.syncCtx()
        if order == "holders_lex":
            self.table.canonicalize(self.pol, axes, first=n_holders)
            self.pol.syncCtx()
        if order == "morton":
            self.table.order_morton(self.pol)
            self.pol.syncCtx()
        elif order == "lex":
            self.table.canonicalize(self.pol, axes)
            self.pol.syncCtx()
        self.block_order, self.block_axes = order, (tuple(axes) if axes is not None else None)
        self.nblocks = self.table.size()
        self.slotted = False
        nc = self.side ** 3
        self.grid = torch.zeros(self.nblocks * 7 * nc, dtype=torch.float32, device=self.device)
        self.nbr = torch.empty(self.nblocks * 8, dtype=torch.int32, device=self.device)
        L.zs_rocm_mpm_build_neighbors(self.pol.handle, self.table.handle, self.nbr.data_ptr(), self.kstride)
        self.binned = False
        return self.nblocks

    def adopt_partition(self, active_keys_ptr, nblocks):
        L = lib()
        self.table = Bht(3, int(nblocks))
        self.table.assign(self.pol, active_keys_ptr, int(nblocks))
        self.nblocks = int(nblocks)
        nc = self.side ** 3
        self.grid = torch.zeros(self.nblocks * 7 * nc, dtype=torch.float32, device=self.device)
        self.nbr = torch.empty(self.nblocks * 8, dtype=torch.int32, device=self.device)
        L.zs_rocm_mpm_build_neighbors(self.pol.handle, self.table.handle, self.nbr.data_ptr(), self.kstride)
        self.binned = False
        return self.nblocks

    def rebin(self, inputs_only=False):
        L = lib()
        if self.order is None or self.order.numel() != self.n:
            self.order = torch.empty(self.n, dtype=torch.int32, device=self.device)
        self.nbins = self.nblocks * (self.side // 4) ** 3
        self.bin_start = torch.empty(self.nbins + 1, dtype=torch.int32, device=self.device)
        self.cell_count = torch.empty(self.nbins * 64, dtype=torch.int32, device=self.device)
        L.zs_rocm_mpm_bin_particles(self.pol.handle, self.table.handle, self._port("x"), self.n, self.params.dx, self.side,
                                    int(self.key_is_origin), self.order.data_ptr(), self.bin_start.data_ptr(), self.cell_count.data_ptr())
        if self.buf2 is None:
            self.buf2 = torch.empty_like(self.buf)
        if inputs_only:
            mask = 0xF | (((1 << self.nF) - 1) << self.off["F"]) | ((1 << self.off["logJp"]) if self.model in HAS_LOGJP else 0)
            L.zs_rocm_tv_gather_channels_f32(self.pol.handle, self.buf.data_ptr(), self.buf2.data_ptr(), self.n, self.nchn, self.L,
                                             self.order.data_ptr(), mask)
        else:
            L.zs_rocm_tv_gather_f32(self.pol.handle, self.buf.data_ptr(), self.buf2.data_ptr(), self.n, self.nchn, self.L,
                                    self.order.data_ptr())
        self.pol.syncCtx()
        self.buf, self.buf2 = self.buf2, self.buf
        self.binned = True
        if self.drift_flag is not None:
            flags = self.drift_flag.cpu()
            self.drift_tripped = self.drift_tripped or bool(flags[0])
            self.outside_tripped = self.outside_tripped or bool(flags[2])
            self._zero(self.drift_flag)

    SLOT_FLAG_NAMES = ["outbox full", "a cell is full (K)", "mass or a mover for a block outside the partition",
                       "early warning: a particle lives next to the partition's edge", "a particle was not stored under its cell"]

    def slot(self, K=24, outbox_cap=128):
        assert self.L == 64 and not self.aos and self.table is not None and not self.slotted
        L = lib()
        self.K = int(K)
        self.outbox_cap = int(outbox_cap)
        self.nbins = self.nblocks * (self.side // 4) ** 3
        self.n_slots = self.nbins * self.K * 64
        sbuf = torch.empty(self.nbins * self.K * 64 * self.nchn, dtype=torch.float32, device=self.device)
        self.cell_mask = torch.empty(self.nbins * 64, dtype=torch.int32, device=self.device)
        self.slot_status = torch.zeros(8 + 2 * 256, dtype=torch.int32, device=self.device)
        self.nbr27 = torch.empty(self.nblocks * 27, dtype=torch.int32, device=self.device)
        L.zs_rocm_mpm_build_neighbors27(self.pol.handle, self.table.handle, self.nbr27.data_ptr(), self.kstride)
        self.block_edge = torch.empty(max(self.nblocks, 1), dtype=torch.uint8, device=self.device)
        L.zs_rocm_mpm_partition_edge(self.pol.handle, self.table.handle, self.block_edge.data_ptr(), self.kstride, -1, 2)
        rc = L.zs_rocm_mpm_slot_particles(self.pol.handle, self.table.handle, self._port("x"), self.n, self.params.dx, self.side,
                                          int(self.key_is_origin), self.K, self.buf.data_ptr(), sbuf.data_ptr(), self.nchn,
                                          self.cell_mask.data_ptr(), self.slot_status.data_ptr())
        if rc != 0:
            raise RuntimeError("zs_rocm_mpm_slot_particles refused its arguments")
        self.mover_count = torch.zeros(L.zs_rocm_mpm_slot_outbox_bytes(self.nbins, self.outbox_cap, 0) // 4, dtype=torch.int32, device=self.device)
        self.mover_dest = torch.zeros(L.zs_rocm_mpm_slot_outbox_bytes(self.nbins, self.outbox_cap, 1) // 4, dtype=torch.int32, device=self.device)
        self.mover_rec = torch.empty(L.zs_rocm_mpm_slot_outbox_bytes(self.nbins, self.outbox_cap, 2) // 4, dtype=torch.float32, device=self.device)
        self.pol.syncCtx()
        st = self.slot_status.cpu().numpy()
        if st[1] or st[2]:
            raise RuntimeError("slot(): %s" % ("a cell holds more than K = %d particles" % self.K if st[1] else "particles outside the partition"))
        self.buf, self.buf2 = sbuf, None
        self.slotted, self.binned = True, False
        self.order = self.bin_start = self.cell_count = None
        self._edge_host = self._edge_event = None
        self.slot_storage = SlotStorage(self.cell_mask.data_ptr(), self.K, self.nbr.data_ptr(), self.nbr27.data_ptr(), self.mover_count.data_ptr(),
                                        self.mover_dest.data_ptr(), self.mover_rec.data_ptr(), self.outbox_cap, self.slot_status.data_ptr(),
                                        self.block_edge.data_ptr())

    def _backing(self, name, numel, dtype, zero=False, spare=False):
        pool = self.__dict__.setdefault("_pool", {})
        t = pool.get(name)
        if t is None or t.numel() < numel or t.dtype != dtype:
            t = torch.empty(int(numel * (1.25 if spare else 1.0)) + 64, dtype=dtype, device=self.device)
            pool[name] = t
        v = t[:numel]
        if zero:
            self._zero(v)
        return v

    def reserve_repartition_buffers(self, growth=1.25):
        assert self.slotted
        n = int(self.buf.numel() * growth)
        pool = self.__dict__.setdefault("_pool", {})
        if "slots_alt" not in pool or pool["slots_alt"].numel() < n:
            pool["slots_alt"] = torch.empty(n, dtype=torch.float32, device=self.device)
        self.pol.syncCtx()

    def repartition_slotted(self, margin=None, strict=True):
        assert self.slotted and self.L == 64
        L = lib()
        self.check_slots(strict=strict)
        old_table, old_nblocks = self.table, self.nblocks
        m = int(getattr(self, "partition_margin", 0) if margin is None else margin)
        new_table = Bht(3, max(2 * int(old_nblocks) + 64, 4096))
        L.zs_rocm_mpm_slot_compute_sparsity(self.pol.handle, old_table.handle, self.cell_mask.data_ptr(), old_nblocks, self.side,
                                            int(self.key_is_origin), new_table.handle)
        if getattr(self, "block_order", "insertion") == "holders_lex":
            self.pol.syncCtx()
            new_table.canonicalize(self.pol, getattr(self, "block_axes", None))
            self.pol.syncCtx()
            n_holders = new_table.size()
        lo, hi = (C.c_int * 3)(-m, -m, -m), (C.c_int * 3)(2 + m, 2 + m, 2 + m)
        L.zs_rocm_mpm_enlarge_sparsity(self.pol.handle, new_table.handle, lo, hi, self.kstride)
        self.pol.syncCtx()
        if getattr(self, "block_order", "insertion") == "holders_lex":
            new_table.canonicalize(self.pol, getattr(self, "block_axes", None), first=n_holders)
            self.pol.syncCtx()
        nb = new_table.size()
        if not new_table.success() or nb == 0:
            raise RuntimeError("repartition_slotted: the new partition did not fit its table (%d blocks, capacity for %d)"
                               % (nb, max(2 * int(old_nblocks) + 64, 4096)))
        bpb = (self.side // 4) ** 3
        nbins = nb * bpb
        nc = self.side ** 3
        pool = self.__dict__.setdefault("_pool", {})
        need = nbins * self.K * 64 * self.nchn
        alt = pool.get("slots_alt")
        if alt is None or alt.numel() < need:
            alt = torch.empty(int(need * 1.1), dtype=torch.float32, device=self.device)
        sbuf = alt[:need]
        old_store = self.buf._base if self.buf._base is not None else self.buf
        flip = self.__dict__.get("_flip", 0) ^ 1
        self._flip = flip
        mask = self._backing("mask%d" % flip, nbins * 64, torch.int32)
        grid = self._backing("grid%d" % flip, nb * 7 * nc, torch.float32)
        if L.zs_rocm_mpm_reslot(self.pol.handle, old_table.handle, new_table.handle, self.side, self.K, self.nchn, self.buf.data_ptr(),
                                sbuf.data_ptr(), self.cell_mask.data_ptr(), mask.data_ptr(), self.grid.data_ptr(), grid.data_ptr(),
                                self.slot_status.data_ptr()) != 0:
            raise RuntimeError("zs_rocm_mpm_reslot refused its arguments")
        self.pol.syncCtx()
        pool["slots_cur"], pool["slots_alt"] = alt, old_store
        self.table, self.nblocks, self.nbins, self.n_slots = new_table, nb, nbins, nbins * self.K * 64
        self.buf, self.cell_mask, self.grid = sbuf, mask, grid
        self.grid2 = self._backing("gridB%d" % flip, nb * 7 * nc, torch.float32, zero=True)
        self.nbr = self._backing("nbr", nb * 8, torch.int32, spare=True)
        L.zs_rocm_mpm_build_neighbors(self.pol.handle, self.table.handle, self.nbr.data_ptr(), self.kstride)
        self.nbr27 = self._backing("nbr27", nb * 27, torch.int32, spare=True)
        L.zs_rocm_mpm_build_neighbors27(self.pol.handle, self.table.handle, self.nbr27.data_ptr(), self.kstride)
        self.block_edge = self._backing("edge", max(nb, 1), torch.uint8, spare=True)
        L.zs_rocm_mpm_partition_edge(self.pol.handle, self.table.handle, self.block_edge.data_ptr(), self.kstride, -1, 2)
        self.mover_count = self._backing("mcount", L.zs_rocm_mpm_slot_outbox_bytes(nbins, self.outbox_cap, 0) // 4, torch.int32, zero=True, spare=True)
        self.mover_dest = self._backing("mdest", L.zs_rocm_mpm_slot_outbox_bytes(nbins, self.outbox_cap, 1) // 4, torch.int32, zero=True, spare=True)
        self.mover_rec = self._backing("mrec", L.zs_rocm_mpm_slot_outbox_bytes(nbins, self.outbox_cap, 2) // 4, torch.float32, spare=True)
        self._edge_host = self._edge_event = None
        self.slot_storage = SlotStorage(self.cell_mask.data_ptr(), self.K, self.nbr.data_ptr(), self.nbr27.data_ptr(), self.mover_count.data_ptr(),
                                        self.mover_dest.data_ptr(), self.mover_rec.data_ptr(), self.outbox_cap, self.slot_status.data_ptr(),
                                        self.block_edge.data_ptr())
        self.pol.syncCtx()
        if int(self.slot_status[2].item()):
            raise RuntimeError("repartition_slotted: a populated block is missing from the new partition")
        return nb

    def _compact_copy(self):
        L = lib()
        slots = torch.empty(self.n_slots, dtype=torch.int32, device=self.device)
        cnt = int(L.zs_rocm_mpm_slot_list(self.pol.handle, self.cell_mask.data_ptr(), self.nbins, self.K, slots.data_ptr()))
        tiles = (cnt + 63) // 64
        out = torch.zeros(max(tiles, 1) * 64 * self.nchn, dtype=torch.float32, device=self.device)
        if cnt:
            L.zs_rocm_tv_gather_f32(self.pol.handle, self.buf.data_ptr(), out.data_ptr(), cnt, self.nchn, 64, slots.data_ptr())
        self.pol.syncCtx()
        return out, cnt

    def unslot(self, strict=True):
        assert self.slotted
        self.check_slots(strict=strict)
        out, cnt = self._compact_copy()
        if cnt != self.n:
            raise RuntimeError("slotted storage holds %d particles, %d went in: particles were lost" % (cnt, self.n))
        self.slotted = False
        self.tiles = (cnt + 63) // 64
        self.buf, self.buf2 = out, None
        self.binned = False

    def check_slots(self, strict=True):
        self.pol.syncCtx()
        st = [int(v) for v in self.slot_status.cpu().numpy()]
        st[5], st[6] = sum(st[8:264]), sum(st[264:520])
        self._zero(self.slot_status)
        rec = self.slot_record
        rec["sent"] += st[5]
        rec["homed"] += st[6]
        rec["periods"] += 1
        rec["edge_periods"] += int(bool(st[3]))
        for k in range(5):
            rec["flags"][k] += int(bool(st[k]))
        bad = [self.SLOT_FLAG_NAMES[k] for k in (0, 1, 2, 4) if st[k]]
        if st[5] != st[6]:
            bad.append("%d movers sent, %d re-homed" % (st[5], st[6]))
        if bad:
            rec["log"].append((rec["periods"], bad))
            if strict:
                raise RuntimeError("slotted G2P2G: " + "; ".join(bad))
        return st[:8]

    def poll_repartition(self, reduce=None):
        ready = False
        if self._edge_event is not None:
            self._edge_event.synchronize()
            ready = bool(self._edge_host[:5].any())
        if self._edge_host is None:
            self._edge_host = torch.zeros(8, dtype=torch.float32).pin_memory()
            self._edge_event = torch.cuda.Event()
        sp = self.pol.getStream()
        with torch.cuda.stream(torch.cuda.ExternalStream(sp) if sp else torch.cuda.default_stream(self.device)):
            w = self.slot_status[:8].float()
            if reduce is not None:
                reduce(w)
            self._edge_host.copy_(w, non_blocking=True)
            self._edge_event.record()
        return ready

    def repartition_requested(self):
        w = self.slot_status[:5].cpu()
        return bool(w.any())

    def clear_grid(self):
        self._zero(self.grid)

    def p2g(self, binned=None):
        binned = self.binned if binned is None else binned
        bs = self.bin_start.data_ptr() if binned else None
        cc = self.cell_count.data_ptr() if binned else None
        nb = self.nbr.data_ptr() if binned else None
        lib().zs_rocm_mpm_p2g(self.pol.handle, C.byref(self.params), self.particles(), self.table.handle, self.grid.data_ptr(),
                              self.nblocks, bs, cc, nb)

    def grid_update(self, extf=(0.0, 0.0, 0.0), max_vel=None):
        e = (C.c_float * 3)(*extf)
        lib().zs_rocm_mpm_grid_update(self.pol.handle, C.byref(self.params), self.grid.data_ptr(), self.nblocks, e,
                                      max_vel.data_ptr() if max_vel is not None else None)

    def apply_boundary(self, collider, levelset=None):
        tr = _transition_view(levelset)
        if tr is not None:
            if lib().zs_rocm_mpm_apply_boundary_transition(self.pol.handle, C.byref(self.params), self.table.handle, self.grid.data_ptr(),
                                                           self.nblocks, C.byref(collider), C.byref(tr)) != 0:
                raise RuntimeError("zs_rocm_mpm_apply_boundary_transition refused its arguments")
            return
        if levelset is not None:
            if lib().zs_rocm_mpm_apply_boundary_levelset(self.pol.handle, C.byref(self.params), self.table.handle, self.grid.data_ptr(),
                                                         self.nblocks, C.byref(collider), C.byref(_levelset_view(levelset))) != 0:
                raise RuntimeError("zs_rocm_mpm_apply_boundary_levelset refused its arguments")
            return
        lib().zs_rocm_mpm_apply_boundary(self.pol.handle, C.byref(self.params), self.table.handle, self.grid.data_ptr(), self.nblocks,
                                         C.byref(collider))

    def g2p(self, binned=None):
        binned = self.binned if binned is None else binned
        bs = self.bin_start.data_ptr() if binned else None
        cc = self.cell_count.data_ptr() if binned else None
        nb = self.nbr.data_ptr() if binned else None
        lib().zs_rocm_mpm_g2p(self.pol.handle, C.byref(self.params), self.particles(), self.table.handle, self.grid.data_ptr(),
                              self.nblocks, bs, cc, nb)

    def dof_vector(self):
        return torch.zeros(self.nblocks * self.side ** 3, 3, dtype=torch.float32, device=self.device)

    def _bins(self, binned):
        binned = self.binned if binned is None else binned
        if self.slotted:
            raise RuntimeError("the implicit operators read compact storage: unslot() first")
        if binned:
            return self.bin_start.data_ptr(), self.cell_count.data_ptr(), self.nbr.data_ptr()
        return None, None, None

    def _check_dof(self, *vs):
        for v in vs:
            if v.dtype != torch.float32 or not v.is_contiguous() or v.numel() != self.nblocks * self.side ** 3 * 3:
                raise ValueError("a dof vector is a contiguous float32 tensor of nblocks * side^3 * 3 entries (dof_vector())")

    def implicit_force(self, v, out, trial=None, binned=None):
        self._check_dof(v, out)
        if trial is not None and (trial.dtype != torch.float32 or not trial.is_contiguous() or trial.numel() != self.n * 27):
            raise ValueError("trial: contiguous float32 [n, 27]")
        bs, cc, nb = self._bins(binned)
        if lib().zs_rocm_mpm_implicit_force(self.pol.handle, C.byref(self.params), self.particles(), self.table.handle, self.nblocks, bs, cc,
                                            nb, v.data_ptr(), out.data_ptr(), trial.data_ptr() if trial is not None else None) != 0:
            raise RuntimeError("zs_rocm_mpm_implicit_force refused its arguments")

    def implicit_multiply(self, v, out, binned=None):
        self._check_dof(v, out)
        bs, cc, nb = self._bins(binned)
        if lib().zs_rocm_mpm_implicit_multiply(self.pol.handle, C.byref(self.params), self.particles(), self.table.handle,
                                               self.grid.data_ptr(), self.nblocks, bs, cc, nb, v.data_ptr(), out.data_ptr()) != 0:
            raise RuntimeError("zs_rocm_mpm_implicit_multiply refused its arguments")

    def implicit_project(self, collider, inout, levelset=None):
        self._check_dof(inout)
        tr = _transition_view(levelset)
        if tr is not None:
            if lib().zs_rocm_mpm_implicit_project_transition(self.pol.handle, C.byref(self.params), self.table.handle, self.grid.data_ptr(),
                                                             self.nblocks, C.byref(collider) if collider is not None else None,
                                                             C.byref(tr), inout.data_ptr()) != 0:
                raise RuntimeError("zs_rocm_mpm_implicit_project_transition refused its arguments")
            return
        if levelset is not None:
            if lib().zs_rocm_mpm_implicit_project_levelset(self.pol.handle, C.byref(self.params), self.table.handle, self.grid.data_ptr(),
                                                           self.nblocks, C.byref(collider) if collider is not None else None,
                                                           C.byref(_levelset_view(levelset)), inout.data_ptr()) != 0:
                raise RuntimeError("zs_rocm_mpm_implicit_project_levelset refused its arguments")
            return
        if lib().zs_rocm_mpm_implicit_project(self.pol.handle, C.byref(self.params), self.table.handle, self.grid.data_ptr(), self.nblocks,
                                              C.byref(collider) if collider is not None else None, inout.data_ptr()) != 0:
            raise RuntimeError("zs_rocm_mpm_implicit_project refused its arguments")

    def implicit_precondition(self, v, out):
        self._check_dof(v, out)
        if lib().zs_rocm_mpm_implicit_precondition(self.pol.handle, self.grid.data_ptr(), self.nblocks, self.side, v.data_ptr(),
                                                   out.data_ptr()) != 0:
            raise RuntimeError("zs_rocm_mpm_implicit_precondition refused its arguments")

    def implicit_solve(self, b, x, max_iters=1000, tol=1e-6, rel_tol=0.5, collider=None, binned=None, levelset=None):
        self._check_dof(b, x)
        bs, cc, nb = self._bins(binned)
        it = C.c_int(0)
        tr = _transition_view(levelset)
        if tr is not None:
            if lib().zs_rocm_mpm_implicit_solve_transition(self.pol.handle, C.byref(self.params), self.particles(), self.table.handle,
                                                           self.grid.data_ptr(), self.nblocks, bs, cc, nb,
                                                           C.byref(collider) if collider is not None else None, C.byref(tr),
                                                           b.data_ptr(), x.data_ptr(), int(max_iters), float(tol), float(rel_tol), C.byref(it)) != 0:
                raise RuntimeError("zs_rocm_mpm_implicit_solve_transition refused its arguments")
            return it.value
        if levelset is not None:
            if lib().zs_rocm_mpm_implicit_solve_levelset(self.pol.handle, C.byref(self.params), self.particles(), self.table.handle,
                                                         self.grid.data_ptr(), self.nblocks, bs, cc, nb,
                                                         C.byref(collider) if collider is not None else None, C.byref(_levelset_view(levelset)),
                                                         b.data_ptr(), x.data_ptr(), int(max_iters), float(tol), float(rel_tol), C.byref(it)) != 0:
                raise RuntimeError("zs_rocm_mpm_implicit_solve_levelset refused its arguments")
            return it.value
        if lib().zs_rocm_mpm_implicit_solve(self.pol.handle, C.byref(self.params), self.particles(), self.table.handle, self.grid.data_ptr(),
                                            self.nblocks, bs, cc, nb, C.byref(collider) if collider is not None else None, b.data_ptr(),
                                            x.data_ptr(), int(max_iters), float(tol), float(rel_tol), C.byref(it)) != 0:
            raise RuntimeError("zs_rocm_mpm_implicit_solve refused its arguments")
        return it.value

    def build_buckets(self, displacement=0.0, dense=False):
        from .containers import IndexBuckets
        if getattr(self, "buckets", None) is None:
            self.buckets = IndexBuckets()
        if dense:
            assert displacement == 0.0
            self.buckets.build_for_partition(self.pol, self._port("x"), self.n, self.params.dx, self.table.handle, self.side,
                                             self.key_is_origin)
            return self.buckets
        cells = min(self.n, self.nblocks * self.side ** 3) if getattr(self, "nblocks", 0) else 0
        self.buckets.build(self.pol, self._port("x"), self.n, self.params.dx, displacement=displacement, expected_cells=cells)
        return self.buckets

    def p2c2g(self, kind=0):
        if lib().zs_rocm_mpm_p2c2g(self.pol.handle, C.byref(self.params), self.particles(), self.buckets._h, self.table.handle,
                                   self.grid.data_ptr(), self.nblocks, int(kind)) != 0:
            raise RuntimeError("zs_rocm_mpm_p2c2g refused its arguments")

    def g2c2p(self, fused=True):
        L = lib()
        if fused:
            if L.zs_rocm_mpm_g2c2p_step(self.pol.handle, C.byref(self.params), self.particles(), self.table.handle, self.grid.data_ptr(),
                                        self.nblocks) != 0:
                raise RuntimeError("zs_rocm_mpm_g2c2p_step refused its arguments")
            self.binned = False
            return
        L.zs_rocm_mpm_pre_g2c2p(self.pol.handle, self.particles())
        if L.zs_rocm_mpm_g2c2p(self.pol.handle, C.byref(self.params), self.particles(), None, self.table.handle, self.grid.data_ptr(),
                               self.nblocks) != 0:
            raise RuntimeError("zs_rocm_mpm_g2c2p refused its arguments")
        L.zs_rocm_mpm_post_g2c2p(self.pol.handle, C.byref(self.params), self.particles())
        self.binned = False

    def g2p2g(self, write_all=False, split=None, between=None, reorder=False):
        if self.slotted:
            if reorder:
                raise ValueError("slotted storage: no re-ordering steps (the step keeps the order itself)")
            if getattr(self, "grid2", None) is None or self.grid2.numel() != self.grid.numel():
                self.grid2 = torch.zeros_like(self.grid)
            else:
                self._zero(self.grid2)
            src, dst = self.grid, self.grid2
            self.grid, self.grid2 = dst, src
            ranges = [(0, self.nblocks)] if not split else [(0, int(split)), (int(split), self.nblocks)]
            for k, (b0, b1) in enumerate(ranges):
                rc = lib().zs_rocm_mpm_g2p2g_slots(self.pol.handle, C.byref(self.params), self.particles(), self.table.handle, src.data_ptr(),
                                                   dst.data_ptr(), self.nblocks, C.byref(self.slot_storage), int(write_all),
                                                   b0, b1, int(k == len(ranges) - 1))
                if rc != 0:
                    raise RuntimeError("zs_rocm_mpm_g2p2g_slotted refused the call")
                if k == 0 and between is not None:
                    between()
            return
        if not (self.cache_stress and self.binned):
            raise RuntimeError("g2p2g needs cache_stress=True and rebin()")
        src_buf = None
        if reorder and write_all:
            raise ValueError("a re-ordering step cannot also materialise v, C, stress (write_all)")
        if reorder:
            L = lib()
            if self.order is None or self.order.numel() != self.n:
                self.order = torch.empty(self.n, dtype=torch.int32, device=self.device)
            L.zs_rocm_mpm_bin_particles(self.pol.handle, self.table.handle, self._port("x"), self.n, self.params.dx, self.side,
                                        int(self.key_is_origin), self.order.data_ptr(), self.bin_start.data_ptr(),
                                        self.cell_count.data_ptr())
            if self.buf2 is None:
                self.buf2 = torch.empty_like(self.buf)
            src_buf, self.buf, self.buf2 = self.buf, self.buf2, self.buf
        if getattr(self, "grid2", None) is None or self.grid2.numel() != self.grid.numel():
            self.grid2 = torch.zeros_like(self.grid)
        else:
            self._zero(self.grid2)
        if self.drift_flag is None:
            self.drift_flag = torch.zeros(3, dtype=torch.int32, device=self.device)
        ranges = [(0, self.nblocks)] if not split else [(0, int(split)), (int(split), self.nblocks)]
        src, dst = self.grid, self.grid2
        self.grid, self.grid2 = dst, src
        for k, (b0, b1) in enumerate(ranges):
            if src_buf is None:
                rc = lib().zs_rocm_mpm_g2p2g_range(self.pol.handle, C.byref(self.params), self.particles(), self.table.handle, src.data_ptr(),
                                                   dst.data_ptr(), self.nblocks, self.bin_start.data_ptr(), self.cell_count.data_ptr(),
                                                   self.nbr.data_ptr(), int(write_all), b0, b1, self.drift_flag.data_ptr())
            else:
                rc = lib().zs_rocm_mpm_g2p2g_reorder_range(self.pol.handle, C.byref(self.params), self.particles(), self.particles(src_buf),
                                                           self.order.data_ptr(), self.table.handle, src.data_ptr(), dst.data_ptr(),
                                                           self.nblocks, self.bin_start.data_ptr(), self.cell_count.data_ptr(),
                                                           self.nbr.data_ptr(), int(write_all), b0, b1, self.drift_flag.data_ptr())
            if rc != 0:
                raise RuntimeError("zs_rocm_mpm_g2p2g refused the call")
            if k == 0 and between is not None:
                between()

    def step_slotted(self, extf=(0.0, 0.0, 0.0), max_vel=None, write_all=False, n_boundary=0, comm=None, plan=None, comm_pol=None,
                     collider=None, halo_grid=None, events=None, breakdown=None, halo_channels=7, range_schedule=0, handover_snapshot=None,
                     levelset=None):
        assert self.slotted
        tr = _transition_view(levelset)
        if tr is not None:
            if collider is None or comm is not None or plan is not None:
                raise RuntimeError("step_slotted: a level-set sequence needs a collider (type and motion) and runs on a single rank")
            self.step_slotted(extf, max_vel, write_all, n_boundary, None, None, comm_pol, None, halo_grid, events, breakdown, halo_channels,
                              range_schedule, handover_snapshot, None)
            self.apply_boundary(collider, levelset=tr)
            return
        if getattr(self, "grid2", None) is None or self.grid2.numel() != self.grid.numel():
            self.grid2 = torch.empty_like(self.grid)
        src, dst = self.grid, self.grid2
        a = getattr(self, "_step_args", None)
        if a is None:
            a = self._step_args = MpmStep()
        a.params = C.addressof(self.params)
        a.particles = self.particles()
        a.table = self.table.handle
        a.gridA, a.gridB = src.data_ptr(), dst.data_ptr()
        a.nblocks = self.nblocks
        a.storage = C.addressof(self.slot_storage)
        a.writeAll = int(write_all)
        a.extf = (C.c_float * 3)(*extf)
        a.maxVelSqr = max_vel.data_ptr() if max_vel is not None else None
        a.collider = C.addressof(collider) if collider is not None else None
        self._step_levelset = _levelset_view(levelset) if levelset is not None else None
        a.levelset = C.addressof(self._step_levelset) if levelset is not None else None
        a.nBoundary = int(n_boundary)
        a.dist = comm._h if comm is not None else None
        a.plan = plan._h if plan is not None else None
        a.commPolicy = comm_pol.handle if comm_pol is not None else None
        a.haloGrid = halo_grid.data_ptr() if halo_grid is not None else None
        a.haloChannels = int(halo_channels)
        a.rangeSchedule = int(range_schedule)
        a.handoverSnapshot = handover_snapshot.data_ptr() if handover_snapshot is not None else None
        a.evTransferBegin, a.evTransferEnd = (events[0], events[1]) if events is not None else (None, None)
        a.evBreakdown = breakdown if breakdown is not None else None
        if getattr(self, "_poisoned", False):
            raise RuntimeError("this MpmTransfer is poisoned: an earlier zs_rocm_mpm_step_slotted failed after committing the particle side of its step")
        if lib().zs_rocm_mpm_step_slotted(self.pol.handle, C.byref(a)) != 0:
            self._poisoned = True
            raise RuntimeError("zs_rocm_mpm_step_slotted failed: the step is half applied (particles advanced, grids not): this object cannot be stepped again")
        self.grid, self.grid2 = dst, src

    def margin_violated(self):
        return self.drift_tripped or (self.drift_flag is not None and bool(self.drift_flag[0].item()))

    def left_partition(self):
        return self.outside_tripped or (self.drift_flag is not None and bool(self.drift_flag[2].item()))

    def exact_path_particles(self, reset=True):
        if self.drift_flag is None:
            return 0
        c = int(self.drift_flag[1].item())
        if reset:
            self._zero(self.drift_flag[1:2])
        return c

    def reorder_partition(self, first_mask):
        import numpy as np
        keys = self.active_keys()
        m = np.asarray(first_mask).astype(bool)
        order = np.concatenate([np.nonzero(m)[0], np.nonzero(~m)[0]])
        pk = torch.from_numpy(np.ascontiguousarray(keys[order])).to(self.device)
        self.adopt_partition(pk.data_ptr(), keys.shape[0])
        self.pol.syncCtx()
        return int(m.sum())

    def active_keys(self):
        import ctypes
        v = self.table.view()
        nb = self.nblocks
        keys = torch.empty(max(nb, 1) * 3, dtype=torch.int32, device=self.device)
        self.pol.syncCtx()
        if nb:
            ctypes.CDLL("libamdhip64.so").hipMemcpy(ctypes.c_void_p(keys.data_ptr()), ctypes.c_void_p(v.activeKeys), ctypes.c_size_t(nb * 12), 3)
        return keys.cpu().numpy()[: nb * 3].reshape(nb, 3)

    def grid_by_key(self):
        v = self.table.view()
        nb = self.nblocks
        keys = torch.empty(nb * 3, dtype=torch.int32, device=self.device)
        import ctypes
        hip = ctypes.CDLL("libamdhip64.so")
        hip.hipMemcpy(ctypes.c_void_p(keys.data_ptr()), ctypes.c_void_p(v.activeKeys), ctypes.c_size_t(nb * 12), 3)
        k = keys.cpu().numpy().reshape(nb, 3)
        g = self.grid.cpu().numpy().reshape(nb, 7, self.side ** 3)
        return {tuple(int(x) for x in k[i]): g[i] for i in range(nb)}


class HipEvents:

    def __init__(self):
        self.hip = C.CDLL("libamdhip64.so")
        self.hip.hipEventElapsedTime.argtypes = [C.POINTER(C.c_float), C.c_void_p, C.c_void_p]
        self.pairs = []

    def pair(self):
        e = [C.c_void_p(), C.c_void_p()]
        for x in e:
            if self.hip.hipEventCreate(C.byref(x)) != 0:
                raise RuntimeError("hipEventCreate failed")
        self.pairs.append(e)
        return e[0], e[1]

    def elapsed_ms(self):
        out = []
        for a, b in self.pairs:
            ms = C.c_float(0)
            if self.hip.hipEventElapsedTime(C.byref(ms), a, b) == 0:
                out.append(ms.value)
        return out

    def __del__(self):
        try:
            for a, b in self.pairs:
                self.hip.hipEventDestroy(a)
                self.hip.hipEventDestroy(b)
        except Exception:
            pass


RANGES_IN_TURN, RANGES_SIDE_BY_SIDE, RANGES_ONE_LAUNCH = 0, 1, 2


class StepBreakdown:
    NEV = 8
    STRETCHES = (("boundary_range_ms", 0, 1), ("interior_range_ms", 1, 2), ("wait_for_exchange_ms", 2, 5), ("grid_update_ms", 5, 6),
                 ("cfl_allreduce_ms", 6, 7), ("exchange_side_stream_ms", 3, 4), ("step_ms", 0, 7),
                 ("both_ranges_ms", 0, 2))

    def __init__(self):
        self.hip = C.CDLL("libamdhip64.so")
        self.hip.hipEventElapsedTime.argtypes = [C.POINTER(C.c_float), C.c_void_p, C.c_void_p]
        self.steps = []

    def next(self):
        arr = (C.c_void_p * self.NEV)()
        for k in range(self.NEV):
            e = C.c_void_p()
            if self.hip.hipEventCreate(C.byref(e)) != 0:
                raise RuntimeError("hipEventCreate failed")
            arr[k] = e
        self.steps.append(arr)
        return arr

    def summary(self):
        out = {}
        for name, i, j in self.STRETCHES:
            v = []
            for arr in self.steps:
                ms = C.c_float(0)
                if self.hip.hipEventElapsedTime(C.byref(ms), C.c_void_p(arr[i]), C.c_void_p(arr[j])) == 0:
                    v.append(ms.value)
            out[name] = (sum(v) / len(v)) if v else None
        return out

    def __del__(self):
        try:
            for arr in self.steps:
                for k in range(self.NEV):
                    self.hip.hipEventDestroy(C.c_void_p(arr[k]))
        except Exception:
            pass


PLANE, CUBOID, SPHERE, CYLINDER = 0, 1, 2, 3
STICKY, SLIP, SEPARATE = 0, 1, 2


def make_collider(geometry, ctype, param, s=1.0, dsdt=0.0, R=None, omega=(0, 0, 0), b=(0, 0, 0), dbdt=(0, 0, 0)):
    from ._lib import Collider
    c = Collider()
    p = [float(v) for v in param]
    lib().zs_rocm_collider_init(C.byref(c), int(geometry), int(ctype), (C.c_float * len(p))(*p), len(p))
    c.s, c.dsdt = float(s), float(dsdt)
    if R is not None:
        c.R = (C.c_float * 9)(*[float(v) for v in (R.reshape(-1) if hasattr(R, "reshape") else R)])
    c.omega = (C.c_float * 3)(*[float(v) for v in omega])
    c.b = (C.c_float * 3)(*[float(v) for v in b])
    c.dbdt = (C.c_float * 3)(*[float(v) for v in dbdt])
    return c


def make_levelset_collider(ctype, s=1.0, dsdt=0.0, R=None, omega=(0, 0, 0), b=(0, 0, 0), dbdt=(0, 0, 0)):
    return make_collider(PLANE, ctype, (), s=s, dsdt=dsdt, R=R, omega=omega, b=b, dbdt=dbdt)


def _transition_view(levelset):
    from ._lib import LevelSetTransition
    from .levelset import LevelSetSequence
    if isinstance(levelset, LevelSetTransition):
        return levelset
    return levelset.view() if isinstance(levelset, LevelSetSequence) else None


def _levelset_view(levelset):
    return levelset.view if hasattr(levelset, "view") else levelset
```

Measured before the change: 10.79 billion.

## Fold source grid zeroing into the slotted step via per-block reader counts

Counts, for each grid block, how many slot blocks read it, and keeps an atomic read counter. The last reader of a block zeroes that block of gridA inside the fused G2P2G kernel, so gridA is already clean when it becomes the next step's gridB. This lets the step skip the full-grid memset. In exchange it adds per-block atomics and extra stores in the kernel, plus Python bookkeeping to track which buffer is known to be clean.

```diff
diff --git a/include/zs_rocm.h b/include/zs_rocm.h
--- a/include/zs_rocm.h
+++ b/include/zs_rocm.h
@@ -641,6 +641,10 @@
 #define ZS_ROCM_RANGES_SIDE_BY_SIDE 1
 #define ZS_ROCM_RANGES_ONE_LAUNCH 2
 ZS_ROCM_EXPORT int zs_rocm_mpm_step_slotted(zs_rocm_policy *, const zs_rocm_mpm_step *);
+ZS_ROCM_EXPORT int zs_rocm_mpm_build_block_readers(zs_rocm_policy *, const int *nbr , size_t nblocks, int *readers,
+                                                   unsigned *readCount);
+ZS_ROCM_EXPORT int zs_rocm_mpm_step_slotted_fold(zs_rocm_policy *, const zs_rocm_mpm_step *, const int *readers, unsigned *readCount,
+                                                 int gridBIsClean);
 
 #ifdef __cplusplus
 }
diff --git a/zpc_amd/_lib.py b/zpc_amd/_lib.py
--- a/zpc_amd/_lib.py
+++ b/zpc_amd/_lib.py
@@ -377,6 +377,10 @@
     L.zs_rocm_mpm_reslot.restype = i32
     L.zs_rocm_mpm_step_slotted.argtypes = [vp, C.POINTER(MpmStep)]
     L.zs_rocm_mpm_step_slotted.restype = i32
+    L.zs_rocm_mpm_step_slotted_fold.argtypes = [vp, C.POINTER(MpmStep), vp, vp, i32]
+    L.zs_rocm_mpm_step_slotted_fold.restype = i32
+    L.zs_rocm_mpm_build_block_readers.argtypes = [vp, vp, sz, vp, vp]
+    L.zs_rocm_mpm_build_block_readers.restype = i32
     L.zs_rocm_dist_halo_plan_from_lists.argtypes = [vp, i32, i32, C.POINTER(C.c_int), C.POINTER(C.c_size_t), C.POINTER(C.c_size_t),
                                                     C.POINTER(C.c_int), sz]
     L.zs_rocm_dist_halo_plan_from_lists.restype = vp
diff --git a/zpc_amd/csrc/common.hpp b/zpc_amd/csrc/common.hpp
--- a/zpc_amd/csrc/common.hpp
+++ b/zpc_amd/csrc/common.hpp
@@ -117,7 +117,7 @@
 
 int mpm_g2p2g_slots_signal(zs_rocm_policy *pol, const zs_rocm_mpm_params *p, zs_rocm_particles ps, const zs_rocm_bht_3 *tab, const float *gridA,
                            float *gridB, size_t nblocks, const zs_rocm_slot_storage *st, int writeAll, size_t blockBegin, size_t blockEnd, int finish,
-                           unsigned long long *signal, size_t signalBlocks);
+                           unsigned long long *signal, size_t signalBlocks, const int *readers, unsigned *readCount);
 bool levelset_collider_ok(const zs_rocm_collider *collider, const zs_rocm_levelset *levelset);
 void levelset_blocks_enqueue(hipStream_t stream, const zs_rocm_mpm_params *p, const int *activeKeys, float *grid, size_t nblocks,
                              const zs_rocm_collider *collider, const zs_rocm_levelset *levelset, float *dof);
diff --git a/zpc_amd/csrc/dist.hip b/zpc_amd/csrc/dist.hip
--- a/zpc_amd/csrc/dist.hip
+++ b/zpc_amd/csrc/dist.hip
@@ -360,14 +360,20 @@
 }
 extern "C" {
 
-int zs_rocm_mpm_step_slotted(zs_rocm_policy *pol, const zs_rocm_mpm_step *a) {
+int zs_rocm_mpm_step_slotted(zs_rocm_policy *pol, const zs_rocm_mpm_step *a) { return zs_rocm_mpm_step_slotted_fold(pol, a, nullptr, nullptr, 0); }
+int zs_rocm_mpm_step_slotted_fold(zs_rocm_policy *pol, const zs_rocm_mpm_step *a, const int *readers, unsigned *readCount, int gridBIsClean) {
   if (!pol || !a || !a->params || !a->table || !a->gridA || !a->gridB || !a->storage) return -1;
   if (a->levelset && !zsr::levelset_collider_ok(a->collider, a->levelset)) return -1;
   const size_t nb = a->nblocks;
   if (!nb) return 0;
   const int side = a->params->side;
+  if ((readers != nullptr) != (readCount != nullptr) || (readers && (side != 8 || ((uintptr_t)a->gridA & 15u) || a->gridA == a->gridB))) return -1;
   const size_t gridBytes = nb * (size_t)7 * side * side * side * sizeof(float);
-  zs_rocm_memset(pol, a->gridB, 0, gridBytes);
+  if (!gridBIsClean) zs_rocm_memset(pol, a->gridB, 0, gridBytes);
+  auto range = [&](zs_rocm_policy *on, size_t b0, size_t b1, int finish, unsigned long long *signal, size_t signalBlocks) {
+    return mpm_g2p2g_slots_signal(on, a->params, a->particles, a->table, a->gridA, a->gridB, nb, a->storage, a->writeAll, b0, b1, finish, signal, signalBlocks,
+                                  readers, readCount);
+  };
   float *const hgrid = a->haloGrid ? a->haloGrid : a->gridB;
   const bool exchange = a->dist && a->plan && a->plan->total;
   if (a->haloChannels < 0 || a->haloChannels > 7) return -1;
@@ -413,7 +419,7 @@
         ZSR_CHECK(hipStreamSynchronize(L.stream));
         p->signalTarget = 0;
       }
-      rc = mpm_g2p2g_slots_signal(pol, a->params, a->particles, a->table, a->gridA, a->gridB, nb, a->storage, a->writeAll, 0, nb, 1, p->signal, a->nBoundary);
+      rc = range(pol, 0, nb, 1, p->signal, a->nBoundary);
       if (rc) return rc;
       p->signalTarget += a->nBoundary;
       {
@@ -440,7 +446,7 @@
         Launch C(a->commPolicy, "step: boundary range start");
         ZSR_CHECK(hipStreamWaitEvent(C.stream, p->evReady, 0));
       }
-      rc = zs_rocm_mpm_g2p2g_slots(bpol, a->params, a->particles, a->table, a->gridA, a->gridB, nb, a->storage, a->writeAll, 0, a->nBoundary, 0);
+      rc = range(bpol, 0, a->nBoundary, 0, nullptr, 0);
       if (rc) return rc;
       bd(1, bpol);
       {
@@ -462,14 +468,14 @@
       ZSR_CHECK(hipEventRecord(p->evDone, C.stream));
     }
     if (sched == ZS_ROCM_RANGES_IN_TURN) {
-      rc = zs_rocm_mpm_g2p2g_slots(pol, a->params, a->particles, a->table, a->gridA, a->gridB, nb, a->storage, a->writeAll, a->nBoundary, nb, 1);
+      rc = range(pol, a->nBoundary, nb, 1, nullptr, 0);
     } else if (sched == ZS_ROCM_RANGES_SIDE_BY_SIDE) {
-      rc = zs_rocm_mpm_g2p2g_slots(pol, a->params, a->particles, a->table, a->gridA, a->gridB, nb, a->storage, a->writeAll, a->nBoundary, nb, 0);
+      rc = range(pol, a->nBoundary, nb, 0, nullptr, 0);
       {
         Launch L(pol, "step: wait for the boundary range");
         ZSR_CHECK(hipStreamWaitEvent(L.stream, p->evBoundary, 0));
       }
-      const int rcf = zs_rocm_mpm_g2p2g_slots(pol, a->params, a->particles, a->table, a->gridA, a->gridB, nb, a->storage, a->writeAll, nb, nb, 1);
+      const int rcf = range(pol, nb, nb, 1, nullptr, 0);
       if (!rc) rc = rcf;
     }
     bd(2, pol);
@@ -482,7 +488,7 @@
     if (rcx || rc) return rcx ? rcx : rc;
   } else {
     bd(1, pol);
-    rc = zs_rocm_mpm_g2p2g_slots(pol, a->params, a->particles, a->table, a->gridA, a->gridB, nb, a->storage, a->writeAll, 0, nb, 1);
+    rc = range(pol, 0, nb, 1, nullptr, 0);
     if (rc) return rc;
     bd(2, pol);
     stamp(a->evTransferEnd);
diff --git a/zpc_amd/csrc/mpm_slot.hpp b/zpc_amd/csrc/mpm_slot.hpp
--- a/zpc_amd/csrc/mpm_slot.hpp
+++ b/zpc_amd/csrc/mpm_slot.hpp
@@ -23,6 +23,8 @@
   const unsigned char *blockEdge;
   unsigned long long *signal;
   int signalBlocks;
+  const int *readers;
+  unsigned *readCount;
 };
 
 constexpr int SL_NCTR = 256, SL_SENT = 8, SL_DELIVERED = 8 + SL_NCTR;
diff --git a/zpc_amd/csrc/mpm_slotblk.hip b/zpc_amd/csrc/mpm_slotblk.hip
--- a/zpc_amd/csrc/mpm_slotblk.hip
+++ b/zpc_amd/csrc/mpm_slotblk.hip
@@ -126,6 +126,26 @@
       }
       __builtin_amdgcn_fence(__ATOMIC_ACQ_REL, "wavefront");
     }
+  }
+}
+
+__device__ __forceinline__ void blk_count_off(const SlotArgs &A, const int *nbr8, int lane) {
+  constexpr int NC = 512;
+  const int bn = lane < 8 ? nbr8[lane] : -1;
+  bool last = false;
+  if (bn >= 0) {
+    const unsigned nr = (unsigned)A.readers[bn];
+    const unsigned old = __hip_atomic_fetch_add(A.readCount + bn, 1u, __ATOMIC_RELAXED, __HIP_MEMORY_SCOPE_AGENT);
+    last = (old + 1u) % nr == 0u;
+  }
+  unsigned long long m = __ballot(last);
+  while (m) {
+    const int k = __builtin_ctzll(m);
+    m &= m - 1ull;
+    const int b = __builtin_amdgcn_readlane(bn, k);
+    float4 *g = reinterpret_cast<float4 *>(const_cast<float *>(A.gridA) + (size_t)b * 7 * NC);
+#pragma unroll
+    for (int i = 0; i < 7 * NC / 4 / 64; ++i) g[i * 64 + lane] = make_float4(0.f, 0.f, 0.f, 0.f);
   }
 }
 
@@ -221,6 +241,7 @@
     blk_chunk_descs(sh.desc, -1 + 1, d);
     binState(-1, d[2], d[3]);
   }
+  if (CS == 0 && A.readers) blk_count_off(A, sh.nbr8, lane);
   for (int g = 0; g < G; ++g) {
     __syncthreads();
     ChunkDesc d[5];
@@ -353,6 +374,7 @@
   if ((s_total[0] | s_total[1] | s_total[2] | s_total[3] | s_total[4] | s_total[5] | s_total[6] | s_total[7]) == 0) {
     if (tid < 8) A.moverCount[bin0 + tid] = 0;
     if (A.signal && blk < A.signalBlocks && tid == 0) atomicAdd(A.signal, 1ull);
+    if (w == 4 && A.readers) blk_count_off(A, s_nbr8, lane);
     return;
   }
   if (tid == 0) {
diff --git a/zpc_amd/csrc/mpm_slotted.hip b/zpc_amd/csrc/mpm_slotted.hip
--- a/zpc_amd/csrc/mpm_slotted.hip
+++ b/zpc_amd/csrc/mpm_slotted.hip
@@ -278,6 +278,12 @@
   const bool dup = lane_id() != 0 && pvalid && px == b[0] && py == b[1] && pz == b[2];
   if (valid && !dup) bht_insert<3>(newT, b);
 }
+static __global__ __launch_bounds__(256) void block_readers_kernel(const int *nbr, size_t n8, int nblocks, int *readers) {
+  const size_t i = blockIdx.x * (size_t)blockDim.x + threadIdx.x;
+  if (i >= n8) return;
+  const int b = nbr[i];
+  if (b >= 0 && b < nblocks) atomicAdd(readers + b, 1);
+}
 static __global__ __launch_bounds__(256) void reslot_map_kernel(BhtDev oldT, int nOld, BhtDev newT, int *map) {
   const int i = (int)(blockIdx.x * blockDim.x + threadIdx.x);
   if (i >= nOld) return;
@@ -333,6 +339,16 @@
   if (!nb) return;
   hipLaunchKernelGGL(build_neighbors27_kernel, dim3(ceil_div((size_t)nb * 27, 256)), dim3(256), 0, L.stream, tab->t.dev(), nb, nbr27,
                      keyStride > 0 ? keyStride : 1);
+}
+
+int zs_rocm_mpm_build_block_readers(zs_rocm_policy *pol, const int *nbr, size_t nblocks, int *readers, unsigned *readCount) {
+  if (!nblocks) return 0;
+  if (!nbr || !readers || !readCount || nblocks > (size_t)1 << 28) return -1;
+  Launch L(pol, "build_block_readers");
+  ZSR_CHECK(hipMemsetAsync(readers, 0, sizeof(int) * nblocks, L.stream));
+  ZSR_CHECK(hipMemsetAsync(readCount, 0, sizeof(unsigned) * nblocks, L.stream));
+  hipLaunchKernelGGL(block_readers_kernel, dim3(ceil_div(nblocks * 8, 256)), dim3(256), 0, L.stream, nbr, nblocks * 8, (int)nblocks, readers);
+  return 0;
 }
 
 int zs_rocm_mpm_slot_particles(zs_rocm_policy *pol, const zs_rocm_bht_3 *tab, zs_rocm_attr pos, size_t n, float dx, int side, int keyIsOrigin,
@@ -376,15 +392,16 @@
 int zs_rocm_mpm_g2p2g_slots(zs_rocm_policy *pol, const zs_rocm_mpm_params *p, zs_rocm_particles ps, const zs_rocm_bht_3 *tab,
                             const float *gridA, float *gridB, size_t nblocks, const zs_rocm_slot_storage *st, int writeAll,
                             size_t blockBegin, size_t blockEnd, int finish) {
-  return zsr::mpm_g2p2g_slots_signal(pol, p, ps, tab, gridA, gridB, nblocks, st, writeAll, blockBegin, blockEnd, finish, nullptr, 0);
+  return zsr::mpm_g2p2g_slots_signal(pol, p, ps, tab, gridA, gridB, nblocks, st, writeAll, blockBegin, blockEnd, finish, nullptr, 0, nullptr, nullptr);
 }
 }
 namespace zsr {
 int mpm_g2p2g_slots_signal(zs_rocm_policy *pol, const zs_rocm_mpm_params *p, zs_rocm_particles ps, const zs_rocm_bht_3 *tab, const float *gridA,
                            float *gridB, size_t nblocks, const zs_rocm_slot_storage *st, int writeAll, size_t blockBegin, size_t blockEnd, int finish,
-                           unsigned long long *signal, size_t signalBlocks) {
+                           unsigned long long *signal, size_t signalBlocks, const int *readers, unsigned *readCount) {
   if (!st) return -1;
   if (signal && p->side != 8) return -1;
+  if ((readers != nullptr) != (readCount != nullptr) || (readers && (p->side != 8 || ((uintptr_t)gridA & 15u)))) return -1;
   unsigned *const cellMask = st->cellMask;
   const int K = st->K, outboxCap = st->outboxCap;
   const int *const nbr = st->nbr, *const nbr27 = st->nbr27;
@@ -407,7 +424,7 @@
   const unsigned nbinsAll = (unsigned)(nblocks * bpb);
   const unsigned nbins = blockBegin < blockEnd ? (unsigned)((blockEnd - blockBegin) * bpb) : 0u;
   const SlotArgs A{gridA, gridB, cellMask, K, nbr, nbr27, moverCount, claim, moverRec, status, (int)(blockBegin * bpb), (int)nbins, (int)nbinsAll, outboxCap,
-                   st->blockEdge, signal, (int)signalBlocks};
+                   st->blockEdge, signal, (int)signalBlocks, readers, readCount};
 #define CALL_REHOME3(M, WA)                                                                                                              \
   hipLaunchKernelGGL((slot_rehome_kernel<model_is_fluid(M), model_uses_logjp(M), WA>), dim3(ceil_div((size_t)nbinsAll, 32)), dim3(256), 0,  \
                      L.stream, pd, (const unsigned *)cellMask, claim, (const int *)moverCount, (const float *)moverRec, outboxCap,        \
diff --git a/zpc_amd/mpm.py b/zpc_amd/mpm.py
--- a/zpc_amd/mpm.py
+++ b/zpc_amd/mpm.py
@@ -51,6 +51,33 @@
         self.n_slots = 0
         self.K = 0
         self.slot_record = {"sent": 0, "homed": 0, "flags": [0] * 5, "periods": 0, "edge_periods": 0, "log": []}
+        self.block_readers = self.read_count = None
+        self._clean_ptr = None
+
+    @property
+    def grid2_clean(self):
+        g2 = getattr(self, "grid2", None)
+        return g2 is not None and self._clean_ptr is not None and self._clean_ptr == g2.data_ptr()
+
+    def _grids_touched(self, grid=None):
+        if grid is None or self._clean_ptr == grid.data_ptr():
+            self._clean_ptr = None
+
+    def _build_block_readers(self, pooled=False):
+        self._clean_ptr = None
+        if self.side != 8:
+            self.block_readers = self.read_count = None
+            return
+        nb = max(self.nblocks, 1)
+        if pooled:
+            self.block_readers = self._backing("readers", nb, torch.int32, spare=True)
+            self.read_count = self._backing("readcnt", nb, torch.int32, spare=True)
+        else:
+            self.block_readers = torch.empty(nb, dtype=torch.int32, device=self.device)
+            self.read_count = torch.empty(nb, dtype=torch.int32, device=self.device)
+        if lib().zs_rocm_mpm_build_block_readers(self.pol.handle, self.nbr.data_ptr(), self.nblocks, self.block_readers.data_ptr(),
+                                                 self.read_count.data_ptr()) != 0:
+            raise RuntimeError("zs_rocm_mpm_build_block_readers refused its arguments")
 
     def _zero(self, t):
         lib().zs_rocm_memset(self.pol.handle, t.data_ptr(), 0, t.numel() * t.element_size())
@@ -142,6 +169,7 @@
         self.nbr = torch.empty(self.nblocks * 8, dtype=torch.int32, device=self.device)
         L.zs_rocm_mpm_build_neighbors(self.pol.handle, self.table.handle, self.nbr.data_ptr(), self.kstride)
         self.binned = False
+        self.block_readers = self.read_count = self._clean_ptr = None
         return self.nblocks
 
     def adopt_partition(self, active_keys_ptr, nblocks):
@@ -154,6 +182,7 @@
         self.nbr = torch.empty(self.nblocks * 8, dtype=torch.int32, device=self.device)
         L.zs_rocm_mpm_build_neighbors(self.pol.handle, self.table.handle, self.nbr.data_ptr(), self.kstride)
         self.binned = False
+        self.block_readers = self.read_count = self._clean_ptr = None
         return self.nblocks
 
     def rebin(self, inputs_only=False):
@@ -205,6 +234,7 @@
                                           self.cell_mask.data_ptr(), self.slot_status.data_ptr())
         if rc != 0:
             raise RuntimeError("zs_rocm_mpm_slot_particles refused its arguments")
+        self._build_block_readers()
         self.mover_count = torch.zeros(L.zs_rocm_mpm_slot_outbox_bytes(self.nbins, self.outbox_cap, 0) // 4, dtype=torch.int32, device=self.device)
         self.mover_dest = torch.zeros(L.zs_rocm_mpm_slot_outbox_bytes(self.nbins, self.outbox_cap, 1) // 4, dtype=torch.int32, device=self.device)
         self.mover_rec = torch.empty(L.zs_rocm_mpm_slot_outbox_bytes(self.nbins, self.outbox_cap, 2) // 4, dtype=torch.float32, device=self.device)
@@ -288,6 +318,7 @@
         self.grid2 = self._backing("gridB%d" % flip, nb * 7 * nc, torch.float32, zero=True)
         self.nbr = self._backing("nbr", nb * 8, torch.int32, spare=True)
         L.zs_rocm_mpm_build_neighbors(self.pol.handle, self.table.handle, self.nbr.data_ptr(), self.kstride)
+        self._build_block_readers(pooled=True)
         self.nbr27 = self._backing("nbr27", nb * 27, torch.int32, spare=True)
         L.zs_rocm_mpm_build_neighbors27(self.pol.handle, self.table.handle, self.nbr27.data_ptr(), self.kstride)
         self.block_edge = self._backing("edge", max(nb, 1), torch.uint8, spare=True)
@@ -322,6 +353,7 @@
         if cnt != self.n:
             raise RuntimeError("slotted storage holds %d particles, %d went in: particles were lost" % (cnt, self.n))
         self.slotted = False
+        self._grids_touched()
         self.tiles = (cnt + 63) // 64
         self.buf, self.buf2 = out, None
         self.binned = False
@@ -369,6 +401,7 @@
         return bool(w.any())
 
     def clear_grid(self):
+        self._grids_touched()
         self._zero(self.grid)
 
     def p2g(self, binned=None):
@@ -376,6 +409,7 @@
         bs = self.bin_start.data_ptr() if binned else None
         cc = self.cell_count.data_ptr() if binned else None
         nb = self.nbr.data_ptr() if binned else None
+        self._grids_touched()
         lib().zs_rocm_mpm_p2g(self.pol.handle, C.byref(self.params), self.particles(), self.table.handle, self.grid.data_ptr(),
                               self.nblocks, bs, cc, nb)
 
@@ -385,6 +419,7 @@
                                       max_vel.data_ptr() if max_vel is not None else None)
 
     def apply_boundary(self, collider, levelset=None):
+        self._grids_touched(self.grid)
         tr = _transition_view(levelset)
         if tr is not None:
             if lib().zs_rocm_mpm_apply_boundary_transition(self.pol.handle, C.byref(self.params), self.table.handle, self.grid.data_ptr(),
@@ -523,6 +558,7 @@
         self.binned = False
 
     def g2p2g(self, write_all=False, split=None, between=None, reorder=False):
+        self._grids_touched()
         if self.slotted:
             if reorder:
                 raise ValueError("slotted storage: no re-ordering steps (the step keeps the order itself)")
@@ -583,14 +619,14 @@
 
     def step_slotted(self, extf=(0.0, 0.0, 0.0), max_vel=None, write_all=False, n_boundary=0, comm=None, plan=None, comm_pol=None,
                      collider=None, halo_grid=None, events=None, breakdown=None, halo_channels=7, range_schedule=0, handover_snapshot=None,
-                     levelset=None):
+                     levelset=None, fold=True):
         assert self.slotted
         tr = _transition_view(levelset)
         if tr is not None:
             if collider is None or comm is not None or plan is not None:
                 raise RuntimeError("step_slotted: a level-set sequence needs a collider (type and motion) and runs on a single rank")
             self.step_slotted(extf, max_vel, write_all, n_boundary, None, None, comm_pol, None, halo_grid, events, breakdown, halo_channels,
-                              range_schedule, handover_snapshot, None)
+                              range_schedule, handover_snapshot, None, fold)
             self.apply_boundary(collider, levelset=tr)
             return
         if getattr(self, "grid2", None) is None or self.grid2.numel() != self.grid.numel():
@@ -623,10 +659,16 @@
         a.evBreakdown = breakdown if breakdown is not None else None
         if getattr(self, "_poisoned", False):
             raise RuntimeError("this MpmTransfer is poisoned: an earlier zs_rocm_mpm_step_slotted failed after committing the particle side of its step")
-        if lib().zs_rocm_mpm_step_slotted(self.pol.handle, C.byref(a)) != 0:
+        fold = bool(fold) and self.side == 8 and self.block_readers is not None
+        clean = fold and self.grid2_clean
+        self._clean_ptr = None
+        if lib().zs_rocm_mpm_step_slotted_fold(self.pol.handle, C.byref(a), self.block_readers.data_ptr() if fold else None,
+                                               self.read_count.data_ptr() if fold else None, int(clean)) != 0:
             self._poisoned = True
             raise RuntimeError("zs_rocm_mpm_step_slotted failed: the step is half applied (particles advanced, grids not): this object cannot be stepped again")
         self.grid, self.grid2 = dst, src
+        if fold:
+            self._clean_ptr = src.data_ptr()
 
     def margin_violated(self):
         return self.drift_tripped or (self.drift_flag is not None and bool(self.drift_flag[0].item()))
```

Result: no change. 10.88 billion, median of 6 (+0.8%).
